# gillesdegottex/percivaltts

Hardware: AMD Instinct MI355X
Metric: acoustic frames/sec per WGAN-GP critic+gen step (higher is better)
Workload: dtype f32

## Files before the change

### percivaltts_amd/csrc/dense.hip

```cpp
#include "common.h"
#include <cstdlib>

namespace ptts {
namespace dns {

typedef __bf16 bf16x8 __attribute__((ext_vector_type(8)));
typedef __bf16 bf16x4 __attribute__((ext_vector_type(4)));
typedef __bf16 bf16x2 __attribute__((ext_vector_type(2)));
typedef float f32x4 __attribute__((ext_vector_type(4)));
typedef float f32x2 __attribute__((ext_vector_type(2)));
typedef unsigned u32x2 __attribute__((ext_vector_type(2)));
typedef unsigned short u16;

constexpr int THREADS = 512;
constexpr int NBLK = 256;
constexpr int BK = 32;

#define DNS_PRODUCTS(X) X(2, 0) X(1, 1) X(0, 2) X(1, 0) X(0, 1) X(0, 0)
#define DNS_PRODUCTS_NPL(NPL, X) do { if (NPL == 3) { X(2, 0) X(1, 1) X(0, 2) X(1, 0) X(0, 1) } X(0, 0) } while (0)

__device__ __forceinline__ unsigned pk_bf16(float a, float b) {
    return __builtin_bit_cast(unsigned, __builtin_convertvector((f32x2){a, b}, bf16x2));
}
__device__ __forceinline__ void split3_pair(float a, float b, unsigned& p1, unsigned& p2, unsigned& p3) {
    p1 = pk_bf16(a, b);
    const float ra = a - __builtin_bit_cast(float, p1 << 16), rb = b - __builtin_bit_cast(float, p1 & 0xffff0000u);
    p2 = pk_bf16(ra, rb);
    const float sa = ra - __builtin_bit_cast(float, p2 << 16), sb = rb - __builtin_bit_cast(float, p2 & 0xffff0000u);
    p3 = pk_bf16(sa, sb);
}
__device__ __forceinline__ float max_fast(float a, float b) {
    float r;
    asm("v_max_f32 %0, %1, %2" : "=v"(r) : "v"(a), "v"(b));
    return r;
}

__global__ __launch_bounds__(256) void split3_dense_weight_kernel(const float* __restrict__ w, long long ldw, int K, int N,
                                                                  int transposed, u16* __restrict__ planes, int NT, int KS) {
    const long long idx = (long long)blockIdx.x * 256 + threadIdx.x;
    if (idx >= (long long)NT * KS * 64) return;
    const int lane = (int)(idx & 63);
    const long long t = idx >> 6;
    const int ks = (int)(t % KS), nt = (int)(t / KS);
    const int n = nt * 16 + (lane & 15), k0 = ks * 32 + (lane >> 4) * 8;
    float v[8];
#pragma unroll
    for (int e = 0; e < 8; ++e) {
        const int k = k0 + e;
        v[e] = (n < N && k < K) ? (transposed ? w[(long long)n * ldw + k] : w[(long long)k * ldw + n]) : 0.f;
    }
    unsigned q[3][4];
#pragma unroll
    for (int h = 0; h < 4; ++h) split3_pair(v[2 * h], v[2 * h + 1], q[0][h], q[1][h], q[2][h]);
    const size_t ps = (size_t)NT * KS * 512;
#pragma unroll
    for (int p = 0; p < 3; ++p)
        *reinterpret_cast<uint4*>(planes + p * ps + (size_t)idx * 8) = make_uint4(q[p][0], q[p][1], q[p][2], q[p][3]);
}

constexpr int SPLIT_GROUP = 32;
struct SplitGroupArgs {
    const float* w[SPLIT_GROUP]; u16* planes[SPLIT_GROUP];
    long long ldw[SPLIT_GROUP];
    int K[SPLIT_GROUP], N[SPLIT_GROUP], transposed[SPLIT_GROUP], NT[SPLIT_GROUP], KS[SPLIT_GROUP];
    int rlo[SPLIT_GROUP], rhi[SPLIT_GROUP];
};
__global__ __launch_bounds__(256) void split3_dense_weight_grouped_kernel(SplitGroupArgs a) {
    const int i = blockIdx.y;
    const int NT = a.NT[i], KS = a.KS[i], K = a.K[i], N = a.N[i], transposed = a.transposed[i];
    const int rlo = a.rlo[i], rhi = a.rhi[i];
    const long long idx = (long long)blockIdx.x * 256 + threadIdx.x;
    if (idx >= (long long)NT * KS * 64) return;
    const float* __restrict__ w = a.w[i];
    u16* __restrict__ planes = a.planes[i];
    const long long ldw = a.ldw[i];
    const int lane = (int)(idx & 63);
    const long long t = idx >> 6;
    const int ks = (int)(t % KS), nt = (int)(t / KS);
    const int n = nt * 16 + (lane & 15), k0 = ks * 32 + (lane >> 4) * 8;
    float v[8];
#pragma unroll
    for (int e = 0; e < 8; ++e) {
        const int k = k0 + e;
        v[e] = (n < N && k < K && k >= rlo && k < rhi) ? (transposed ? w[(long long)n * ldw + k] : w[(long long)k * ldw + n]) : 0.f;
    }
    unsigned q[3][4];
#pragma unroll
    for (int h = 0; h < 4; ++h) split3_pair(v[2 * h], v[2 * h + 1], q[0][h], q[1][h], q[2][h]);
    const size_t ps = (size_t)NT * KS * 512;
#pragma unroll
    for (int p = 0; p < 3; ++p)
        *reinterpret_cast<uint4*>(planes + p * ps + (size_t)idx * 8) = make_uint4(q[p][0], q[p][1], q[p][2], q[p][3]);
}

constexpr int WDFT_FCH = 32;
template <int KW>
__global__ __launch_bounds__(256) void conv1d_wdft_planes_kernel(const float* __restrict__ w, const float* __restrict__ tw,
                                                                u16* __restrict__ planes, long long fstride, int NB, int Cin,
                                                                int N, int Kh, int NT, int KS) {
    const long long idx = (long long)blockIdx.x * 256 + threadIdx.x;
    if (idx >= (long long)NT * KS * 64) return;
    const int lane = (int)(idx & 63);
    const long long t = idx >> 6;
    const int ks = (int)(t % KS), nt = (int)(t / KS);
    const int n = nt * 16 + (lane & 15), k0 = ks * 32 + (lane >> 4) * 8;
    const int part = k0 >= Kh ? 1 : 0, c0 = k0 - part * Kh;
    float wr[KW][8];
#pragma unroll
    for (int k = 0; k < KW; ++k)
#pragma unroll
        for (int e = 0; e < 8; ++e)
            wr[k][e] = (n < N && c0 + e < Cin && k0 < 2 * Kh) ? w[((long long)k * Cin + c0 + e) * N + n] : 0.f;
    const size_t ps = (size_t)NT * KS * 512;
    const int f0 = blockIdx.y * WDFT_FCH;
    for (int f = f0; f < min(NB, f0 + WDFT_FCH); ++f) {
        const float* __restrict__ tr = tw + ((long long)f * 2 + part) * KW;
        float v[8] = {0.f, 0.f, 0.f, 0.f, 0.f, 0.f, 0.f, 0.f};
#pragma unroll
        for (int k = 0; k < KW; ++k) {
            const float c = tr[k];
#pragma unroll
            for (int e = 0; e < 8; ++e) v[e] = fmaf(c, wr[k][e], v[e]);
        }
        unsigned q[3][4];
#pragma unroll
        for (int h = 0; h < 4; ++h) split3_pair(v[2 * h], v[2 * h + 1], q[0][h], q[1][h], q[2][h]);
        u16* pf = planes + (long long)f * fstride;
#pragma unroll
        for (int p = 0; p < 3; ++p)
            *reinterpret_cast<uint4*>(pf + p * ps + (size_t)idx * 8) = make_uint4(q[p][0], q[p][1], q[p][2], q[p][3]);
    }
}

struct SplitStridedArgs {
    const float* w; u16* planes;
    long long stride_w, stride_p, ldw;
    int K, N, transposed, NT, KS;
    int windows;
    int T, NS, S, row_off, kvalid;
};
__global__ __launch_bounds__(256) void split3_dense_weight_strided_kernel(SplitStridedArgs a) {
    const int z = blockIdx.y;
    const int NT = a.NT, KS = a.KS, K = a.K, N = a.N, transposed = a.transposed;
    const long long idx = (long long)blockIdx.x * 256 + threadIdx.x;
    if (idx >= (long long)NT * KS * 64) return;
    const float* __restrict__ w;
    int rlo = 0, rhi = K;
    if (a.windows) {
        const int b = z / a.NS, sg = z - b * a.NS;
        const int r0 = a.row_off + sg * a.S;
        w = a.w + ((long long)b * a.T + r0) * a.ldw;
        rlo = r0 < 0 ? -r0 : 0;
        rhi = min(a.kvalid, a.T - r0);
    } else {
        w = a.w + (long long)z * a.stride_w;
    }
    u16* __restrict__ planes = a.planes + (long long)z * a.stride_p;
    const long long ldw = a.ldw;
    const int lane = (int)(idx & 63);
    const long long t = idx >> 6;
    const int ks = (int)(t % KS), nt = (int)(t / KS);
    const int n = nt * 16 + (lane & 15), k0 = ks * 32 + (lane >> 4) * 8;
    float v[8];
#pragma unroll
    for (int e = 0; e < 8; ++e) {
        const int k = k0 + e;
        v[e] = (n < N && k < K && k >= rlo && k < rhi) ? (transposed ? w[(long long)n * ldw + k] : w[(long long)k * ldw + n]) : 0.f;
    }
    unsigned q[3][4];
#pragma unroll
    for (int h = 0; h < 4; ++h) split3_pair(v[2 * h], v[2 * h + 1], q[0][h], q[1][h], q[2][h]);
    const size_t ps = (size_t)NT * KS * 512;
#pragma unroll
    for (int p = 0; p < 3; ++p)
        *reinterpret_cast<uint4*>(planes + p * ps + (size_t)idx * 8) = make_uint4(q[p][0], q[p][1], q[p][2], q[p][3]);
}

constexpr int SPL_ROW = 256 + 2;
__global__ __launch_bounds__(256) void split3_dense_weight_strided_lds_kernel(SplitStridedArgs a) {
    __shared__ float tile[32 * SPL_ROW];
    const int z = blockIdx.y, ks = blockIdx.x % a.KS, cb = blockIdx.x / a.KS;
    const float* __restrict__ w = a.w + (long long)z * a.stride_w;
    u16* __restrict__ planes = a.planes + (long long)z * a.stride_p;
    const int lane = threadIdx.x & 63, wave = threadIdx.x >> 6;
    const int n0 = cb * 256;
#pragma unroll
    for (int j = 0; j < 8; ++j) {
        const int r = wave + 4 * j, k = ks * 32 + r, n = n0 + 4 * lane;
        f32x4 v = {0.f, 0.f, 0.f, 0.f};
        if (k < a.K && n < a.N) v = *reinterpret_cast<const f32x4*>(w + (long long)k * a.ldw + n);
        float* d = tile + r * SPL_ROW + 4 * lane;
        d[0] = v[0]; d[1] = v[1]; d[2] = v[2]; d[3] = v[3];
    }
    __syncthreads();
    const size_t ps = (size_t)a.NT * a.KS * 512;
    const int li = lane & 15, lg = lane >> 4;
#pragma unroll
    for (int j = 0; j < 4; ++j) {
        const int ntl = wave + 4 * j;
        const int nt = cb * 16 + ntl;
        if (nt >= a.NT) continue;
        float v[8];
#pragma unroll
        for (int e = 0; e < 8; ++e) v[e] = tile[(8 * lg + e) * SPL_ROW + 16 * ntl + li];
        unsigned q[3][4];
#pragma unroll
        for (int h = 0; h < 4; ++h) split3_pair(v[2 * h], v[2 * h + 1], q[0][h], q[1][h], q[2][h]);
        const size_t idx = ((size_t)nt * a.KS + ks) * 64 + lane;
#pragma unroll
        for (int p = 0; p < 3; ++p)
            *reinterpret_cast<uint4*>(planes + p * ps + idx * 8) = make_uint4(q[p][0], q[p][1], q[p][2], q[p][3]);
    }
}

#ifndef DNS_DEPTH
#define DNS_DEPTH 2
#endif
struct DenseArgs {
    const float* A; const float* mask_src; const float* in_scale; const float* in_shift;
    const u16* planes; const float* bias; const float* out_mask; float* C;
    int M, N, K, NT, KS;
    long long lda, ldc;
    float alpha, out_alpha;
    int accumulate, has_affine, vec_out;
    const float* res; int res_rows; long long ldr;
    long long bsA, bsP, bsC;
    double* stats;
    const float* om_scale; const float* om_shift;
};

template <int MODE, bool AFFINE, int MT, int NPL>
__global__ __launch_bounds__(THREADS) void dense_bf16x6_kernel(DenseArgs g) {
    if (gridDim.z > 1) {
        g.A += (long long)blockIdx.z * g.bsA;
        g.planes += (long long)blockIdx.z * g.bsP;
        g.C += (long long)blockIdx.z * g.bsC;
    }
    constexpr int TBM = 16 * MT;
    constexpr int NA = (TBM * 8 + THREADS - 1) / THREADS;
    constexpr int ROWS = NA * THREADS / 8;
    constexpr int PL = ROWS * BK;
    constexpr bool MASK = MODE == PTTS_IN_MASKMUL;
    __shared__ __attribute__((aligned(16))) u16 As[2][NPL * PL];
    const int tid = threadIdx.x, lane = tid & 63;
    const int wave = __builtin_amdgcn_readfirstlane(tid >> 6);
    const int li = lane & 15, lg = lane >> 4;
    const int m0 = blockIdx.x * TBM, n0 = blockIdx.y * NBLK;
    const int KS = g.KS;
    const bool wave_live = n0 + 32 * wave < g.N;

    const int kq = tid & 7;
    const float* pa[NA]; const float* pm[NA]; bool oka[NA]; int dst[NA];
#pragma unroll
    for (int j = 0; j < NA; ++j) {
        const int row = (tid + j * THREADS) >> 3;
        oka[j] = row < TBM && m0 + row < g.M;
        const long long base = (long long)(oka[j] ? m0 + row : 0) * g.lda + 4 * kq;
        pa[j] = g.A + base;
        pm[j] = MASK ? g.mask_src + base : nullptr;
        dst[j] = row * BK + ((((kq >> 1) ^ ((row >> 1) & 2))) << 3) + (kq & 1) * 4;
    }
    struct Stage { f32x4 va[NA], vm[MASK ? NA : 1], sc, sh; bool kok; };
    auto load_a = [&](int s, Stage& sg) {
        const int k = s * BK + 4 * kq;
        sg.kok = k < g.K;
        const int ko = sg.kok ? s * BK : -4 * kq;
#pragma unroll
        for (int j = 0; j < NA; ++j) {
            sg.va[j] = *reinterpret_cast<const f32x4*>(pa[j] + ko);
            if (MASK) sg.vm[j] = *reinterpret_cast<const f32x4*>(pm[j] + ko);
        }
        if (AFFINE) {
            sg.sc = *reinterpret_cast<const f32x4*>(g.in_scale + (sg.kok ? k : 0));
            sg.sh = *reinterpret_cast<const f32x4*>(g.in_shift + (sg.kok ? k : 0));
        }
    };
    auto commit = [&](const Stage& sg, u16* as) {
        const f32x4 z4 = {0.f, 0.f, 0.f, 0.f};
#pragma unroll
        for (int j = 0; j < NA; ++j) {
            f32x4 a = sg.va[j];
            if (MODE == PTTS_IN_LRELU) {
                if (AFFINE) a = a * sg.sc + sg.sh;
                if (!(oka[j] && sg.kok)) a = z4;
#pragma unroll
                for (int e = 0; e < 4; ++e) a[e] = max_fast(a[e], g.alpha * a[e]);
            } else if (MASK) {
                if (!(oka[j] && sg.kok)) a = z4;
#pragma unroll
                for (int e = 0; e < 4; ++e) a[e] = a[e] * (sg.vm[j][e] > 0.f ? 1.f : g.alpha);
            } else {
                if (!(oka[j] && sg.kok)) a = z4;
            }
            u16* d = as + dst[j];
            if (NPL == 3) {
                unsigned a1, a2, a3, b1, b2, b3;
                split3_pair(a[0], a[1], a1, a2, a3);
                split3_pair(a[2], a[3], b1, b2, b3);
                *reinterpret_cast<u32x2*>(d) = (u32x2){a1, b1};
                *reinterpret_cast<u32x2*>(d + PL) = (u32x2){a2, b2};
                *reinterpret_cast<u32x2*>(d + 2 * PL) = (u32x2){a3, b3};
            } else {
                *reinterpret_cast<u32x2*>(d) = (u32x2){pk_bf16(a[0], a[1]), pk_bf16(a[2], a[3])};
            }
        }
    };

    const size_t ps = (size_t)g.NT * KS * 512;
    const u16* wp[2];
#pragma unroll
    for (int j = 0; j < 2; ++j) wp[j] = g.planes + (((size_t)((n0 >> 4) + 2 * (wave_live ? wave : 0) + j) * KS) * 64 + lane) * 8;
    auto load_w = [&](int s, bf16x8 (&wf)[2][NPL]) {
#pragma unroll
        for (int j = 0; j < 2; ++j)
#pragma unroll
            for (int p = 0; p < NPL; ++p) wf[j][p] = *reinterpret_cast<const bf16x8*>(wp[j] + p * ps + (size_t)s * 512);
    };

    f32x4 acc[MT][2];
#pragma unroll
    for (int i = 0; i < MT; ++i) { acc[i][0] = f32x4{0.f, 0.f, 0.f, 0.f}; acc[i][1] = f32x4{0.f, 0.f, 0.f, 0.f}; }
    const int boff = li * BK + ((lg ^ ((li >> 1) & 2)) << 3);
    auto mfma_rows = [&](const u16* as, const bf16x8 (&wf)[2][NPL], int i0, int i1) {
#pragma unroll
        for (int i = i0; i < i1; ++i) {
            bf16x8 bf[NPL];
#pragma unroll
            for (int p = 0; p < NPL; ++p) bf[p] = *reinterpret_cast<const bf16x8*>(as + p * PL + boff + i * 16 * BK);
#define DNS_MM(PA, PW)                                                                                    \
            acc[i][0] = __builtin_amdgcn_mfma_f32_16x16x32_bf16(wf[0][PW < NPL ? PW : 0], bf[PA < NPL ? PA : 0], acc[i][0], 0, 0, 0);    \
            acc[i][1] = __builtin_amdgcn_mfma_f32_16x16x32_bf16(wf[1][PW < NPL ? PW : 0], bf[PA < NPL ? PA : 0], acc[i][1], 0, 0, 0);
            DNS_PRODUCTS_NPL(NPL, DNS_MM);
#undef DNS_MM
        }
    };

    constexpr int DEPTH = DNS_DEPTH;
    Stage sg[DEPTH];
    bf16x8 wc[2][NPL], wn[2][NPL];
#pragma unroll
    for (int j = 0; j < DEPTH; ++j) load_a(j, sg[j]);
    load_w(0, wc);
    commit(sg[0], As[0]);
    load_a(DEPTH, sg[0]);
    __syncthreads();
    auto step = [&](int s, int cut, Stage& nx) {
        const u16* as = As[s & 1];
        load_w(s + 1 < KS ? s + 1 : s, wn);
        mfma_rows(as, wc, 0, cut);
        commit(nx, As[(s + 1) & 1]);
        load_a(s + 1 + DEPTH, nx);
        mfma_rows(as, wc, cut, MT);
#pragma unroll
        for (int j = 0; j < 2; ++j)
#pragma unroll
            for (int p = 0; p < NPL; ++p) wc[j][p] = wn[j][p];
        __syncthreads();
    };
    auto run = [&](int cut) {
        int s = 0;
        for (; s + DEPTH <= KS; s += DEPTH) {
#pragma unroll
            for (int j = 0; j < DEPTH; ++j) step(s + j, cut, sg[(j + 1) % DEPTH]);
        }
#pragma unroll
        for (int j = 0; j < DEPTH; ++j)
            if (s + j < KS) step(s + j, cut, sg[(j + 1) % DEPTH]);
    };
    if (wave < 4) run(2); else run(MT - 2);
    if (!wave_live) return;
    const bool interior = m0 + TBM <= g.M;
    if (!g.vec_out) {
#pragma unroll
        for (int j = 0; j < 2; ++j)
#pragma unroll
            for (int i = 0; i < MT; ++i) {
                const int m = m0 + 16 * i + li;
                if (m >= g.M) continue;
#pragma unroll
                for (int e = 0; e < 4; ++e) {
                    const int n = n0 + 32 * wave + 16 * j + 4 * lg + e;
                    if (n >= g.N) continue;
                    const long long off = (long long)m * g.ldc + n;
                    float v = acc[i][j][e] + (g.bias ? g.bias[n] : 0.f);
                    if (g.out_mask) v *= g.out_mask[off] > 0.f ? 1.f : g.out_alpha;
                    if (g.res) { int mr = m; while (mr >= g.res_rows) mr -= g.res_rows; v += g.res[(long long)mr * g.ldr + n]; }
                    g.C[off] = v;
                }
            }
        return;
    }
#pragma unroll
    for (int j = 0; j < 2; ++j) {
        const int n = n0 + 32 * wave + 16 * j + 4 * lg;
        if (n >= g.N) continue;
        f32x4 bv = {0.f, 0.f, 0.f, 0.f};
        if (g.bias) bv = *reinterpret_cast<const f32x4*>(g.bias + n);
        const long long off0 = (long long)(m0 + li) * g.ldc + n;
        auto res_at = [&](int m) { int mr = m; while (mr >= g.res_rows) mr -= g.res_rows; return g.res + (long long)mr * g.ldr + n; };
        f32x4 ssum = {0.f, 0.f, 0.f, 0.f}, ssq = {0.f, 0.f, 0.f, 0.f};
        f32x4 osc = {1.f, 1.f, 1.f, 1.f}, osh = {0.f, 0.f, 0.f, 0.f};
        if (g.om_scale) { osc = *reinterpret_cast<const f32x4*>(g.om_scale + n); osh = *reinterpret_cast<const f32x4*>(g.om_shift + n); }
        auto aff_store = [&](f32x4& v, const f32x4& z) {
#pragma unroll
            for (int e = 0; e < 4; ++e) {
                const float gd = v[e] * ((z[e] * osc[e] + osh[e]) > 0.f ? 1.f : g.out_alpha);
                ssum[e] += gd * z[e]; ssq[e] += gd;
                v[e] = gd * osc[e];
            }
        };
        if (interior) {
            f32x4 mk[MT], old[MT];
            if (g.out_mask) {
#pragma unroll
                for (int i = 0; i < MT; ++i) mk[i] = *reinterpret_cast<const f32x4*>(g.out_mask + off0 + (long long)16 * i * g.ldc);
            }
            if (g.res) {
#pragma unroll
                for (int i = 0; i < MT; ++i) old[i] = *reinterpret_cast<const f32x4*>(res_at(m0 + 16 * i + li));
            }
#pragma unroll
            for (int i = 0; i < MT; ++i) {
                f32x4 v = acc[i][j] + bv;
                if (g.om_scale) {
                    aff_store(v, mk[i]);
                } else if (g.out_mask) {
#pragma unroll
                    for (int e = 0; e < 4; ++e) v[e] = v[e] * (mk[i][e] > 0.f ? 1.f : g.out_alpha);
                }
                if (g.res) v += old[i];
                if (g.stats && !g.om_scale) { ssum += v; ssq += v * v; }
                *reinterpret_cast<f32x4*>(g.C + off0 + (long long)16 * i * g.ldc) = v;
            }
        } else {
#pragma unroll
            for (int i = 0; i < MT; ++i) {
                const int m = m0 + 16 * i + li;
                if (m >= g.M) continue;
                const long long off = off0 + (long long)16 * i * g.ldc;
                f32x4 v = acc[i][j] + bv;
                if (g.out_mask) {
                    const f32x4 mk = *reinterpret_cast<const f32x4*>(g.out_mask + off);
                    if (g.om_scale) {
                        aff_store(v, mk);
                    } else {
#pragma unroll
                        for (int e = 0; e < 4; ++e) v[e] = v[e] * (mk[e] > 0.f ? 1.f : g.out_alpha);
                    }
                }
                if (g.res) v += *reinterpret_cast<const f32x4*>(res_at(m));
                if (g.stats && !g.om_scale) { ssum += v; ssq += v * v; }
                *reinterpret_cast<f32x4*>(g.C + off) = v;
            }
        }
        if (g.stats) {
#pragma unroll
            for (int e = 0; e < 4; ++e)
#pragma unroll
                for (int m = 1; m < 16; m <<= 1) { ssum[e] += __shfl_xor(ssum[e], m, 64); ssq[e] += __shfl_xor(ssq[e], m, 64); }
            if (li == 0) {
                double* row = g.stats + (size_t)blockIdx.x * 2 * g.N;
#pragma unroll
                for (int e = 0; e < 4; ++e) { row[n + e] = (double)ssum[e]; row[g.N + n + e] = (double)ssq[e]; }
            }
        }
    }
}

static int pick_mt(int M, int col_blocks) {
    static int forced = -1;
    if (forced < 0) { const char* e = getenv("PTTS_DENSE_MT"); forced = e ? atoi(e) : 0; }
    if (forced >= 4 && forced <= 8) return forced;
    int best = 8; double best_eff = -1.0;
    for (int mt = 4; mt <= 8; ++mt) {
        const long long blocks = (long long)((M + 16 * mt - 1) / (16 * mt)) * col_blocks;
        const long long rounds = (blocks + 255) / 256;
        const double eff = (double)M * col_blocks / (double)(rounds * 256 * 16 * mt);
        if (eff > best_eff + 1e-9) { best_eff = eff; best = mt; }
    }
    return best;
}


typedef short s16x4 __attribute__((ext_vector_type(4)));
typedef s16x4 __attribute__((address_space(3)))* lds_s16x4_ptr;
__device__ __forceinline__ bf16x4 tr_read(const u16* p) {
    return __builtin_bit_cast(bf16x4, __builtin_amdgcn_ds_read_tr16_b64_v4i16((lds_s16x4_ptr)(p)));
}
__device__ __forceinline__ bf16x8 cat8(bf16x4 a, bf16x4 b) { return __builtin_shufflevector(a, b, 0, 1, 2, 3, 4, 5, 6, 7); }

struct WgradArgs {
    const float* A; const float* dY; const float* mask_src; const float* in_scale; const float* in_shift;
    float* partials;
    int Kin, N, M;
    long long lda, ldb;
    float alpha;
    int tiles_n, steps_total, split;
};

constexpr int WT = 128;
constexpr int WROW = WT;
constexpr int WPL = 32 * WROW;
constexpr int WPART = WT * WT + WT;

template <int MODE, bool AFFINE, int NPL>
__global__ __launch_bounds__(THREADS) void dense_wgrad_bf16x6_kernel(WgradArgs g) {
    constexpr bool MASK = MODE == PTTS_IN_MASKMUL;
    extern __shared__ __attribute__((aligned(16))) u16 lds_w[];
    const int tid = threadIdx.x, lane = tid & 63;
    const int wave = __builtin_amdgcn_readfirstlane(tid >> 6);
    const int li = lane & 15, lg = lane >> 4;
    const int tile = blockIdx.y, tk = tile / g.tiles_n, tn = tile - tk * g.tiles_n;
    const int k0 = tk * WT, n0 = tn * WT;
    const int per = (g.steps_total + g.split - 1) / g.split;
    const int s_begin = blockIdx.x * per, s_end = min(g.steps_total, s_begin + per);
    const int nsteps = max(0, s_end - s_begin);

    const int c4 = tid & 31;
    const bool a_ok = k0 + 4 * c4 < g.Kin, d_ok = n0 + 4 * c4 < g.N;
    const float* pa = g.A + (a_ok ? k0 + 4 * c4 : 0);
    const float* pm = MASK ? g.mask_src + (a_ok ? k0 + 4 * c4 : 0) : nullptr;
    const float* pd = g.dY + (d_ok ? n0 + 4 * c4 : 0);
    int dst[2];
#pragma unroll
    for (int j = 0; j < 2; ++j) {
        const int row = (tid + j * THREADS) >> 5;
        dst[j] = row * WROW + ((((c4 >> 2) + row + 4 * (row >> 3)) & 7) << 4) + (c4 & 3) * 4;
    }
    f32x4 sc = {1.f, 1.f, 1.f, 1.f}, sh = {0.f, 0.f, 0.f, 0.f};
    if (AFFINE && a_ok) { sc = *reinterpret_cast<const f32x4*>(g.in_scale + k0 + 4 * c4); sh = *reinterpret_cast<const f32x4*>(g.in_shift + k0 + 4 * c4); }
    struct Stage { f32x4 va[2], vm[MASK ? 2 : 1], vd[2]; bool ok[2]; };
    auto load = [&](int s, Stage& sg) {
#pragma unroll
        for (int j = 0; j < 2; ++j) {
            const int m = (s_begin + s) * 32 + ((tid + j * THREADS) >> 5);
            sg.ok[j] = s < nsteps && m < g.M;
            const long long r = sg.ok[j] ? m : 0;
            sg.va[j] = *reinterpret_cast<const f32x4*>(pa + r * g.lda);
            if (MASK) sg.vm[j] = *reinterpret_cast<const f32x4*>(pm + r * g.lda);
            sg.vd[j] = *reinterpret_cast<const f32x4*>(pd + r * g.ldb);
        }
    };
    f32x4 bsum = {0.f, 0.f, 0.f, 0.f};
    auto commit = [&](const Stage& sg, u16* ls) {
        const f32x4 z4 = {0.f, 0.f, 0.f, 0.f};
#pragma unroll
        for (int j = 0; j < 2; ++j) {
            f32x4 a = sg.va[j], d = sg.vd[j];
            if (MODE == PTTS_IN_LRELU) {
                if (AFFINE) a = a * sc + sh;
                if (!(sg.ok[j] && a_ok)) a = z4;
#pragma unroll
                for (int e = 0; e < 4; ++e) a[e] = max_fast(a[e], g.alpha * a[e]);
            } else if (MASK) {
                if (!(sg.ok[j] && a_ok)) a = z4;
#pragma unroll
                for (int e = 0; e < 4; ++e) a[e] = a[e] * (sg.vm[j][e] > 0.f ? 1.f : g.alpha);
            } else {
                if (!(sg.ok[j] && a_ok)) a = z4;
            }
            if (!(sg.ok[j] && d_ok)) d = z4;
            bsum += d;
            u16* q = ls + dst[j];
            if (NPL == 3) {
                unsigned a1, a2, a3, b1, b2, b3;
                split3_pair(a[0], a[1], a1, a2, a3);
                split3_pair(a[2], a[3], b1, b2, b3);
                *reinterpret_cast<u32x2*>(q) = (u32x2){a1, b1};
                *reinterpret_cast<u32x2*>(q + WPL) = (u32x2){a2, b2};
                *reinterpret_cast<u32x2*>(q + 2 * WPL) = (u32x2){a3, b3};
                split3_pair(d[0], d[1], a1, a2, a3);
                split3_pair(d[2], d[3], b1, b2, b3);
                q += 3 * WPL;
                *reinterpret_cast<u32x2*>(q) = (u32x2){a1, b1};
                *reinterpret_cast<u32x2*>(q + WPL) = (u32x2){a2, b2};
                *reinterpret_cast<u32x2*>(q + 2 * WPL) = (u32x2){a3, b3};
            } else {
                *reinterpret_cast<u32x2*>(q) = (u32x2){pk_bf16(a[0], a[1]), pk_bf16(a[2], a[3])};
                *reinterpret_cast<u32x2*>(q + 3 * WPL) = (u32x2){pk_bf16(d[0], d[1]), pk_bf16(d[2], d[3])};
            }
        }
    };

    auto tr_off = [&](int t, int half) {
        const int row = 8 * lg + (li >> 2) + 4 * half;
        return row * WROW + (((t + row + 4 * (row >> 3)) & 7) << 4) + (li & 3) * 4;
    };
    int ao[2][2], bo[4][2];
#pragma unroll
    for (int h = 0; h < 2; ++h) {
#pragma unroll
        for (int i = 0; i < 2; ++i) ao[i][h] = tr_off(2 * (wave & 3) + i, h);
#pragma unroll
        for (int i = 0; i < 4; ++i) bo[i][h] = 3 * WPL + tr_off(4 * (wave >> 2) + i, h);
    }
    f32x4 acc[2][4];
#pragma unroll
    for (int i = 0; i < 2; ++i)
#pragma unroll
        for (int j = 0; j < 4; ++j) acc[i][j] = f32x4{0.f, 0.f, 0.f, 0.f};
    auto mfma_tile_row = [&](const u16* ls, int i, const bf16x8 (&bf)[4][NPL]) {
        bf16x8 af[NPL];
#pragma unroll
        for (int p = 0; p < NPL; ++p) af[p] = cat8(tr_read(ls + p * WPL + ao[i][0]), tr_read(ls + p * WPL + ao[i][1]));
#define DNS_MM(PA, PW)                                                                                       \
        _Pragma("unroll") for (int j = 0; j < 4; ++j)                                                        \
            acc[i][j] = __builtin_amdgcn_mfma_f32_16x16x32_bf16(af[PA < NPL ? PA : 0], bf[j][PW < NPL ? PW : 0], acc[i][j], 0, 0, 0);
        DNS_PRODUCTS_NPL(NPL, DNS_MM);
#undef DNS_MM
    };
    auto read_bf = [&](const u16* ls, bf16x8 (&bf)[4][NPL]) {
#pragma unroll
        for (int j = 0; j < 4; ++j)
#pragma unroll
            for (int p = 0; p < NPL; ++p) bf[j][p] = cat8(tr_read(ls + p * WPL + bo[j][0]), tr_read(ls + p * WPL + bo[j][1]));
    };

    Stage sg;
    load(0, sg);
    commit(sg, lds_w);
    load(1, sg);
    __syncthreads();
    u16* const buf0 = lds_w;
    u16* const buf1 = lds_w + 6 * WPL;
    auto step = [&](int s, const u16* cur, u16* nxt, bool stage_first) {
        bf16x8 bf[4][NPL];
        if (stage_first) { commit(sg, nxt); load(s + 2, sg); }
        read_bf(cur, bf);
        mfma_tile_row(cur, 0, bf);
        if (!stage_first) { commit(sg, nxt); load(s + 2, sg); }
        mfma_tile_row(cur, 1, bf);
        __syncthreads();
    };
    if (wave < 4) {
        int s = 0;
        for (; s + 1 < nsteps; s += 2) { step(s, buf0, buf1, false); step(s + 1, buf1, buf0, false); }
        if (s < nsteps) step(s, buf0, buf1, false);
    } else {
        int s = 0;
        for (; s + 1 < nsteps; s += 2) { step(s, buf0, buf1, true); step(s + 1, buf1, buf0, true); }
        if (s < nsteps) step(s, buf0, buf1, true);
    }

    float* out = g.partials + ((size_t)tile * g.split + blockIdx.x) * WPART;
#pragma unroll
    for (int i = 0; i < 2; ++i)
#pragma unroll
        for (int j = 0; j < 4; ++j) {
            const int n = 64 * (wave >> 2) + 16 * j + li;
#pragma unroll
            for (int r = 0; r < 4; ++r) {
                const int k = 32 * (wave & 3) + 16 * i + 4 * lg + r;
                out[k * WT + n] = acc[i][j][r];
            }
        }
    {
        float* red = reinterpret_cast<float*>(lds_w);
        __syncthreads();
        *reinterpret_cast<f32x4*>(red + tid * 4) = bsum;
        __syncthreads();
        if (tid < WT) {
            float v = 0.f;
#pragma unroll
            for (int q = 0; q < 16; ++q) v += red[(q * 32 + (tid >> 2)) * 4 + (tid & 3)];
            out[WT * WT + tid] = v;
        }
    }
}


constexpr int DR_MAX = 16;
struct DwReduceArgs {
    int n;
    int blk_begin[DR_MAX + 1];
    const float* partials[DR_MAX]; float* C[DR_MAX]; float* colsum[DR_MAX];
    int split[DR_MAX], tiles_n[DR_MAX], Kin[DR_MAX], N[DR_MAX];
    long long ldc[DR_MAX];
};
constexpr int DR_BPT = (WPART + 255) / 256;
__global__ __launch_bounds__(256) void dense_wgrad_reduce_kernel(DwReduceArgs a) {
    int gi = 0;
    while ((int)blockIdx.x >= a.blk_begin[gi + 1]) ++gi;
    const int b = blockIdx.x - a.blk_begin[gi];
    const int tile = b / DR_BPT, e = (b - tile * DR_BPT) * 256 + threadIdx.x;
    if (e >= WPART) return;
    const int S = a.split[gi];
    const float* p = a.partials[gi] + (size_t)tile * S * WPART + e;
    float v0 = 0.f, v1 = 0.f, v2 = 0.f, v3 = 0.f, v4 = 0.f, v5 = 0.f, v6 = 0.f, v7 = 0.f;
    int s = 0;
    for (; s + 8 <= S; s += 8) {
        const float* q = p + (size_t)s * WPART;
        const float t0 = q[0], t1 = q[(size_t)WPART], t2 = q[(size_t)2 * WPART], t3 = q[(size_t)3 * WPART];
        const float t4 = q[(size_t)4 * WPART], t5 = q[(size_t)5 * WPART], t6 = q[(size_t)6 * WPART], t7 = q[(size_t)7 * WPART];
        v0 += t0; v1 += t1; v2 += t2; v3 += t3; v4 += t4; v5 += t5; v6 += t6; v7 += t7;
    }
    for (; s < S; ++s) v0 += p[(size_t)s * WPART];
    const float v = ((v0 + v1) + (v2 + v3)) + ((v4 + v5) + (v6 + v7));
    const int tk = tile / a.tiles_n[gi], tn = tile - tk * a.tiles_n[gi];
    if (e < WT * WT) {
        const int k = tk * WT + (e >> 7), n = tn * WT + (e & (WT - 1));
        if (k < a.Kin[gi] && n < a.N[gi]) atomicAdd(a.C[gi] + (long long)k * a.ldc[gi] + n, v);
    } else if (tk == 0 && a.colsum[gi]) {
        const int n = tn * WT + (e - WT * WT);
        if (n < a.N[gi]) atomicAdd(a.colsum[gi] + n, v);
    }
}

}
}

using namespace ptts;
using namespace ptts::dns;

extern "C" size_t ptts_dense_planes_bytes(int N, int K) {
    if (N <= 0 || K <= 0) return 0;
    const size_t NT = (size_t)((N + NBLK - 1) / NBLK) * (NBLK / 16), KS = (size_t)(K + BK - 1) / BK;
    return 3 * NT * KS * 512 * sizeof(u16);
}

extern "C" int ptts_split3_dense_weight(const float* w, long long ldw, int K, int N, int transposed, void* planes, void* stream) {
    PTTS_REQUIRE(w && planes, "split3_dense_weight: null pointer");
    PTTS_REQUIRE(K > 0 && N > 0 && ldw >= (transposed ? K : N), "split3_dense_weight: bad dims K=%d N=%d ldw=%lld", K, N, ldw);
    const int NT = (N + NBLK - 1) / NBLK * (NBLK / 16), KS = (K + BK - 1) / BK;
    const long long total = (long long)NT * KS * 64;
    hipLaunchKernelGGL(split3_dense_weight_kernel, dim3((unsigned)((total + 255) / 256)), dim3(256), 0, (hipStream_t)stream,
                       w, ldw, K, N, transposed, (u16*)planes, NT, KS);
    return check_launch("split3_dense_weight");
}

extern "C" int ptts_split3_dense_weight_grouped(const ptts_dense_split_desc* descs, int n, void* stream) {
    PTTS_REQUIRE(descs && n > 0, "split3_dense_weight_grouped: nothing to split");
    for (int base = 0; base < n; base += SPLIT_GROUP) {
        SplitGroupArgs a;
        const int m = n - base < SPLIT_GROUP ? n - base : SPLIT_GROUP;
        long long most = 0;
        for (int i = 0; i < m; ++i) {
            const ptts_dense_split_desc& d = descs[base + i];
            PTTS_REQUIRE(d.w && d.planes, "split3_dense_weight_grouped: null pointer (weight %d)", base + i);
            PTTS_REQUIRE(d.K > 0 && d.N > 0 && d.ldw >= (d.transposed ? d.K : d.N), "split3_dense_weight_grouped: bad dims K=%d N=%d ldw=%lld (weight %d)", d.K, d.N, d.ldw, base + i);
            a.w[i] = d.w; a.planes[i] = (u16*)d.planes; a.ldw[i] = d.ldw; a.K[i] = d.K; a.N[i] = d.N; a.transposed[i] = d.transposed;
            a.rlo[i] = 0; a.rhi[i] = d.K;
            a.NT[i] = (d.N + NBLK - 1) / NBLK * (NBLK / 16); a.KS[i] = (d.K + BK - 1) / BK;
            const long long total = (long long)a.NT[i] * a.KS[i] * 64;
            if (total > most) most = total;
        }
        hipLaunchKernelGGL(split3_dense_weight_grouped_kernel, dim3((unsigned)((most + 255) / 256), (unsigned)m), dim3(256), 0, (hipStream_t)stream, a);
    }
    return check_launch("split3_dense_weight_grouped");
}

extern "C" int ptts_split3_dense_weight_strided(const float* w, long long stride_w, void* planes, long long stride_planes_bytes, int n,
                                                long long ldw, int K, int N, int transposed, void* stream) {
    PTTS_REQUIRE(w && planes && n > 0 && n <= 65535, "split3_dense_weight_strided: nothing to split (or more than 65535 matrices)");
    PTTS_REQUIRE(K > 0 && N > 0 && ldw >= (transposed ? K : N), "split3_dense_weight_strided: bad dims K=%d N=%d ldw=%lld", K, N, ldw);
    PTTS_REQUIRE(stride_planes_bytes % 16 == 0, "split3_dense_weight_strided: the planes' stride must keep 16-byte alignment");
    SplitStridedArgs a;
    a.w = w; a.planes = (u16*)planes; a.stride_w = stride_w; a.stride_p = stride_planes_bytes / 2; a.ldw = ldw;
    a.K = K; a.N = N; a.transposed = transposed;
    a.NT = (N + NBLK - 1) / NBLK * (NBLK / 16); a.KS = (K + BK - 1) / BK;
    a.windows = 0; a.T = a.NS = a.S = a.row_off = a.kvalid = 0;
    const long long total = (long long)a.NT * a.KS * 64;
    static int lds_form = -1;
    if (lds_form < 0) { const char* e = getenv("PTTS_SPLIT_LDS"); lds_form = e ? atoi(e) : 1; }
    if (lds_form && !transposed && N % 4 == 0 && ldw % 4 == 0 && stride_w % 4 == 0 && ((uintptr_t)w & 15) == 0) {
        const unsigned cbn = (unsigned)((N + 255) / 256);
        hipLaunchKernelGGL(split3_dense_weight_strided_lds_kernel, dim3((unsigned)a.KS * cbn, (unsigned)n), dim3(256), 0, (hipStream_t)stream, a);
        return check_launch("split3_dense_weight_strided");
    }
    hipLaunchKernelGGL(split3_dense_weight_strided_kernel, dim3((unsigned)((total + 255) / 256), (unsigned)n), dim3(256), 0, (hipStream_t)stream, a);
    return check_launch("split3_dense_weight_strided");
}

extern "C" int ptts_split3_frame_windows(const float* x, int B, int T, int C, int NS, int S, int row_off, int P, int kvalid,
                                         void* planes, long long stride_planes_bytes, void* stream) {
    PTTS_REQUIRE(x && planes && B > 0 && T > 0 && C > 0 && NS > 0 && S > 0 && P > 0 && kvalid > 0 && kvalid <= P, "split3_frame_windows: bad arguments");
    PTTS_REQUIRE((long long)B * NS <= 65535 && stride_planes_bytes % 16 == 0, "split3_frame_windows: more than 65535 windows, or a planes stride off 16-byte alignment");
    SplitStridedArgs a;
    a.w = x; a.planes = (u16*)planes; a.stride_w = 0; a.stride_p = stride_planes_bytes / 2; a.ldw = C;
    a.K = P; a.N = C; a.transposed = 0;
    a.NT = (C + NBLK - 1) / NBLK * (NBLK / 16); a.KS = (P + BK - 1) / BK;
    a.windows = 1; a.T = T; a.NS = NS; a.S = S; a.row_off = row_off; a.kvalid = kvalid;
    const long long total = (long long)a.NT * a.KS * 64;
    hipLaunchKernelGGL(split3_dense_weight_strided_kernel, dim3((unsigned)((total + 255) / 256), (unsigned)(B * NS)), dim3(256), 0, (hipStream_t)stream, a);
    return check_launch("split3_frame_windows");
}

extern "C" int ptts_dense_bf16x6_supported(int M, int N, int K, long long lda, long long ldc) {
    (void)ldc;
    return (M > 0 && N > 0 && K > 0 && K % 4 == 0 && lda % 4 == 0 && K <= 65536 &&
            (long long)((N + NBLK - 1) / NBLK) <= 65535) ? 1 : 0;
}

extern "C" int ptts_dense_bf16x6_res(const float* A, const void* planes, const float* bias, float* C, int M, int N, int K,
                                     long long lda, long long ldc, int in_mode, const float* in_scale, const float* in_shift,
                                     const float* mask_src, float alpha, const float* res, int res_rows, long long ldr,
                                     const float* out_mask, void* stream);
extern "C" int ptts_dense_bf16x6(const float* A, const void* planes, const float* bias, float* C, int M, int N, int K,
                                 long long lda, long long ldc, int in_mode, const float* in_scale, const float* in_shift,
                                 const float* mask_src, float alpha, int accumulate, const float* out_mask, void* stream) {
    return ptts_dense_bf16x6_res(A, planes, bias, C, M, N, K, lda, ldc, in_mode, in_scale, in_shift, mask_src, alpha,
                                 accumulate ? C : nullptr, M, ldc, out_mask, stream);
}

static int dense_launch(const float* A, const void* planes, const float* bias, float* C, int M, int N, int K,
                        long long lda, long long ldc, int in_mode, const float* in_scale, const float* in_shift,
                        const float* mask_src, float alpha, const float* res, int res_rows, long long ldr,
                        const float* out_mask, double* stats, int stats_capacity_rows, int* stats_rows_out, void* stream);
static thread_local const float* g_om_scale = nullptr;
static thread_local const float* g_om_shift = nullptr;

extern "C" int ptts_dense_bf16x6_res(const float* A, const void* planes, const float* bias, float* C, int M, int N, int K,
                                     long long lda, long long ldc, int in_mode, const float* in_scale, const float* in_shift,
                                     const float* mask_src, float alpha, const float* res, int res_rows, long long ldr,
                                     const float* out_mask, void* stream) {
    return dense_launch(A, planes, bias, C, M, N, K, lda, ldc, in_mode, in_scale, in_shift, mask_src, alpha, res, res_rows, ldr, out_mask,
                        nullptr, 0, nullptr, stream);
}

extern "C" int ptts_dense_bf16x6_stats(const float* A, const void* planes, const float* bias, float* C, int M, int N, int K,
                                       long long lda, long long ldc, int in_mode, const float* in_scale, const float* in_shift,
                                       float alpha, double* stats, int capacity_rows, int* nrows_out, void* stream) {
    PTTS_REQUIRE(stats && nrows_out && capacity_rows > 0, "dense_bf16x6_stats: no room for the sums");
    return dense_launch(A, planes, bias, C, M, N, K, lda, ldc, in_mode, in_scale, in_shift, nullptr, alpha, nullptr, 0, 0, nullptr,
                        stats, capacity_rows, nrows_out, stream);
}
extern "C" int ptts_dense_bf16x6_bwd_affine(const float* A, const void* planes, float* C, int M, int N, int K, long long lda, long long ldc,
                                            const float* z, const float* scale, const float* shift, float alpha,
                                            double* stats, int capacity_rows, int* nrows_out, void* stream) {
    PTTS_REQUIRE(z && scale && shift && stats && nrows_out && capacity_rows > 0, "dense_bf16x6_bwd_affine: null pointer");
    PTTS_REQUIRE((((uintptr_t)scale | (uintptr_t)shift) & 15) == 0, "dense_bf16x6_bwd_affine: scale / shift must be 16-byte aligned");
    g_om_scale = scale; g_om_shift = shift;
    const int rc = dense_launch(A, planes, nullptr, C, M, N, K, lda, ldc, PTTS_IN_NONE, nullptr, nullptr, nullptr, alpha, nullptr, 0, 0, z,
                                stats, capacity_rows, nrows_out, stream);
    g_om_scale = g_om_shift = nullptr;
    return rc;
}
extern "C" int ptts_dense_bf16x6_stats_rows(int M, int N) {
    if (M <= 0 || N <= 0) return 0;
    const int mt = pick_mt(M, (N + NBLK - 1) / NBLK);
    return (M + 16 * mt - 1) / (16 * mt);
}

static int dense_launch(const float* A, const void* planes, const float* bias, float* C, int M, int N, int K,
                        long long lda, long long ldc, int in_mode, const float* in_scale, const float* in_shift,
                        const float* mask_src, float alpha, const float* res, int res_rows, long long ldr,
                        const float* out_mask, double* stats, int stats_capacity_rows, int* stats_rows_out, void* stream) {
    const int accumulate = res != nullptr;
    PTTS_REQUIRE(!res || (res_rows > 0 && ldr >= N && M <= 8LL * res_rows), "dense_bf16x6: bad residual (rows %d, ldr %lld)", res_rows, ldr);
    PTTS_REQUIRE(A && planes && C, "dense_bf16x6: null matrix");
    PTTS_REQUIRE(ptts_dense_bf16x6_supported(M, N, K, lda, ldc), "dense_bf16x6: unsupported shape M=%d N=%d K=%d lda=%lld ldc=%lld (K and lda must be multiples of 4)", M, N, K, lda, ldc);
    PTTS_REQUIRE(lda >= K && ldc >= N, "dense_bf16x6: bad leading dims");
    PTTS_REQUIRE(in_mode >= 0 && in_mode <= 2, "dense_bf16x6: bad in_mode %d", in_mode);
    PTTS_REQUIRE((in_scale == nullptr) == (in_shift == nullptr), "dense_bf16x6: scale/shift must come together");
    PTTS_REQUIRE(in_mode != PTTS_IN_MASKMUL || mask_src, "dense_bf16x6: MASKMUL needs mask_src");
    PTTS_REQUIRE(in_mode == PTTS_IN_LRELU || !in_scale, "dense_bf16x6: scale/shift need PTTS_IN_LRELU");
    PTTS_REQUIRE(!(out_mask && bias), "dense_bf16x6: out_mask with bias is not defined");
    PTTS_REQUIRE(alpha >= 0.f && alpha <= 1.f, "dense_bf16x6: LeakyReLU slope %g outside [0, 1]", alpha);
    const bool vec_out = N % 4 == 0 && ldc % 4 == 0 && ((uintptr_t)C & 15) == 0 && (!bias || ((uintptr_t)bias & 15) == 0) &&
                         (!out_mask || ((uintptr_t)out_mask & 15) == 0) && (!res || (((uintptr_t)res & 15) == 0 && ldr % 4 == 0));
    PTTS_REQUIRE(((uintptr_t)A & 15) == 0 && (!mask_src || ((uintptr_t)mask_src & 15) == 0) &&
                 (!in_scale || (((uintptr_t)in_scale | (uintptr_t)in_shift) & 15) == 0), "dense_bf16x6: A, its mask and scale/shift must be 16-byte aligned");
    DenseArgs g;
    g.A = A; g.mask_src = mask_src; g.in_scale = in_scale; g.in_shift = in_shift; g.planes = (const u16*)planes; g.bias = bias;
    g.out_mask = out_mask; g.C = C; g.M = M; g.N = N; g.K = K;
    g.NT = (N + NBLK - 1) / NBLK * (NBLK / 16); g.KS = (K + BK - 1) / BK;
    g.lda = lda; g.ldc = ldc; g.alpha = alpha; g.out_alpha = alpha; g.accumulate = accumulate; g.has_affine = in_scale != nullptr; g.vec_out = vec_out;
    g.res = res; g.res_rows = res ? res_rows : 1; g.ldr = ldr;
    g.bsA = g.bsP = g.bsC = 0;
    const int cb = (N + NBLK - 1) / NBLK;
    const int mt = pick_mt(M, cb);
    const dim3 grid((unsigned)((M + 16 * mt - 1) / (16 * mt)), (unsigned)cb);
    g.stats = stats;
    g.om_scale = g_om_scale; g.om_shift = g_om_shift;
    if (stats) {
        PTTS_REQUIRE(vec_out, "dense_bf16x6_stats: N and ldc must be multiples of 4, C (and bias) 16-byte aligned");
        PTTS_REQUIRE(stats_capacity_rows >= (int)grid.x, "dense_bf16x6_stats: room for %d rows of sums, %d needed", stats_capacity_rows, (int)grid.x);
        *stats_rows_out = (int)grid.x;
    }
    hipStream_t st = (hipStream_t)stream;
    const bool one = ptts::bf16_products();
#define DNS_L(MODE, AFF, MT) do { if (one) hipLaunchKernelGGL((dense_bf16x6_kernel<MODE, AFF, MT, 1>), grid, dim3(THREADS), 0, st, g); \
                                  else hipLaunchKernelGGL((dense_bf16x6_kernel<MODE, AFF, MT, 3>), grid, dim3(THREADS), 0, st, g); } while (0)
#define DNS_M(MT)                                                                \
    do {                                                                         \
        if (in_mode == PTTS_IN_LRELU) { if (in_scale) DNS_L(PTTS_IN_LRELU, true, MT); else DNS_L(PTTS_IN_LRELU, false, MT); } \
        else if (in_mode == PTTS_IN_MASKMUL) DNS_L(PTTS_IN_MASKMUL, false, MT);  \
        else DNS_L(PTTS_IN_NONE, false, MT);                                     \
    } while (0)
    switch (mt) {
        case 4: DNS_M(4); break;
        case 5: DNS_M(5); break;
        case 6: DNS_M(6); break;
        case 7: DNS_M(7); break;
        default: DNS_M(8); break;
    }
#undef DNS_M
#undef DNS_L
    return check_launch("dense_bf16x6");
}

extern "C" int ptts_conv1d_freq_kernel_planes(const float* w, const float* tw, void* planes, int NB, int KW, int Cin, int N, int Kh,
                                              void* stream) {
    PTTS_REQUIRE(w && tw && planes && NB > 0 && Cin > 0 && N > 0, "conv1d_freq_kernel_planes: bad arguments");
    PTTS_REQUIRE(Kh >= Cin && Kh % 8 == 0, "conv1d_freq_kernel_planes: Kh=%d must be a multiple of 8 and >= Cin=%d", Kh, Cin);
    const int NT = (N + NBLK - 1) / NBLK * (NBLK / 16), KS = (2 * Kh + BK - 1) / BK;
    const long long total = (long long)NT * KS * 64;
    const long long fstride = (long long)(ptts_dense_planes_bytes(N, 2 * Kh) / sizeof(u16));
    const dim3 grid((unsigned)((total + 255) / 256), (unsigned)((NB + WDFT_FCH - 1) / WDFT_FCH));
#define WDFT(KWv) hipLaunchKernelGGL(conv1d_wdft_planes_kernel<KWv>, grid, dim3(256), 0, (hipStream_t)stream, w, tw, (u16*)planes, fstride, NB, Cin, N, Kh, NT, KS)
    switch (KW) {
        case 3: WDFT(3); break;
        case 5: WDFT(5); break;
        case 7: WDFT(7); break;
        case 9: WDFT(9); break;
        case 11: WDFT(11); break;
        case 21: WDFT(21); break;
        default: set_error("conv1d_freq_kernel_planes: KW=%d not instantiated (3, 5, 7, 9, 11, 21)", KW); return PTTS_EINVAL;
    }
#undef WDFT
    return check_launch("conv1d_freq_kernel_planes");
}

extern "C" int ptts_dense_bf16x6_batched(const float* A, long long strideA, const void* planes, long long stride_planes_bytes,
                                         const float* bias, float* C, long long strideC, int nbatch, int M, int N, int K,
                                         long long lda, long long ldc, int planes_count, void* stream) {
    PTTS_REQUIRE(A && planes && C && nbatch > 0 && nbatch <= 65535, "dense_bf16x6_batched: bad arguments");
    PTTS_REQUIRE(ptts_dense_bf16x6_supported(M, N, K, lda, ldc), "dense_bf16x6_batched: unsupported shape M=%d N=%d K=%d lda=%lld ldc=%lld", M, N, K, lda, ldc);
    PTTS_REQUIRE(lda >= K && ldc >= N && planes_count >= 1 && planes_count <= 3 && planes_count != 2, "dense_bf16x6_batched: bad leading dims / planes");
    PTTS_REQUIRE(stride_planes_bytes % 16 == 0 && strideA % 4 == 0 && ((uintptr_t)A & 15) == 0, "dense_bf16x6_batched: strides of A / planes must keep 16-byte alignment");
    const bool vec_out = N % 4 == 0 && ldc % 4 == 0 && strideC % 4 == 0 && ((uintptr_t)C & 15) == 0 && (!bias || ((uintptr_t)bias & 15) == 0);
    DenseArgs g;
    g.A = A; g.mask_src = nullptr; g.in_scale = nullptr; g.in_shift = nullptr; g.planes = (const u16*)planes; g.bias = bias;
    g.out_mask = nullptr; g.C = C; g.M = M; g.N = N; g.K = K;
    g.NT = (N + NBLK - 1) / NBLK * (NBLK / 16); g.KS = (K + BK - 1) / BK;
    g.lda = lda; g.ldc = ldc; g.alpha = 0.f; g.out_alpha = 0.f; g.accumulate = 0; g.has_affine = 0; g.vec_out = vec_out;
    g.res = nullptr; g.res_rows = 1; g.ldr = 0;
    g.bsA = strideA; g.bsP = stride_planes_bytes / 2; g.bsC = strideC;
    g.stats = nullptr; g.om_scale = g.om_shift = nullptr;
    const int cb = (N + NBLK - 1) / NBLK;
    int mt = 8; double best_eff = -1.0;
    {
        static int forced = -1;
        if (forced < 0) { const char* e = getenv("PTTS_DENSE_BATCHED_MT"); forced = e ? atoi(e) : 0; }
        for (int m = 8; m >= 4; --m) {
            const int tiles = (M + 16 * m - 1) / (16 * m);
            const double eff = (double)M / (double)(tiles * 16 * m);
            if (eff > best_eff + 1e-9) { best_eff = eff; mt = m; }
        }
        if (forced >= 4 && forced <= 8) mt = forced;
    }
    const dim3 grid((unsigned)((M + 16 * mt - 1) / (16 * mt)), (unsigned)cb, (unsigned)nbatch);
    hipStream_t st = (hipStream_t)stream;
    const bool one = planes_count == 1;
#define DNS_B(MT) do { if (one) hipLaunchKernelGGL((dense_bf16x6_kernel<PTTS_IN_NONE, false, MT, 1>), grid, dim3(THREADS), 0, st, g); \
                       else hipLaunchKernelGGL((dense_bf16x6_kernel<PTTS_IN_NONE, false, MT, 3>), grid, dim3(THREADS), 0, st, g); } while (0)
    switch (mt) {
        case 4: DNS_B(4); break;
        case 5: DNS_B(5); break;
        case 6: DNS_B(6); break;
        case 7: DNS_B(7); break;
        default: DNS_B(8); break;
    }
#undef DNS_B
    return check_launch("dense_bf16x6_batched");
}

extern "C" int ptts_dense_wgrad_bf16x6_supported(int Kin, int N, int M, long long lda, long long ldb) {
    return (Kin > 0 && N > 0 && M > 0 && Kin % 4 == 0 && N % 4 == 0 && lda % 4 == 0 && ldb % 4 == 0 &&
            (long long)((Kin + WT - 1) / WT) * ((N + WT - 1) / WT) <= 65535) ? 1 : 0;
}

namespace {
int wgrad_split(int Kin, int N, int M) {
    const int tiles = ((Kin + WT - 1) / WT) * ((N + WT - 1) / WT), steps = (M + 31) / 32;
    int split = (256 + tiles - 1) / tiles;
    static int env_split = -1;
    if (env_split < 0) { const char* e = getenv("PTTS_DENSE_WGRAD_SPLIT"); env_split = e ? atoi(e) : 0; }
    if (env_split > 0) split = env_split;
    if (split > steps) split = steps;
    return split < 1 ? 1 : split;
}
}

extern "C" size_t ptts_dense_wgrad_workspace_bytes(int Kin, int N, int M) {
    if (Kin <= 0 || N <= 0 || M <= 0) return 0;
    const size_t tiles = (size_t)((Kin + WT - 1) / WT) * ((N + WT - 1) / WT);
    return tiles * wgrad_split(Kin, N, M) * WPART * sizeof(float);
}

extern "C" int ptts_dense_wgrad_bf16x6_partials(const float* A, const float* dY, const float* mask_src, const float* in_scale,
                                                const float* in_shift, void* workspace, size_t workspace_bytes, int* split_out,
                                                int Kin, int N, int M, long long lda, long long ldb, int in_mode, float alpha,
                                                void* stream) {
    PTTS_REQUIRE(A && dY && workspace && split_out, "dense_wgrad_bf16x6: null pointer");
    PTTS_REQUIRE(ptts_dense_wgrad_bf16x6_supported(Kin, N, M, lda, ldb), "dense_wgrad_bf16x6: unsupported shape Kin=%d N=%d M=%d lda=%lld ldb=%lld", Kin, N, M, lda, ldb);
    PTTS_REQUIRE(lda >= Kin && ldb >= N, "dense_wgrad_bf16x6: bad leading dims");
    PTTS_REQUIRE(in_mode >= 0 && in_mode <= 2, "dense_wgrad_bf16x6: bad in_mode %d", in_mode);
    PTTS_REQUIRE((in_scale == nullptr) == (in_shift == nullptr), "dense_wgrad_bf16x6: scale/shift must come together");
    PTTS_REQUIRE(in_mode != PTTS_IN_MASKMUL || mask_src, "dense_wgrad_bf16x6: MASKMUL needs mask_src");
    PTTS_REQUIRE(in_mode == PTTS_IN_LRELU || !in_scale, "dense_wgrad_bf16x6: scale/shift need PTTS_IN_LRELU");
    PTTS_REQUIRE(alpha >= 0.f && alpha <= 1.f, "dense_wgrad_bf16x6: LeakyReLU slope %g outside [0, 1]", alpha);
    PTTS_REQUIRE(((uintptr_t)A & 15) == 0 && ((uintptr_t)dY & 15) == 0 && (!mask_src || ((uintptr_t)mask_src & 15) == 0) &&
                 (!in_scale || (((uintptr_t)in_scale | (uintptr_t)in_shift) & 15) == 0), "dense_wgrad_bf16x6: operands must be 16-byte aligned");
    const size_t need = ptts_dense_wgrad_workspace_bytes(Kin, N, M);
    if (workspace_bytes < need) { set_error("dense_wgrad_bf16x6: workspace %zu < %zu", workspace_bytes, need); return PTTS_EWORKSPACE; }
    WgradArgs g;
    g.A = A; g.dY = dY; g.mask_src = mask_src; g.in_scale = in_scale; g.in_shift = in_shift; g.partials = (float*)workspace;
    g.Kin = Kin; g.N = N; g.M = M; g.lda = lda; g.ldb = ldb; g.alpha = alpha;
    const int tiles_k = (Kin + WT - 1) / WT;
    g.tiles_n = (N + WT - 1) / WT;
    g.steps_total = (M + 31) / 32;
    const int tiles = tiles_k * g.tiles_n;
    g.split = wgrad_split(Kin, N, M);
    *split_out = g.split;
    const dim3 grid((unsigned)g.split, (unsigned)tiles);
    hipStream_t st = (hipStream_t)stream;
    constexpr size_t lds = (size_t)2 * 6 * WPL * sizeof(u16);
    const bool one = ptts::bf16_products();
#define DNS_W(MODE, AFF)                                                                                                  \
    do {                                                                                                                  \
        static bool attr = false;                                                                                         \
        if (!attr) { (void)hipFuncSetAttribute(reinterpret_cast<const void*>(&dense_wgrad_bf16x6_kernel<MODE, AFF, 3>), hipFuncAttributeMaxDynamicSharedMemorySize, (int)lds); \
                     (void)hipFuncSetAttribute(reinterpret_cast<const void*>(&dense_wgrad_bf16x6_kernel<MODE, AFF, 1>), hipFuncAttributeMaxDynamicSharedMemorySize, (int)lds); attr = true; } \
        if (one) hipLaunchKernelGGL((dense_wgrad_bf16x6_kernel<MODE, AFF, 1>), grid, dim3(THREADS), lds, st, g);          \
        else hipLaunchKernelGGL((dense_wgrad_bf16x6_kernel<MODE, AFF, 3>), grid, dim3(THREADS), lds, st, g);              \
    } while (0)
    if (in_mode == PTTS_IN_LRELU) { if (in_scale) DNS_W(PTTS_IN_LRELU, true); else DNS_W(PTTS_IN_LRELU, false); }
    else if (in_mode == PTTS_IN_MASKMUL) DNS_W(PTTS_IN_MASKMUL, false);
    else DNS_W(PTTS_IN_NONE, false);
#undef DNS_W
    return check_launch("dense_wgrad_bf16x6_partials");
}

extern "C" int ptts_dense_wgrad_reduce_grouped(const ptts_dense_wgrad_reduce_desc* descs, int n, void* stream) {
    PTTS_REQUIRE(descs && n > 0, "dense_wgrad_reduce_grouped: nothing to reduce");
    for (int base = 0; base < n; base += DR_MAX) {
        DwReduceArgs a;
        a.n = n - base < DR_MAX ? n - base : DR_MAX;
        int blocks = 0;
        for (int i = 0; i < a.n; ++i) {
            const ptts_dense_wgrad_reduce_desc& d = descs[base + i];
            PTTS_REQUIRE(d.partials && d.C && d.split > 0 && d.Kin > 0 && d.N > 0 && d.ldc >= d.N, "dense_wgrad_reduce_grouped: bad product %d", base + i);
            a.blk_begin[i] = blocks;
            a.tiles_n[i] = (d.N + WT - 1) / WT;
            blocks += ((d.Kin + WT - 1) / WT) * a.tiles_n[i] * DR_BPT;
            a.partials[i] = d.partials; a.C[i] = d.C; a.colsum[i] = d.colsum_b; a.split[i] = d.split; a.Kin[i] = d.Kin; a.N[i] = d.N; a.ldc[i] = d.ldc;
        }
        a.blk_begin[a.n] = blocks;
        hipLaunchKernelGGL(dense_wgrad_reduce_kernel, dim3((unsigned)blocks), dim3(256), 0, (hipStream_t)stream, a);
        int rc = check_launch("dense_wgrad_reduce_grouped");
        if (rc) return rc;
    }
    return PTTS_OK;
}

extern "C" int ptts_dense_wgrad_bf16x6(const float* A, const float* dY, const float* mask_src, const float* in_scale,
                                       const float* in_shift, float* C, float* colsum_b, void* workspace, size_t workspace_bytes,
                                       int Kin, int N, int M, long long lda, long long ldb, long long ldc, int in_mode,
                                       float alpha, void* stream) {
    PTTS_REQUIRE(C && ldc >= N, "dense_wgrad_bf16x6: bad output");
    int split = 0;
    int rc = ptts_dense_wgrad_bf16x6_partials(A, dY, mask_src, in_scale, in_shift, workspace, workspace_bytes, &split, Kin, N, M,
                                              lda, ldb, in_mode, alpha, stream);
    if (rc) return rc;
    ptts_dense_wgrad_reduce_desc d;
    d.partials = (const float*)workspace; d.split = split; d.Kin = Kin; d.N = N; d.ldc = ldc; d.C = C; d.colsum_b = colsum_b;
    return ptts_dense_wgrad_reduce_grouped(&d, 1, stream);
}
```

### percivaltts_amd/ops.py

```python
import contextlib
import ctypes
import os

import torch

from . import _hip
from ._hip import call, ptr, stream, f32c, _workspace
from .ops_offline import *

IN_NONE, IN_LRELU, IN_MASKMUL = 0, 1, 2
PAD_SAME, PAD_CAUSAL = 0, 1
ACT_NONE, ACT_LRELU, ACT_SIGMOID, ACT_TANH = 0, 1, 2, 3
ACT_CODES = {None: ACT_NONE, 'linear': ACT_NONE, 'lrelu': ACT_LRELU, 'sigmoid': ACT_SIGMOID, 'tanh': ACT_TANH}


class Lazy(object):
    __slots__ = ('z', 'scale', 'shift', 'lrelu', 'alpha')

    def __init__(self, z, scale=None, shift=None, lrelu=False, alpha=0.3):
        self.z, self.scale, self.shift, self.lrelu, self.alpha = z, scale, shift, lrelu, alpha

    @property
    def shape(self):
        return self.z.shape

    def tensor(self):
        if self.scale is None and not self.lrelu:
            return self.z
        return affine_act(self.z, self.scale, self.shift, 'lrelu' if self.lrelu else None, self.alpha)


def as_lazy(v):
    return v if isinstance(v, Lazy) else Lazy(v)


def as_tensor(v):
    return v.tensor() if isinstance(v, Lazy) else v


def _fusable(lz):
    if lz.lrelu:
        return IN_LRELU, lz.scale, lz.shift
    if lz.scale is None:
        return IN_NONE, None, None
    return None


def _prep(v):
    lz = as_lazy(v)
    f = _fusable(lz)
    if f is None:
        return lz.tensor(), IN_NONE, None, None, lz.alpha
    return lz.z, f[0], f[1], f[2], lz.alpha


class _Flags(object):
    skip_param_grads = False
    deterministic = os.environ.get('PTTS_DETERMINISTIC', '0') == '1'
    bf16_products = False


def bf16_products(on=None):
    if on is not None:
        _Flags.bf16_products = bool(on)
    _hip.lib().ptts_set_bf16_products(1 if _Flags.bf16_products else 0)
    return _Flags.bf16_products


def deterministic(on=None):
    if on is not None:
        _Flags.deterministic = bool(on)
    _hip.lib().ptts_set_deterministic(1 if _Flags.deterministic else 0)
    return _Flags.deterministic


@contextlib.contextmanager
def input_grad_only():
    old = _Flags.skip_param_grads
    _Flags.skip_param_grads = True
    try:
        yield
    finally:
        _Flags.skip_param_grads = old


class _Deferred(object):
    active = False
    items = []
    conv_items = []
    streams = []

    @classmethod
    def live(cls):
        return cls.active and not _Flags.deterministic

    @classmethod
    def targets(cls, *params):
        return tuple([grad_target(p) for p in params] if cls.live() else [None] * len(params))

    @classmethod
    def note_stream(cls, s=None):
        sid = _hip.stream_id() if s is None else s.cuda_stream
        if all(sid != q.cuda_stream for q in cls.streams):
            cls.streams.append(torch.cuda.current_stream() if s is None else s)
        return sid

    @classmethod
    def queue_conv(cls, *passes):
        cls.note_stream()
        cls.conv_items.extend(passes)

    @classmethod
    def reset(cls):
        st = (cls.items, cls.conv_items, cls.streams)
        cls.items, cls.conv_items, cls.streams = [], [], []
        return st


@contextlib.contextmanager
def deferred_weight_grads():
    old = _Deferred.active
    _Deferred.active = True
    try:
        yield
        flush_weight_grads()
    finally:
        _Deferred.active = old
        _Deferred.reset()


def deferred_detach():
    return _Deferred.reset()


def deferred_attach(st):
    if st is None:
        return
    items, conv_items, streams = st
    _Deferred.items = list(items) + _Deferred.items
    _Deferred.conv_items = list(conv_items) + _Deferred.conv_items
    for q in streams:
        _Deferred.note_stream(q)


def grad_target(p):
    if p is None or not p.requires_grad:
        return None
    if p.is_leaf:
        g = p.grad
        return g if (g is not None and g.is_contiguous() and g.shape == p.shape) else None
    base = p._base
    if base is None or not base.is_leaf or base.grad is None or not p.is_contiguous() or not base.grad.is_contiguous():
        return None
    if base.stride() != base.grad.stride():
        return None
    off = p.storage_offset() - base.storage_offset()
    return base.grad.view(-1)[off:off + p.numel()].view(p.shape)


_WG_FLUSH_AT = int(__import__('os').environ.get('PTTS_WG_FLUSH', '3'))


def _defer_wgrad(x2, dy2, gw, gb, K_in, N, M_rows, mode, scale, shift, mask_src, alpha):
    sid = _Deferred.note_stream()
    _Deferred.items.append((sid, x2, dy2, mask_src, scale, shift, gw, gb, K_in, N, M_rows, mode, alpha))
    if _WG_FLUSH_AT > 0:
        mine = [it for it in _Deferred.items if it[0] == sid]
        if len(mine) >= _WG_FLUSH_AT:
            _Deferred.items = [it for it in _Deferred.items if it[0] != sid]
            _launch_wgrads(mine)


def _wgrad_split_ok(x2, dy2, mask_src, scale, shift, K_in, N, M_rows):
    if not (_DenseSplit.enabled and not _Flags.deterministic and M_rows >= 2048 and N >= _DenseSplit.wgrad_min_n and K_in >= 16):
        return False
    if not _hip.lib().ptts_dense_wgrad_bf16x6_supported(K_in, N, M_rows, x2.stride(0), dy2.stride(0)):
        return False
    return all(t is None or t.data_ptr() % 16 == 0 for t in (x2, dy2, mask_src, scale, shift))


def _launch_wgrads(items):
    cur = torch.cuda.current_stream()
    rest, split_items = [], []
    for it in items:
        (_, x2, dy2, mask_src, scale, shift, gw, gb, K_in, N, M_rows, mode, alpha) = it
        if _wgrad_split_ok(x2, dy2, mask_src, scale, shift, K_in, N, M_rows):
            for t in (x2, dy2, mask_src):
                if t is not None:
                    t.record_stream(cur)
            ws = torch.empty(_hip.lib().ptts_dense_wgrad_workspace_bytes(K_in, N, M_rows), dtype=torch.uint8, device=x2.device)
            nsplit = ctypes.c_int(0)
            call('ptts_dense_wgrad_bf16x6_partials', ptr(x2), ptr(dy2), ptr(mask_src), ptr(scale), ptr(shift), ptr(ws), ws.numel(),
                 ctypes.byref(nsplit), K_in, N, M_rows, x2.stride(0), dy2.stride(0), mode, alpha, stream(), tag=(K_in, N, M_rows))
            split_items.append((ws, nsplit.value, K_in, N, gw, gb))
        else:
            rest.append(it)
    if split_items:
        descs = (_hip.DenseWgradReduceDesc * len(split_items))()
        for d, (ws, nsplit, K_in, N, gw, gb) in zip(descs, split_items):
            d.partials, d.split, d.Kin, d.N, d.ldc = ws.data_ptr(), nsplit, K_in, N, gw.stride(0)
            d.C, d.colsum_b = gw.data_ptr(), (gb.data_ptr() if gb is not None else None)
        call('ptts_dense_wgrad_reduce_grouped', ctypes.cast(descs, ctypes.c_void_p), len(split_items), stream(), tag=(len(split_items),))
    items = rest
    if not items:
        return
    descs = (_hip.WGradDesc * len(items))()
    for d, (_, x2, dy2, mask_src, scale, shift, gw, gb, K_in, N, M_rows, mode, alpha) in zip(descs, items):
        for t in (x2, dy2, mask_src):
            if t is not None:
                t.record_stream(cur)
        d.A, d.B, d.C, d.colsum_b = x2.data_ptr(), dy2.data_ptr(), gw.data_ptr(), (gb.data_ptr() if gb is not None else None)
        d.in_scale = scale.data_ptr() if scale is not None else None
        d.in_shift = shift.data_ptr() if shift is not None else None
        d.mask_src = mask_src.data_ptr() if mask_src is not None else None
        d.M, d.N, d.K = K_in, N, M_rows
        d.lda, d.ldb, d.ldc = x2.stride(0), dy2.stride(0), gw.stride(0)
        d.in_mode, d.alpha = mode, alpha
    call('ptts_gemm_wgrad_grouped', ctypes.cast(descs, ctypes.c_void_p), len(items), stream(), tag=(len(items),))


def flush_weight_grads():
    items, conv_items, streams = _Deferred.reset()
    if not (items or conv_items or streams):
        return
    cur = torch.cuda.current_stream()
    for s in streams:
        if s.cuda_stream != cur.cuda_stream:
            cur.wait_stream(s)
    if items:
        _launch_wgrads(items)
    if conv_items:
        _conv2d_reduce(conv_items, cur)


def _conv2d_reduce(passes, record=None):
    descs = (_hip.Conv2dReduceDesc * len(passes))()
    for d, (buf, off, nblocks, npart, nw, cout, dw, db) in zip(descs, passes):
        if record is not None:
            buf.record_stream(record)
        d.partials = buf.data_ptr() + off
        d.nblocks, d.npart, d.nw, d.cout = nblocks, npart, nw, cout
        d.dw = dw.data_ptr() if dw is not None else None
        d.dbias = db.data_ptr() if db is not None else None
    call('ptts_conv2d_reduce_grouped', ctypes.cast(descs, ctypes.c_void_p), len(passes), stream(), tag=(len(passes),))


_counter_cache = {}


def _stream_counter(device):
    key = (device.index, _hip.stream_id())
    c = _counter_cache.get(key)
    if c is None:
        c = _counter_cache[key] = torch.zeros(1, dtype=torch.int32, device=device)
    return c


class _C2M(object):
    default = os.environ.get('PTTS_CONV2D_MFMA', '1') == '1'
    enabled = default
    tables = {}

    @staticmethod
    def eligible(x, w, dil_t):
        KT, KF, Cin, Cout = w.shape
        return x.is_cuda and Cin == 4 and Cout == 4 and KT == 5 and KF == 5 and dil_t in (1, 2, 4, 8)

    @classmethod
    def table(cls, w, transposed, planes=3):
        flat = getattr(w, '_ptts_flat', None)
        epoch = None if flat is None else flat.epoch
        sid = _hip.stream_id()
        key = (id(w), sid, planes)
        ent = cls.tables.get(key)
        if ent is None or ent[0] is not w or ent[1] != w._version or ent[2] != epoch or flat is None:
            nb = _hip.lib().ptts_conv2d_mfma_table_bytes(5)
            reuse = ent is not None and ent[0] is w
            tf = ent[3] if reuse else torch.empty(nb, dtype=torch.uint8, device=w.device)
            tb = ent[4] if reuse else torch.empty(nb, dtype=torch.uint8, device=w.device)
            if len(cls.tables) > 512:
                cls.tables = {}
            cls.tables[key] = ent = (w, w._version, epoch, tf, tb)
            todo = [ent]
            if flat is not None:
                for k2, e2 in cls.tables.items():
                    if k2 is not key and k2[1] == sid and k2[2] == planes and getattr(e2[0], '_ptts_flat', None) is flat and \
                            (e2[1] != e2[0]._version or e2[2] != epoch):
                        cls.tables[k2] = e2 = (e2[0], e2[0]._version, epoch, e2[3], e2[4])
                        todo.append(e2)
            if len(todo) == 1:
                call('ptts_conv2d_mfma_tables', ptr(w), ptr(tf), ptr(tb), 5, 5, 4, 4, planes, stream(), tag=(5, 5, planes))
            else:
                n = len(todo)
                pw = (ctypes.c_void_p * n)(*[e[0].data_ptr() for e in todo])
                pf = (ctypes.c_void_p * n)(*[e[3].data_ptr() for e in todo])
                pb = (ctypes.c_void_p * n)(*[e[4].data_ptr() for e in todo])
                call('ptts_conv2d_mfma_tables_grouped', ctypes.cast(pw, ctypes.c_void_p), ctypes.cast(pf, ctypes.c_void_p),
                     ctypes.cast(pb, ctypes.c_void_p), n, planes, stream(), tag=(n, planes))
        return ent[4] if transposed else ent[3]

    @staticmethod
    def pad_t(dil_t, pad_mode):
        return 4 * dil_t if pad_mode == PAD_CAUSAL else 2 * dil_t

    @classmethod
    def clear(cls):
        cls.tables = {k: (e[0], None, -1, e[3], e[4]) for k, e in cls.tables.items()}


def conv2d_mfma(on):
    _C2M.enabled = _C2M.default if on is None else bool(on)
    _C2M.clear()


def conv2d_path_description():
    return ('4->4 5x5 layers: bf16x6 split on the bf16 matrix cores (fp32 accumulate); 1->4 / 4->1 layers: fp32 packed-FMA stencil'
            if _C2M.enabled else 'fp32 packed-FMA stencil')


def _is16(t):
    return t is not None and t.dtype == torch.bfloat16


class _BNStats(object):
    enabled = os.environ.get('PTTS_CONV_BN_STATS', '1') == '1'
    want = False
    last = None


def conv_bn_stats(on):
    _BNStats.enabled = (os.environ.get('PTTS_CONV_BN_STATS', '1') == '1') if on is None else bool(on)


def _conv2d_mfma_fwd(x, w, table, b, scale, shift, mask_src, out_mask, mode, alpha, dil_t, pad_t, planes=3, out_bf16=False):
    B, T, F, _ = x.shape
    assert planes in (1, 3) and (planes == 1 or not (_is16(x) or out_bf16)), 'bf16 tensors need the one-plane (bf16 arithmetic) kernels'
    assert mask_src is None or mask_src.dtype == x.dtype, 'conv2d: the mask source has the input\'s storage type'
    y = torch.empty((B, T, F, 4), dtype=torch.bfloat16 if out_bf16 else torch.float32, device=x.device)
    assert out_mask is None or out_mask.dtype == y.dtype, 'conv2d: the output mask has the output\'s storage type'
    if _BNStats.want and _BNStats.enabled and planes == 3 and mask_src is None and out_mask is None and \
            _hip.lib().ptts_conv2d_mfma_fwd_stats_supported(F, dil_t, mode):
        part = torch.empty((256, 8), dtype=torch.float64, device=x.device)
        nrows = ctypes.c_int(0)
        call('ptts_conv2d_mfma_fwd_stats', ptr(x), ptr(table), ptr(b), ptr(scale), ptr(shift), ptr(y), B, T, F, 5, pad_t, mode, alpha,
             ptr(part), 256, ctypes.byref(nrows), stream(), tag=(B, T, F, 4, 4, mode, 'stats'))
        _BNStats.last = (part, nrows.value, B * T * F)
        return y
    call('ptts_conv2d_mfma_fwd', ptr(x), ptr(table), ptr(b), ptr(scale), ptr(shift), ptr(mask_src), ptr(out_mask), ptr(y),
         B, T, F, 5, dil_t, pad_t, mode, alpha, planes, int(_is16(x)), int(out_bf16), stream(),
         tag=(B, T, F, 4, 4, mode, int(out_mask is not None), planes))
    return y


def _conv2d_mfma_wgrad(dy, x, mask_src, mode, alpha, dil_t, pad_t, planes=3):
    B, T, F, _ = x.shape
    assert planes == 1 or not (_is16(x) or _is16(dy))
    assert mask_src is None or mask_src.dtype == x.dtype
    nws = _hip.lib().ptts_conv2d_mfma_wgrad_workspace_bytes(B, T)
    buf = torch.empty(int(nws), dtype=torch.uint8, device=x.device)
    nblocks, npart = ctypes.c_int(0), ctypes.c_int(0)
    call('ptts_conv2d_mfma_wgrad_partials', ptr(dy), ptr(x), ptr(mask_src), ptr(buf), buf.numel(), ctypes.byref(nblocks),
         ctypes.byref(npart), B, T, F, 5, dil_t, pad_t, mode, alpha, planes, int(_is16(x)), int(_is16(dy)), stream(),
         tag=(B, T, F, 4, 4, mode, planes))
    return buf, nblocks.value, npart.value


class _C2MFused(object):
    default = os.environ.get('PTTS_C2M_FUSED', '1') == '1'
    enabled = default

    @staticmethod
    def ok(x, dil_t, pad_mode, planes):
        return _C2MFused.enabled and planes == 3 and dil_t == 1 and pad_mode == PAD_SAME and not _is16(x)


def conv2d_fused(on):
    _C2MFused.enabled = _C2MFused.default if on is None else bool(on)


def _conv2d_mfma_bwd_fused(kind, p, q, mask_src, w, alpha):
    B, T, F, _ = p.shape
    f32c(p, 'conv2d_bwd_fused.p'); f32c(q, 'conv2d_bwd_fused.q'); f32c(mask_src)
    assert q.shape == p.shape and (mask_src is None or mask_src.shape == p.shape)
    y = torch.empty_like(p)
    nws = _hip.lib().ptts_conv2d_mfma_bwd_fused_workspace_bytes(B, T)
    buf = torch.empty(int(nws), dtype=torch.uint8, device=p.device)
    nblocks, npart = ctypes.c_int(0), ctypes.c_int(0)
    call('ptts_conv2d_mfma_bwd_fused', ptr(p), ptr(q), ptr(mask_src), ptr(_C2M.table(w, kind == 1)), ptr(y), ptr(buf), buf.numel(),
         ctypes.byref(nblocks), ctypes.byref(npart), B, T, F, 5, 2, kind, alpha, stream(), tag=(B, T, F, kind))
    return y, buf, nblocks.value, npart.value


def _conv2d_mfma_bwd_fused_affine(dy, x, w, alpha, scale, shift):
    B, T, F, _ = dy.shape
    f32c(dy, 'conv2d_bwd_fused.dy'); f32c(x, 'conv2d_bwd_fused.x'); f32c(scale); f32c(shift)
    assert x.shape == dy.shape
    y = torch.empty_like(dy)
    nws = _hip.lib().ptts_conv2d_mfma_bwd_fused_workspace_bytes(B, T)
    buf = torch.empty(int(nws), dtype=torch.uint8, device=dy.device)
    nblocks, npart = ctypes.c_int(0), ctypes.c_int(0)
    call('ptts_conv2d_mfma_bwd_fused_affine', ptr(dy), ptr(x), ptr(_C2M.table(w, True)), ptr(y), ptr(buf), buf.numel(),
         ctypes.byref(nblocks), ctypes.byref(npart), B, T, F, 5, 2, alpha, ptr(scale), ptr(shift), stream(), tag=(B, T, F, 'affine'))
    return y, buf, nblocks.value, npart.value


def _st(t, name='tensor'):
    if t is None:
        return None
    if not (t.is_cuda and t.dtype in (torch.float32, torch.bfloat16) and t.is_contiguous()):
        raise _hip.HipLibraryError('{}: expected a contiguous float32 / bfloat16 device tensor, got {} {} contiguous={}'.format(
            name, t.device, t.dtype, t.is_contiguous()))
    return t


def _conv2d_fwd_raw(x, w, b, scale, shift, mask_src, mode, alpha, dil_t, pad_mode, planes=3, out_bf16=False):
    if planes == 1:
        _st(x, 'conv2d.x'); _st(mask_src, 'conv2d.mask_src'); f32c(w, 'conv2d.w'); f32c(b, 'conv2d.b'); f32c(scale); f32c(shift)
        if not (_C2M.eligible(x, w, dil_t) and dil_t == 1 and 0.0 <= alpha <= 1.0):
            raise _hip.HipLibraryError('conv2d: bf16 storage is built for the 4 -> 4 channel 5x5 layers at dilation 1')
        return _conv2d_mfma_fwd(x, w, _C2M.table(w, False, 1), b, scale, shift, mask_src, None, mode, alpha, dil_t,
                                _C2M.pad_t(dil_t, pad_mode), 1, out_bf16)
    f32c(x, 'conv2d.x'); f32c(w, 'conv2d.w'); f32c(b, 'conv2d.b'); f32c(scale); f32c(shift); f32c(mask_src)
    B, T, F, Cin = x.shape
    KT, KF, Ci2, Cout = w.shape
    assert Ci2 == Cin, 'conv2d: kernel Cin {} != input {}'.format(Ci2, Cin)
    assert b is None or b.numel() == Cout
    assert scale is None or (scale.numel() == Cin and shift.numel() == Cin)
    assert mask_src is None or mask_src.shape == x.shape
    if _C2M.enabled and _C2M.eligible(x, w, dil_t) and 0.0 <= alpha <= 1.0:
        return _conv2d_mfma_fwd(x, w, _C2M.table(w, False), b, scale, shift, mask_src, None, mode, alpha, dil_t,
                                _C2M.pad_t(dil_t, pad_mode))
    y = torch.empty((B, T, F, Cout), dtype=torch.float32, device=x.device)
    call('ptts_conv2d_fwd', ptr(x), ptr(w), ptr(b), ptr(scale), ptr(shift), ptr(mask_src), ptr(y),
         B, T, F, Cin, Cout, KT, KF, dil_t, pad_mode, mode, alpha, stream(), tag=(B, T, F, Cin, Cout, mode))
    return y


def _conv2d_mfma_bwd(dy, x, w, mask_src, mode, alpha, dil_t, pad_mode, want_dx, want_rows, planes):
    pad_t = _C2M.pad_t(dil_t, pad_mode)
    dx = None
    if want_dx and want_rows and mode == IN_LRELU and _C2MFused.ok(x, dil_t, pad_mode, planes):
        dx, buf, nblocks, npart = _conv2d_mfma_bwd_fused(1, dy, x, None, w, alpha)
    else:
        if want_dx:
            assert mode != IN_MASKMUL, 'conv2d_bwd: dx is not defined for MASKMUL (weight-only sweep)'
            dx = _conv2d_mfma_fwd(dy, w, _C2M.table(w, True, planes), None, None, None, None, x if mode == IN_LRELU else None,
                                  IN_NONE, alpha, dil_t, 4 * dil_t - pad_t, planes, _is16(x))
        if want_rows:
            buf, nblocks, npart = _conv2d_mfma_wgrad(dy, x, mask_src, mode, alpha, dil_t, pad_t, planes)
    return dx, ((buf, 4096, nblocks, npart, w.numel(), w.shape[3]) if want_rows else None)


def _conv2d_bwd_raw(dy, x, w, scale, shift, mask_src, mode, alpha, dil_t, pad_mode,
                    want_dx, want_dw, want_db, want_affine, planes=3):
    if planes == 1:
        _st(dy, 'conv2d_bwd.dy'); _st(x, 'conv2d_bwd.x'); _st(mask_src); f32c(w)
        assert scale is None and not want_affine, 'conv2d: no BatchNorm-fused input on the bf16-storage path'
    else:
        f32c(dy, 'conv2d_bwd.dy'); f32c(x, 'conv2d_bwd.x'); f32c(w); f32c(scale); f32c(shift); f32c(mask_src)
    B, T, F, Cin = x.shape
    KT, KF, _, Cout = w.shape
    assert dy.shape == (B, T, F, Cout), 'conv2d_bwd: dy shape {} vs {}'.format(tuple(dy.shape), (B, T, F, Cout))
    assert mask_src is None or mask_src.shape == x.shape
    dev = x.device
    if (planes == 1 or _C2M.enabled) and _C2M.eligible(x, w, dil_t) and scale is None and not want_affine and 0.0 <= alpha <= 1.0:
        dw = db = None
        dx, rows = _conv2d_mfma_bwd(dy, x, w, mask_src, mode, alpha, dil_t, pad_mode, want_dx, want_dw or want_db, planes)
        if rows is not None:
            dw = torch.zeros_like(w) if want_dw else None
            db = torch.zeros(Cout, dtype=torch.float32, device=dev) if want_db else None
            _conv2d_reduce([rows + (dw, db)])
        return dx, dw, db, None, None
    if planes == 3 and scale is not None and mode == IN_LRELU and want_dx and mask_src is None and _C2M.enabled and _BNStats.enabled and \
            _C2M.eligible(x, w, dil_t) and 0.0 <= alpha <= 1.0 and _C2MFused.ok(x, dil_t, pad_mode, planes) and \
            scale.data_ptr() % 16 == 0 and shift.data_ptr() % 16 == 0:
        dx, buf, nblocks, npart = _conv2d_mfma_bwd_fused_affine(dy, x, w, alpha, scale, shift)
        nw = KT * KF * Cin * Cout
        dw = torch.zeros_like(w) if want_dw else None
        db = torch.zeros(Cout, dtype=torch.float32, device=dev) if want_db else None
        daff = torch.zeros(2 * Cin, dtype=torch.float32, device=dev) if want_affine else None
        passes = []
        if want_dw or want_db:
            passes.append((buf, 4096, nblocks, npart, nw, Cout, dw, db))
        if want_affine:
            passes.append((buf, 4096 + 4 * (nw + Cout), nblocks, npart, Cin, Cin, daff[:Cin], daff[Cin:]))
        if passes:
            _conv2d_reduce(passes)
        return dx, dw, db, (daff[:Cin] if want_affine else None), (daff[Cin:] if want_affine else None)
    dx = torch.empty_like(x) if want_dx else None
    dw = torch.empty_like(w) if (want_dw or want_db) else None
    db = torch.empty(Cout, dtype=torch.float32, device=dev) if want_db else None
    dscale = torch.empty(Cin, dtype=torch.float32, device=dev) if want_affine else None
    dshift = torch.empty(Cin, dtype=torch.float32, device=dev) if want_affine else None
    nws = _hip.lib().ptts_conv2d_bwd_workspace_bytes(B, T, F, Cin, Cout, KT, KF, dil_t)
    ws = _workspace(nws, dev)
    call('ptts_conv2d_bwd', ptr(dy), ptr(x), ptr(w), ptr(scale), ptr(shift), ptr(mask_src),
         ptr(dx), ptr(dw), ptr(db), ptr(dscale), ptr(dshift), ptr(ws), ws.numel(),
         B, T, F, Cin, Cout, KT, KF, dil_t, pad_mode, mode, alpha, stream(),
         tag=(B, T, F, Cin, Cout, mode, int(want_dx), int(want_dw or want_db), int(want_affine)))
    return dx, (dw if want_dw else None), db, dscale, dshift


def _conv2d_bwd_deferred(dy, x, w, mask_src, mode, alpha, dil_t, pad_mode, want_dx, gw, gb, planes=3):
    B, T, F, Cin = x.shape
    KT, KF, _, Cout = w.shape
    if (planes == 1 or _C2M.enabled) and _C2M.eligible(x, w, dil_t) and 0.0 <= alpha <= 1.0:
        dx, rows = _conv2d_mfma_bwd(dy, x, w, mask_src, mode, alpha, dil_t, pad_mode, want_dx, True, planes)
        _Deferred.queue_conv(rows + (gw, gb))
        return dx
    nws = _hip.lib().ptts_conv2d_bwd_workspace_bytes(B, T, F, Cin, Cout, KT, KF, dil_t)
    if nws <= 16:
        return False
    dev = x.device
    buf = torch.empty(int(nws), dtype=torch.uint8, device=dev)
    dx = torch.empty_like(x) if want_dx else None
    nblocks = ctypes.c_int(0)
    call('ptts_conv2d_bwd_partials', ptr(dy), ptr(x), ptr(w), ptr(mask_src), ptr(dx), ptr(buf), buf.numel(),
         ctypes.byref(nblocks), B, T, F, Cin, Cout, KT, KF, dil_t, pad_mode, mode, alpha, stream(),
         tag=(B, T, F, Cin, Cout, mode, int(want_dx), 1, 0))
    nw = KT * KF * Cin * Cout
    _Deferred.queue_conv((buf, 4096, nblocks.value, nw + Cout + 2 * Cin, nw, Cout, gw, gb))
    return dx


class _DenseSplit(object):
    default = os.environ.get('PTTS_DENSE_SPLIT', '1') == '1'
    enabled = default
    planes = {}
    wgrad_min_n = int(os.environ.get('PTTS_DENSE_WGRAD_MIN_N', '16'))

    @classmethod
    def get(cls, Bm, K, N, ldb, transB):
        owner = Bm if hasattr(Bm, '_ptts_flat') else getattr(Bm, '_base', None)
        flat = getattr(owner, '_ptts_flat', None)
        if flat is None:
            return None
        sid = _hip.stream_id()
        key = (id(owner), Bm.data_ptr(), K, N, ldb, transB, sid)
        ent = cls.planes.get(key)
        if ent is None or ent[0] is not owner or ent[1] != owner._version or ent[2] != flat.epoch:
            reuse = ent is not None and ent[0] is owner
            buf = ent[3] if reuse else torch.empty(_hip.lib().ptts_dense_planes_bytes(N, K), dtype=torch.uint8, device=Bm.device)
            if len(cls.planes) > 512:
                cls.planes = {}
            cls.planes[key] = ent = (owner, owner._version, flat.epoch, buf, Bm)
            todo = [(key, ent)]
            for k2, e2 in cls.planes.items():
                if k2 is not key and k2[6] == sid and len(e2) == 5 and getattr(e2[0], '_ptts_flat', None) is flat and \
                        (e2[1] != e2[0]._version or e2[2] != flat.epoch) and e2[4].data_ptr() == k2[1]:
                    todo.append((k2, e2))
            if len(todo) == 1:
                call('ptts_split3_dense_weight', ptr(Bm), ldb, K, N, transB, ptr(buf), stream(), tag=(K, N, transB))
            else:
                descs = (_hip.DenseSplitDesc * len(todo))()
                for d, (k2, e2) in zip(descs, todo):
                    d.w, d.planes, d.ldw, d.K, d.N, d.transposed = k2[1], e2[3].data_ptr(), k2[4], k2[2], k2[3], k2[5]
                    cls.planes[k2] = (e2[0], e2[0]._version, flat.epoch, e2[3], e2[4])
                call('ptts_split3_dense_weight_grouped', ctypes.cast(descs, ctypes.c_void_p), len(todo), stream(), tag=(len(todo),))
        return ent[3]

    @classmethod
    def clear(cls):
        cls.planes = {k: (e[0], None, None, e[3], e[4]) for k, e in cls.planes.items() if len(e) == 5}

    @classmethod
    def eligible(cls, A, C, M, N, K, lda, ldc, in_side):
        if not (cls.enabled and M >= 1024 and N >= 16 and K >= 16 and K % 4 == 0 and lda % 4 == 0):
            return False
        if not _hip.lib().ptts_dense_bf16x6_supported(M, N, K, lda, ldc):
            return False
        return all(t is None or t.data_ptr() % 16 == 0 for t in (A,) + tuple(in_side))


def dense_split(on):
    _DenseSplit.enabled = _DenseSplit.default if on is None else bool(on)


def _ptr_off(t, off):
    return None if t is None else t.as_strided((1,), (1,), t.storage_offset() + off)


def gemm_raw(A, Bm, C, M, N, K, transA=0, lda=None, rows_per_seg=None, seg_stride=0, transB=0, ldb=None, ldc=None,
             bias=None, mode=IN_NONE, scale=None, shift=None, mask_src=None, alpha=0.3, accumulate=0, out_mask=None,
             colsum_b=None, res=None):
    if res is not None:
        R = res.numel() // N
        assert not accumulate and out_mask is None and M % R == 0 and res.is_contiguous()
        N1 = N if (N <= 256 or N % 256 == 0 or N % 256 > 32) else N - N % 256
        if transA == 0 and seg_stride == 0 and (rows_per_seg is None or rows_per_seg == M) and colsum_b is None and N1 == N and \
                _DenseSplit.eligible(A, C, M, N, K, K if lda is None else lda, N if ldc is None else ldc, (scale, shift, mask_src)):
            planes = _DenseSplit.get(Bm, K, N, (N if transB == 0 else K) if ldb is None else ldb, transB)
            if planes is not None:
                call('ptts_dense_bf16x6_res', ptr(A), ptr(planes), ptr(bias), ptr(C), M, N, K, K if lda is None else lda, N if ldc is None else ldc,
                     mode, ptr(scale), ptr(shift), ptr(mask_src), alpha, ptr(res), R, N, None, stream(), tag=(M, N, K, transB, 'res'))
                return C
        gemm_raw(A, Bm, C, M, N, K, transA, lda, rows_per_seg, seg_stride, transB, ldb, ldc, bias, mode, scale, shift, mask_src, alpha)
        Cv = C.view(M // R, R, N) if (ldc is None or ldc == N) else None
        assert Cv is not None, 'gemm_raw: a residual needs a dense C'
        Cv.add_(res.view(1, R, N))
        return C
    for t in (A, Bm, C, bias, scale, shift, mask_src):
        if t is not None:
            assert t.is_cuda and t.dtype == torch.float32
    if lda is None:
        lda = K if transA == 0 else M
    if rows_per_seg is None:
        rows_per_seg = M if transA == 0 else K
    if ldb is None:
        ldb = N if transB == 0 else K
    if ldc is None:
        ldc = N
    if transA == 1 and transB == 0 and seg_stride == 0 and rows_per_seg == K and out_mask is None and bias is None \
            and _wgrad_split_ok(A.as_strided((1, 1), (lda, 1)), Bm.as_strided((1, 1), (ldb, 1)), mask_src, scale, shift, M, N, K):
        if not accumulate:
            C.zero_()
        if colsum_b is not None:
            colsum_b.zero_()
        ws = _workspace(_hip.lib().ptts_dense_wgrad_workspace_bytes(M, N, K), A.device)
        call('ptts_dense_wgrad_bf16x6', ptr(A), ptr(Bm), ptr(mask_src), ptr(scale), ptr(shift), ptr(C), ptr(colsum_b),
             ptr(ws), ws.numel(), M, N, K, lda, ldb, ldc, mode, alpha, stream(), tag=(M, N, K))
        return C
    if transA == 0 and seg_stride == 0 and rows_per_seg == M and colsum_b is None:
        N1 = N if (N <= 256 or N % 256 == 0 or N % 256 > 32) else N - N % 256
        if _DenseSplit.eligible(A, C, M, N1, K, lda, ldc, (scale, shift, mask_src)):
            planes = _DenseSplit.get(Bm, K, N1, ldb, transB)
            if planes is not None and _BNStats.want and _BNStats.enabled and N1 == N and N % 4 == 0 and ldc % 4 == 0 and mask_src is None and \
                    out_mask is None and not accumulate and mode in (IN_NONE, IN_LRELU):
                cap = _hip.lib().ptts_dense_bf16x6_stats_rows(M, N)
                part = torch.empty((cap, 2 * N), dtype=torch.float64, device=A.device)
                nrows = ctypes.c_int(0)
                call('ptts_dense_bf16x6_stats', ptr(A), ptr(planes), ptr(bias), ptr(C), M, N, K, lda, ldc, mode, ptr(scale), ptr(shift),
                     alpha, ptr(part), cap, ctypes.byref(nrows), stream(), tag=(M, N, K, transB, 'stats'))
                _BNStats.last = (part, nrows.value, M)
                return C
            if planes is not None:
                call('ptts_dense_bf16x6', ptr(A), ptr(planes), ptr(bias), ptr(C), M, N1, K, lda, ldc, mode, ptr(scale), ptr(shift),
                     ptr(mask_src), alpha, accumulate, ptr(out_mask), stream(), tag=(M, N1, K, transB))
                if N1 < N:
                    gemm_raw(A, _ptr_off(Bm, N1 * (ldb if transB else 1)), _ptr_off(C, N1), M, N - N1, K, lda=lda,
                             transB=transB, ldb=ldb, ldc=ldc, bias=_ptr_off(bias, N1), mode=mode, scale=scale,
                             shift=shift, mask_src=mask_src, alpha=alpha, accumulate=accumulate, out_mask=_ptr_off(out_mask, N1))
                return C
    call('ptts_gemm', ptr(A), ptr(Bm), ptr(bias), ptr(C), M, N, K, transA, lda, rows_per_seg, seg_stride,
         transB, ldb, ldc, mode, ptr(scale), ptr(shift), ptr(mask_src), alpha, accumulate, ptr(out_mask), ptr(colsum_b), stream(),
         tag=(M, N, K, transA, transB, int(seg_stride != 0)))
    return C


def colsums(x2d, mode=IN_NONE, scale=None, shift=None, mask_src=None, alpha=0.3):
    f32c(x2d, 'colsums.x')
    rows, C = x2d.shape
    sums = torch.empty(2 * C, dtype=torch.float64, device=x2d.device)
    nws = _hip.lib().ptts_colstats_workspace_bytes(rows, C)
    ws = _workspace(nws, x2d.device)
    call('ptts_colstats', ptr(x2d), rows, C, mode, ptr(scale), ptr(shift), ptr(mask_src), alpha, ptr(sums),
         ptr(ws), ws.numel(), stream(), tag=(rows, C, mode))
    return sums


def _colsum_f32(x2d):
    return colsums(x2d)[:x2d.shape[1]].to(torch.float32)


def _affine_act_bwd_raw(dy, x, y, scale, shift, act, alpha, want_dx=True):
    f32c(dy, 'act_bwd.dy'); f32c(x, 'act_bwd.x')
    C = x.shape[-1]
    rows = x.numel() // C
    dx = torch.empty_like(x) if want_dx else None
    dsums = torch.empty(2 * C, dtype=torch.float64, device=x.device)
    nws = _hip.lib().ptts_colstats_workspace_bytes(rows, C)
    ws = _workspace(nws, x.device)
    call('ptts_affine_act_bwd', ptr(dy), ptr(x), ptr(y), ptr(scale), ptr(shift), ptr(dx), ptr(dsums), ptr(ws),
         ws.numel(), rows, C, act, alpha, stream())
    d32 = dsums.to(torch.float32)
    return dx, d32[:C], d32[C:]


class Conv2dFn(torch.autograd.Function):
    @staticmethod
    def forward(ctx, x, w, b, scale, shift, mode, alpha, dil_t, pad_mode, bf16=None):
        ctx.save_for_backward(x, w, scale, shift)
        ctx.has_b = b is not None
        ctx.cfg = (mode, alpha, dil_t, pad_mode)
        ctx.planes = 1 if bf16 else 3
        ctx.gw, ctx.gb = _Deferred.targets(w, b)
        ctx.set_materialize_grads(False)
        return _conv2d_fwd_raw(x, w, b, scale, shift, None, mode, alpha, dil_t, pad_mode, ctx.planes, bf16 == 'out16')

    @staticmethod
    def backward(ctx, dy):
        if dy is None:
            return (None,) * 10
        x, w, scale, shift = ctx.saved_tensors
        mode, alpha, dil_t, pad_mode = ctx.cfg
        planes = ctx.planes
        need_x, need_w, need_b = ctx.needs_input_grad[0], ctx.needs_input_grad[1], ctx.has_b and ctx.needs_input_grad[2]
        need_aff = scale is not None and (ctx.needs_input_grad[3] or ctx.needs_input_grad[4])
        dy = dy.contiguous()
        if _Flags.skip_param_grads:
            need_w = need_b = need_aff = False
        if torch.is_grad_enabled() and need_x:
            if scale is not None:
                raise RuntimeError('second-order gradients through a BatchNorm-fused conv2d are not supported')
            dx = Conv2dBwdDataFn.apply(dy, x, w, mode, alpha, dil_t, pad_mode, ctx.gw, planes)
            dw = db = None
            if need_w or need_b:
                with torch.no_grad():
                    if _conv2d_can_defer(ctx, need_w, need_b) and \
                            _conv2d_bwd_deferred(dy, x, w, None, mode, alpha, dil_t, pad_mode, False,
                                                 ctx.gw if need_w else None, ctx.gb if need_b else None, planes) is not False:
                        return dx, None, None, None, None, None, None, None, None, None
                    _, dw, db, _, _ = _conv2d_bwd_raw(dy, x, w, None, None, None, mode, alpha, dil_t, pad_mode,
                                                      False, need_w, need_b, False, planes)
            return dx, dw, db, None, None, None, None, None, None, None
        if (need_w or need_b) and not need_aff and scale is None and _conv2d_can_defer(ctx, need_w, need_b):
            dxd = _conv2d_bwd_deferred(dy, x, w, None, mode, alpha, dil_t, pad_mode, need_x,
                                       ctx.gw if need_w else None, ctx.gb if need_b else None, planes)
            if dxd is not False:
                return dxd, None, None, None, None, None, None, None, None, None
        dx, dw, db, dscale, dshift = _conv2d_bwd_raw(dy, x, w, scale, shift, None, mode, alpha, dil_t, pad_mode,
                                                     need_x, need_w, need_b, need_aff, planes)
        return dx, dw, db, dscale, dshift, None, None, None, None, None


def _conv2d_can_defer(ctx, need_w, need_b):
    return _Deferred.live() and (not need_w or ctx.gw is not None) and (not need_b or ctx.gb is not None)


class Conv2dBwdDataFn(torch.autograd.Function):
    @staticmethod
    def forward(ctx, dy, x, w, mode, alpha, dil_t, pad_mode, gw=None, planes=3):
        ctx.save_for_backward(dy, x, w)
        ctx.cfg = (mode, alpha, dil_t, pad_mode)
        ctx.gw = gw
        ctx.planes = planes
        ctx.set_materialize_grads(False)
        dx, _, _, _, _ = _conv2d_bwd_raw(dy, x, w, None, None, None, mode, alpha, dil_t, pad_mode,
                                         True, False, False, False, planes)
        return dx

    @staticmethod
    @torch.autograd.function.once_differentiable
    def backward(ctx, u):
        if u is None:
            return (None,) * 9
        dy, x, w = ctx.saved_tensors
        mode, alpha, dil_t, pad_mode = ctx.cfg
        planes = ctx.planes
        u = u.contiguous()
        m2, msk = (IN_MASKMUL, x) if mode == IN_LRELU else (IN_NONE, None)
        cot_dy = cot_w = None
        if ctx.needs_input_grad[0] and ctx.needs_input_grad[2] and m2 == IN_MASKMUL and _C2M.enabled and _C2M.eligible(u, w, dil_t) and \
                0.0 <= alpha <= 1.0 and _C2MFused.ok(u, dil_t, pad_mode, planes):
            cot_dy, buf, nblocks, npart = _conv2d_mfma_bwd_fused(2, u, dy, msk, w, alpha)
            rows = (buf, 4096, nblocks, npart, w.numel(), w.shape[3])
            if _Deferred.live() and ctx.gw is not None:
                _Deferred.queue_conv(rows + (ctx.gw, None))
            else:
                cot_w = torch.zeros_like(w)
                _conv2d_reduce([rows + (cot_w, None)])
            return cot_dy, None, cot_w, None, None, None, None, None, None
        if ctx.needs_input_grad[0]:
            cot_dy = _conv2d_fwd_raw(u, w, None, None, None, msk, m2, alpha, dil_t, pad_mode, planes, _is16(dy))
        if ctx.needs_input_grad[2]:
            if _Deferred.live() and ctx.gw is not None and \
                    _conv2d_bwd_deferred(dy, u, w, msk, m2, alpha, dil_t, pad_mode, False, ctx.gw, None, planes) is not False:
                return cot_dy, None, None, None, None, None, None, None, None
            _, cot_w, _, _, _ = _conv2d_bwd_raw(dy, u, w, None, None, msk, m2, alpha, dil_t, pad_mode,
                                                False, True, False, False, planes)
        return cot_dy, None, cot_w, None, None, None, None, None, None


def conv2d(v, w, b=None, dil_t=1, pad_mode=PAD_SAME, bf16=None):
    z, mode, scale, shift, alpha = _prep(v)
    return Conv2dFn.apply(z, w, b, scale, shift, mode, alpha, dil_t, pad_mode, bf16)


class _PairFlags(object):
    enabled = os.environ.get('PTTS_PAIR_FORWARD', '1') == '1'


def pair_forward(on):
    _PairFlags.enabled = (os.environ.get('PTTS_PAIR_FORWARD', '1') == '1') if on is None else bool(on)


def _adjacent(x0, x1):
    return (torch.is_tensor(x0) and torch.is_tensor(x1) and x0.is_cuda and x0.dtype == torch.float32 and x1.dtype == torch.float32 and
            x0.is_contiguous() and x1.is_contiguous() and x0.shape[1:] == x1.shape[1:] and
            x1.data_ptr() == x0.data_ptr() + x0.numel() * 4 and
            x0.untyped_storage().data_ptr() == x1.untyped_storage().data_ptr())


def _cat_view(x0, x1):
    return torch.as_strided(x0, (x0.shape[0] + x1.shape[0],) + tuple(x0.shape[1:]), x0.stride())


class _FakeCtx(object):
    def __init__(self, saved, needs, **attrs):
        self.saved_tensors, self.needs_input_grad = saved, needs
        for k, v in attrs.items():
            setattr(self, k, v)


def _sum_opt(a, b):
    return b if a is None else (a if b is None else a + b)


class Conv2dPairFn(torch.autograd.Function):
    @staticmethod
    def forward(ctx, x0, x1, w, b, mode, alpha, dil_t, pad_mode):
        y = _conv2d_fwd_raw(_cat_view(x0, x1), w, b, None, None, None, mode, alpha, dil_t, pad_mode, 3, False)
        ctx.save_for_backward(x0, x1, w)
        ctx.has_b = b is not None
        ctx.cfg = (mode, alpha, dil_t, pad_mode)
        ctx.gw, ctx.gb = _Deferred.targets(w, b)
        ctx.set_materialize_grads(False)
        return y[:x0.shape[0]], y[x0.shape[0]:]

    @staticmethod
    def backward(ctx, dy0, dy1):
        x0, x1, w = ctx.saved_tensors
        nig = ctx.needs_input_grad
        dxs, dw, db = [None, None], None, None
        for i, (dy, x) in enumerate(((dy0, x0), (dy1, x1))):
            if dy is None:
                continue
            c = _FakeCtx((x, w, None, None), (nig[i], nig[2], nig[3], False, False), has_b=ctx.has_b, cfg=ctx.cfg, planes=3, gw=ctx.gw, gb=ctx.gb)
            g = Conv2dFn.backward(c, dy)
            dxs[i], dw, db = g[0], _sum_opt(dw, g[1]), _sum_opt(db, g[2])
        return dxs[0], dxs[1], dw, db, None, None, None, None


def conv2d_pair(v0, v1, w, b=None, dil_t=1, pad_mode=PAD_SAME, bf16=None):
    z0, mode0, sc0, sh0, al0 = _prep(v0)
    z1, mode1, sc1, sh1, al1 = _prep(v1)
    if _PairFlags.enabled and bf16 is None and sc0 is None and sc1 is None and mode0 == mode1 and al0 == al1 and _adjacent(z0, z1):
        return Conv2dPairFn.apply(z0, z1, w, b, mode0, al0, dil_t, pad_mode)
    return conv2d(v0, w, b, dil_t, pad_mode, bf16), conv2d(v1, w, b, dil_t, pad_mode, bf16)


class _C2C(object):
    tables = {}

    @staticmethod
    def supported(F, ws):
        if not ws:
            return False
        KT, KF, cin0, Cc = ws[0].shape
        if any(tuple(w.shape) != (KT, KF, 4, Cc) for w in ws[1:]):
            return False
        return bool(_hip.lib().ptts_conv2d_chain_supported(int(F), len(ws), int(cin0), int(Cc), int(KT), int(KF)))

    @classmethod
    def table(cls, ws, bs):
        flat = getattr(ws[0], '_ptts_flat', None)
        epoch = None if flat is None else flat.epoch
        sid = _hip.stream_id()
        key = (tuple(id(w) for w in ws), sid)
        vers = tuple(w._version for w in ws) + tuple(-1 if b is None else b._version for b in bs)
        ent = cls.tables.get(key)
        if ent is None or any(a is not b for a, b in zip(ent[0], ws)) or ent[2] != vers or ent[3] != epoch or flat is None:
            tab = ent[4] if ent is not None else torch.empty(_hip.lib().ptts_conv2d_chain_tables_bytes(), dtype=torch.uint8, device=ws[0].device)
            for w in ws:
                f32c(w, 'conv2d_chain.w')
            wp = (ctypes.c_void_p * len(ws))(*[w.data_ptr() for w in ws])
            bp = (ctypes.c_void_p * len(ws))(*[None if b is None else f32c(b, 'conv2d_chain.b').data_ptr() for b in bs])
            call('ptts_conv2d_chain_tables', wp, bp, ptr(tab), len(ws), int(ws[0].shape[2]), stream(), tag=(len(ws),))
            ent = (tuple(ws), tuple(bs), vers, epoch, tab)
            if len(cls.tables) > 64:
                cls.tables = {}
            cls.tables[key] = ent
        return ent[4]

    @classmethod
    def clear(cls):
        cls.tables = {}


def _chain_x0(x0):
    if not (x0.is_cuda and x0.dtype == torch.float32 and x0.dim() == 3 and x0.stride(2) == 1 and x0.stride(0) == x0.shape[1] * x0.stride(1)):
        x0 = x0.contiguous()
        if not (x0.is_cuda and x0.dtype == torch.float32):
            raise _hip.HipLibraryError('conv2d_chain: expected a float32 device tensor [B,T,F], got {} {}'.format(x0.device, x0.dtype))
    return x0


def _chain_reduce(parts, nblocks, npart, ws, gws, gbs, want_b):
    L = len(ws)
    rows = [(parts, l * nblocks * npart * 4, nblocks, npart, w.numel(), w.shape[3]) for l, w in enumerate(ws)]
    if _Deferred.live() and all(g is not None for g in gws) and (not want_b or all(g is not None for g in gbs)):
        _Deferred.queue_conv(*[r + (gw, gb if want_b else None) for r, gw, gb in zip(rows, gws, gbs)])
        return None, None
    dws = [torch.zeros_like(w) for w in ws]
    dbs = [torch.zeros(w.shape[3], dtype=torch.float32, device=w.device) for w in ws] if want_b else [None] * L
    _conv2d_reduce([r + (dw, db) for r, dw, db in zip(rows, dws, dbs)])
    return dws, dbs


class Conv2dChainFn(torch.autograd.Function):
    @staticmethod
    def forward(ctx, x0, alpha, *wb):
        ws, bs = list(wb[0::2]), list(wb[1::2])
        x0 = _chain_x0(x0)
        B, T, F = x0.shape
        L = len(ws)
        tab = _C2C.table(ws, bs)
        FP = (F + 1) & ~1
        maps = torch.empty((max(L - 1, 1), B, T, FP, 4), dtype=torch.bfloat16, device=x0.device)
        a_last = torch.empty((B, T, F, 4), dtype=torch.bfloat16, device=x0.device)
        call('ptts_conv2d_chain_fwd', ptr(x0), x0.stride(1), ptr(tab), ptr(maps), ptr(a_last), B, T, F, L, alpha, stream(), tag=(B, T, F, L))
        ctx.save_for_backward(x0, maps, a_last, tab, *ws)
        ctx.alpha, ctx.L, ctx.has_b = alpha, L, [b is not None for b in bs]
        ctx.gws, ctx.gbs = _Deferred.targets(*ws), _Deferred.targets(*bs)
        ctx.set_materialize_grads(False)
        return a_last

    @staticmethod
    def backward(ctx, d_last):
        if d_last is None:
            return (None,) * (2 + 2 * ctx.L)
        x0, maps, a_last, tab = ctx.saved_tensors[:4]
        a_last = a_last.detach()
        ws = list(ctx.saved_tensors[4:])
        L, alpha = ctx.L, ctx.alpha
        B, T, F = x0.shape
        need_x = ctx.needs_input_grad[0]
        need_w = any(ctx.needs_input_grad[2 + 2 * l] or (ctx.has_b[l] and ctx.needs_input_grad[3 + 2 * l]) for l in range(L))
        if _Flags.skip_param_grads:
            need_w = False
        d_last = _st(d_last.contiguous(), 'conv2d_chain.d_last')
        g0 = None
        grads = [None] * (2 * L)
        if need_x:
            if torch.is_grad_enabled():
                g0 = Conv2dChainBwdDataFn.apply(d_last, maps, a_last, tab, alpha, (ctx.gws, int(ws[0].shape[2])), *ws)
            else:
                g0 = torch.empty((B, T, F), dtype=torch.float32, device=x0.device)
                call('ptts_conv2d_chain_bwd_data', ptr(d_last), int(_is16(d_last)), ptr(maps), ptr(a_last), ptr(tab), None, ptr(g0),
                     B, T, F, L, alpha, stream(), tag=(B, T, F, L, 0))
        if need_w:
            with torch.no_grad():
                parts = torch.empty(_hip.lib().ptts_conv2d_chain_partials_bytes(L), dtype=torch.uint8, device=x0.device)
                nblocks, npart = ctypes.c_int(0), ctypes.c_int(0)
                call('ptts_conv2d_chain_bwd', ptr(d_last), int(_is16(d_last)), ptr(x0), x0.stride(1), ptr(maps), ptr(a_last), ptr(tab),
                     ptr(parts), parts.numel(), ctypes.byref(nblocks), ctypes.byref(npart), B, T, F, L, int(ws[0].shape[2]), alpha, stream(),
                     tag=(B, T, F, L))
                want_b = any(ctx.has_b)
                dws, dbs = _chain_reduce(parts, nblocks.value, npart.value, ws, ctx.gws, ctx.gbs, want_b)
                if dws is not None:
                    for l in range(L):
                        grads[2 * l] = dws[l]
                        grads[2 * l + 1] = dbs[l] if ctx.has_b[l] else None
        return (g0, None) + tuple(grads)


class Conv2dChainBwdDataFn(torch.autograd.Function):
    @staticmethod
    def forward(ctx, d_last, maps, a_last, tab, alpha, extra, *ws):
        gws, cin0 = extra
        B, T, F, _ = a_last.shape
        L = len(ws)
        FP = (F + 1) & ~1
        gmaps = torch.empty((L, B, T, FP, 4), dtype=torch.bfloat16, device=a_last.device)
        g0 = torch.empty((B, T, F), dtype=torch.float32, device=a_last.device)
        call('ptts_conv2d_chain_bwd_data', ptr(d_last), int(_is16(d_last)), ptr(maps), ptr(a_last), ptr(tab), ptr(gmaps), ptr(g0),
             B, T, F, L, alpha, stream(), tag=(B, T, F, L, 1))
        ctx.save_for_backward(gmaps, maps, a_last, tab, *ws)
        ctx.cfg = (alpha, L, cin0, d_last.dtype)
        ctx.gws = gws
        ctx.set_materialize_grads(False)
        return g0

    @staticmethod
    @torch.autograd.function.once_differentiable
    def backward(ctx, u0):
        if u0 is None:
            return (None,) * (6 + len(ctx.saved_tensors) - 4)
        gmaps, maps, a_last, tab = ctx.saved_tensors[:4]
        ws = list(ctx.saved_tensors[4:])
        alpha, L, cin0, d_dtype = ctx.cfg
        B, T, F, _ = a_last.shape
        u0 = f32c(u0.contiguous(), 'conv2d_chain.u0')
        out = torch.empty((B, T, F, 4), dtype=d_dtype, device=u0.device)
        parts = torch.empty(_hip.lib().ptts_conv2d_chain_partials_bytes(L), dtype=torch.uint8, device=u0.device)
        nblocks, npart = ctypes.c_int(0), ctypes.c_int(0)
        call('ptts_conv2d_chain_second', ptr(u0), ptr(gmaps), ptr(maps), ptr(a_last), ptr(tab), ptr(out), int(d_dtype == torch.bfloat16),
             ptr(parts), parts.numel(), ctypes.byref(nblocks), ctypes.byref(npart), B, T, F, L, cin0, alpha, stream(), tag=(B, T, F, L))
        need_w = any(ctx.needs_input_grad[6 + l] for l in range(L))
        grads = [None] * L
        if need_w:
            dws, _ = _chain_reduce(parts, nblocks.value, npart.value, ws, ctx.gws, [None] * L, False)
            if dws is not None:
                grads = dws
        return (out if ctx.needs_input_grad[0] else None, None, None, None, None, None) + tuple(grads)


def conv2d_chain(x0, ws, bs, alpha=0.3):
    wb = []
    for w, b in zip(ws, bs):
        wb += [w, b]
    return Conv2dChainFn.apply(x0, float(alpha), *wb)


def _dense_bwd_data(dy2, x2, w, mode, scale, shift, alpha, want_affine):
    M, N = dy2.shape
    K = w.shape[0]
    da = torch.empty((M, K), dtype=torch.float32, device=dy2.device)
    if mode == IN_LRELU and scale is None:
        gemm_raw(dy2, w, da, M, K, N, transB=1, ldb=N, alpha=alpha, out_mask=x2)
        return da, None, None
    if mode == IN_LRELU and _BNStats.enabled and K % 4 == 0 and _DenseSplit.eligible(dy2, da, M, K, N, N, K, (x2, scale, shift)):
        planes = _DenseSplit.get(w, N, K, N, 1)
        if planes is not None:
            cap = _hip.lib().ptts_dense_bf16x6_stats_rows(M, K)
            part = torch.empty((cap, 2 * K), dtype=torch.float64, device=dy2.device)
            nrows = ctypes.c_int(0)
            call('ptts_dense_bf16x6_bwd_affine', ptr(dy2), ptr(planes), ptr(da), M, K, N, N, K, ptr(x2), ptr(scale), ptr(shift), alpha,
                 ptr(part), cap, ctypes.byref(nrows), stream(), tag=(M, K, N, 1, 'bwd_affine'))
            if not want_affine:
                return da, None, None
            dsums = torch.empty(2 * K, dtype=torch.float64, device=dy2.device)
            call('ptts_partial_rows_sum', ptr(part), nrows.value, 2 * K, ptr(dsums), stream())
            d32 = dsums.to(torch.float32)
            return da, d32[:K], d32[K:]
    gemm_raw(dy2, w, da, M, K, N, transB=1, ldb=N)
    if mode == IN_NONE:
        return da, None, None
    dx, dscale, dshift = _affine_act_bwd_raw(da, x2, None, scale, shift, ACT_LRELU, alpha)
    if not want_affine:
        dscale = dshift = None
    return dx, dscale, dshift


class DenseFn(torch.autograd.Function):
    @staticmethod
    def forward(ctx, x, w, b, scale, shift, mode, alpha, res=None):
        f32c(x, 'dense.x'); f32c(w, 'dense.w')
        K, N = w.shape
        assert x.shape[-1] == K, 'dense: input width {} != kernel rows {}'.format(x.shape[-1], K)
        M = x.numel() // K
        y = torch.empty(x.shape[:-1] + (N,), dtype=torch.float32, device=x.device)
        gemm_raw(x, w, y, M, N, K, bias=b, mode=mode, scale=scale, shift=shift, alpha=alpha, res=None if res is None else f32c(res, 'dense.res'))
        ctx.res_shape = None if res is None else tuple(res.shape)
        ctx.save_for_backward(x, w, scale, shift)
        ctx.has_b = b is not None
        ctx.cfg = (mode, alpha)
        ctx.gw, ctx.gb = _Deferred.targets(w, b)
        ctx.set_materialize_grads(False)
        return y

    @staticmethod
    def backward(ctx, dy):
        if dy is None:
            return (None,) * 8
        x, w, scale, shift = ctx.saved_tensors
        mode, alpha = ctx.cfg
        K, N = w.shape
        M = x.numel() // K
        dres = None
        if ctx.res_shape is not None and ctx.needs_input_grad[7]:
            R = 1
            for d_ in ctx.res_shape: R *= d_
            k = dy.numel() // R
            dres = dy.reshape(ctx.res_shape) if k == 1 else dy.reshape((k,) + ctx.res_shape).sum(0)
        need_x, need_w, need_b = ctx.needs_input_grad[0], ctx.needs_input_grad[1], ctx.has_b and ctx.needs_input_grad[2]
        need_aff = scale is not None and (ctx.needs_input_grad[3] or ctx.needs_input_grad[4])
        if _Flags.skip_param_grads:
            need_w = need_b = need_aff = False
        dy = dy.contiguous()
        dy2, x2 = dy.view(M, N), x.view(M, K)
        second_order = torch.is_grad_enabled() and need_x
        dx = dw = db = dscale = dshift = None
        if second_order:
            if scale is not None:
                raise RuntimeError('second-order gradients through a BatchNorm-fused dense layer are not supported')
            dx = DenseBwdDataFn.apply(dy, x, w, mode, alpha, ctx.gw)
        with torch.no_grad():
            if need_x and not second_order:
                dx2, dscale, dshift = _dense_bwd_data(dy2, x2, w, mode, scale, shift, alpha, need_aff)
                dx = dx2.view(x.shape)
            elif need_aff:
                _, dscale, dshift = _dense_bwd_data(dy2, x2, w, mode, scale, shift, alpha, True)
            if need_w and _Deferred.live() and ctx.gw is not None and N > 4 and (not need_b or ctx.gb is not None) \
                    and M >= 2048 and (scale is None or mode == IN_LRELU):
                _defer_wgrad(x2, dy2, ctx.gw, ctx.gb if need_b else None, K, N, M, mode, scale, shift, None, alpha)
                need_w = need_b = False
            if need_w:
                dw = torch.empty_like(w)
                fuse_b = need_b and N > 4
                if fuse_b:
                    db = torch.empty(N, dtype=torch.float32, device=dy.device)
                gemm_raw(x2, dy2, dw, K, N, M, transA=1, lda=K, rows_per_seg=M,
                         mode=mode, scale=scale, shift=shift, alpha=alpha, colsum_b=db if fuse_b else None)
            if need_b and db is None:
                db = _colsum_f32(dy2)
        return dx, dw, db, dscale, dshift, None, None, dres


class DenseBwdDataFn(torch.autograd.Function):
    @staticmethod
    def forward(ctx, dy, x, w, mode, alpha, gw=None):
        K, N = w.shape
        M = x.numel() // K
        ctx.save_for_backward(dy, x, w)
        ctx.cfg = (mode, alpha)
        ctx.gw = gw
        ctx.set_materialize_grads(False)
        dx2, _, _ = _dense_bwd_data(dy.view(M, N), x.view(M, K), w, mode, None, None, alpha, False)
        return dx2.view(x.shape)

    @staticmethod
    @torch.autograd.function.once_differentiable
    def backward(ctx, u):
        if u is None:
            return (None,) * 6
        dy, x, w = ctx.saved_tensors
        mode, alpha = ctx.cfg
        K, N = w.shape
        M = x.numel() // K
        u2 = u.contiguous().view(M, K)
        m2, msk = (IN_MASKMUL, x.view(M, K)) if mode == IN_LRELU else (IN_NONE, None)
        cot_dy = cot_w = None
        if ctx.needs_input_grad[0]:
            cot_dy = torch.empty((M, N), dtype=torch.float32, device=u.device)
            gemm_raw(u2, w, cot_dy, M, N, K, mode=m2, mask_src=msk, alpha=alpha)
            cot_dy = cot_dy.view(dy.shape)
        if ctx.needs_input_grad[2]:
            if _Deferred.live() and ctx.gw is not None and N > 4 and M >= 2048:
                _defer_wgrad(u2, dy.view(M, N), ctx.gw, None, K, N, M, m2, None, None, msk, alpha)
            else:
                cot_w = torch.empty_like(w)
                gemm_raw(u2, dy.view(M, N), cot_w, K, N, M, transA=1, lda=K, rows_per_seg=M,
                         mode=m2, mask_src=msk, alpha=alpha)
        return cot_dy, None, cot_w, None, None, None


class DensePairFn(torch.autograd.Function):
    @staticmethod
    def forward(ctx, x0, x1, w, b, mode, alpha, res):
        K, N = w.shape
        xc = _cat_view(x0, x1)
        M = xc.numel() // K
        y = torch.empty(xc.shape[:-1] + (N,), dtype=torch.float32, device=xc.device)
        gemm_raw(xc, w, y, M, N, K, bias=b, mode=mode, alpha=alpha, res=res)
        ctx.save_for_backward(x0, x1, w)
        ctx.has_b = b is not None
        ctx.cfg = (mode, alpha)
        ctx.res_shape = None if res is None else tuple(res.shape)
        ctx.gw, ctx.gb = _Deferred.targets(w, b)
        ctx.set_materialize_grads(False)
        return y[:x0.shape[0]], y[x0.shape[0]:]

    @staticmethod
    def backward(ctx, dy0, dy1):
        x0, x1, w = ctx.saved_tensors
        nig = ctx.needs_input_grad
        dxs, dw, db, dres = [None, None], None, None, None
        for i, (dy, x) in enumerate(((dy0, x0), (dy1, x1))):
            if dy is None:
                continue
            c = _FakeCtx((x, w, None, None), (nig[i], nig[2], nig[3], False, False, False, False, nig[6]), has_b=ctx.has_b, cfg=ctx.cfg,
                         res_shape=ctx.res_shape, gw=ctx.gw, gb=ctx.gb)
            g = DenseFn.backward(c, dy)
            dxs[i], dw, db, dres = g[0], _sum_opt(dw, g[1]), _sum_opt(db, g[2]), _sum_opt(dres, g[7])
        return dxs[0], dxs[1], dw, db, None, None, dres


def dense_pair(v0, v1, w, b=None, res=None):
    z0, mode0, sc0, sh0, al0 = _prep(v0)
    z1, mode1, sc1, sh1, al1 = _prep(v1)
    if _PairFlags.enabled and sc0 is None and sc1 is None and mode0 == mode1 and al0 == al1 and _adjacent(z0, z1):
        return DensePairFn.apply(z0, z1, w, b, mode0, al0, None if res is None else res.contiguous())
    return dense(v0, w, b, res), dense(v1, w, b, res)


def dense(v, w, b=None, res=None):
    z, mode, scale, shift, alpha = _prep(v)
    if res is None:
        return DenseFn.apply(z, w, b, scale, shift, mode, alpha)
    return DenseFn.apply(z, w, b, scale, shift, mode, alpha, res.contiguous())


def _pad_time(a, lo, hi):
    B, T, C = a.shape
    ap = torch.zeros((B, T + lo + hi, C), dtype=torch.float32, device=a.device)
    ap[:, lo:lo + T].copy_(a)
    return ap


class _C1Cache(object):
    enabled = False
    capture = False
    key = None
    ap = None
    y = None


def conv1d_cache(on):
    _C1Cache.enabled = bool(on)
    _C1Cache.key = _C1Cache.ap = _C1Cache.y = None


class _C1Split(object):
    default = os.environ.get('PTTS_CONV1D_SPLIT', '1') == '1'
    enabled = default
    x_src = None
    x_key = None
    x_planes = None
    w_planes = {}

    @staticmethod
    def eligible(a, w):
        B, T, Cin = a.shape
        KW, _, N = w.shape
        return a.is_cuda and N % 128 == 0 and (T >= 128 or B == 1) and 2 * (KW - 1) + 127 < 176

    @classmethod
    def frames(cls, a, pl, pr):
        B, T, Cin = a.shape
        Cp = (Cin + 31) // 32 * 32
        key = (a._version, tuple(a.shape), pl, pr, _hip.stream_id())
        if cls.x_src is a and cls.x_key == key:
            return cls.x_planes, Cp
        planes = torch.empty((3, Cp // 32, B, T + pl + pr, 32), dtype=torch.bfloat16, device=a.device)
        call('ptts_split3_frames', ptr(a), ptr(planes[0]), ptr(planes[1]), ptr(planes[2]), B, T, Cin, pl, pr, Cp, stream(),
             tag=(B, T, Cin))
        cls.x_src, cls.x_key, cls.x_planes = a, key, planes
        return planes, Cp

    @classmethod
    def kernel(cls, w):
        KW, Cin, N = w.shape
        Cp = (Cin + 31) // 32 * 32
        flat = getattr(w, '_ptts_flat', None)
        epoch = None if flat is None else flat.epoch
        ent = cls.w_planes.get(id(w))
        sid = _hip.stream_id()
        if ent is not None and ent[0] is w and ent[1] == w._version and ent[2] == epoch and ent[4] == sid and flat is not None:
            return ent[3]
        planes = ent[3] if ent is not None and ent[0] is w and ent[4] == sid else torch.empty((3, Cp // 32, N, KW, 32), dtype=torch.bfloat16, device=w.device)
        call('ptts_split3_weight_t', ptr(w), ptr(planes[0]), ptr(planes[1]), ptr(planes[2]), KW, Cin, N, Cp, stream(),
             tag=(KW, Cin, N))
        cls.w_planes[id(w)] = (w, w._version, epoch, planes, sid)
        return planes

    WGRAD_KW = (3, 5, 21)
    xt_src = None
    xt_key = None
    xt_planes = None

    @staticmethod
    def eligible_wgrad(KW, N):
        return KW in _C1Split.WGRAD_KW and N % 32 == 0

    @staticmethod
    def plane_len(B, T, KW):
        qsteps = (B * (T + KW - 1) + 31) // 32
        return (qsteps * 32 + 64 + 63) // 64 * 64

    @staticmethod
    def transposed(x, B, T, C, pl, Tp, Pp):
        Crows = (C + 63) // 64 * 64
        planes = torch.empty((3, Crows, Pp), dtype=torch.bfloat16, device=x.device)
        call('ptts_split3_frames_t', ptr(x), ptr(planes[0]), ptr(planes[1]), ptr(planes[2]), B, T, C, pl, Tp, Crows, Pp, stream(),
             tag=(B, T, C))
        return planes, Crows

    @classmethod
    def frames_t(cls, src, saved, padded, B, T, C, KW):
        Tp = T + KW - 1
        Pp = cls.plane_len(B, T, KW)
        key = None if src is None else (src._version, tuple(src.shape), KW, _hip.stream_id())
        if src is not None and cls.xt_src is src and cls.xt_key == key:
            return cls.xt_planes
        if padded:
            planes, Crows = cls.transposed(saved, B, Tp, C, 0, Tp, Pp)
        else:
            planes, Crows = cls.transposed(saved, B, T, C, (KW - 1) // 2, Tp, Pp)
        out = (planes, Crows, Pp)
        if src is not None:
            cls.xt_src, cls.xt_key, cls.xt_planes = src, key, out
        return out

    @classmethod
    def clear(cls):
        cls.x_src = cls.x_key = cls.x_planes = None
        cls.xt_src = cls.xt_key = cls.xt_planes = None
        cls.w_planes = {}


class _C1WgradT(object):
    enabled = os.environ.get('PTTS_WGRAD_T', '1') == '1'
    src = None
    key = None
    planes = None

    @classmethod
    def frames_t(cls, src, ap, KW):
        B, Tp, C = ap.shape
        Pp = _C1Split.plane_len(B, Tp - (KW - 1), KW)
        Crows = (C + 63) // 64 * 64
        key = None if src is None else (src._version, tuple(src.shape), KW, _hip.stream_id())
        if src is not None and cls.src is src and cls.key == key:
            return cls.planes
        xt = torch.empty((Crows, Pp), dtype=torch.float32, device=ap.device)
        call('ptts_transpose_frames', ptr(ap), ptr(xt), B, Tp, C, 0, Tp, Crows, Pp, stream(), tag=(B, Tp, C))
        out = (xt, Crows, Pp)
        if src is not None:
            cls.src, cls.key, cls.planes = src, key, out
        return out

    @classmethod
    def clear(cls):
        cls.src = cls.key = cls.planes = None


def clear_caches():
    _C1Split.clear()
    _C1FFT.clear()
    _C1WgradT.clear()
    _C2M.clear()
    _C2C.clear()
    _DenseSplit.clear()
    _C1Cache.key = _C1Cache.ap = _C1Cache.y = None


class _C1FFT(object):
    default = os.environ.get('PTTS_CONV1D_FFT', '1') == '1'
    enabled = default
    KWS = (3, 5, 7, 9, 11, 21)
    wgrad_enabled = os.environ.get('PTTS_CONV1D_FFT_WGRAD', '1') == '1'
    bf16_one_product = os.environ.get('PTTS_CONV1D_FFT_BF16', '1') == '1'
    seg_target = int(os.environ.get('PTTS_CONV1D_FFT_SEG', '100'))
    consts = {}
    x_src = None; x_key = None; x_hat = None
    xw_src = None; xw_key = None; xw_planes = None
    w_hat = {}
    bufs = {}

    @staticmethod
    def eligible(a, w):
        B, T, Cin = a.shape
        KW, _, N = w.shape
        if not (a.is_cuda and B * T >= 4096 and KW >= 3 and KW % 2 == 1 and T % 4 == 0 and N % 4 == 0 and Cin >= 64):
            return False
        return B * (T // _C1FFT.segment(T, KW)) <= 65535

    @classmethod
    def segment(cls, T, KW):
        tgt = cls.seg_target
        if tgt <= 0:
            return T
        best = T
        for S in range(4, T + 1, 4):
            if T % S == 0 and S >= 2 * KW and abs(S - tgt) < abs(best - tgt):
                best = S
        return best

    @classmethod
    def _buf(cls, name, key, nfloats, dev):
        sid = _hip.stream_id()
        k = (name, key, sid)
        t = cls.bufs.get(k)
        if t is None:
            for k2 in [k2 for k2 in cls.bufs if k2[0] == name and k2[2] == sid]:
                del cls.bufs[k2]
            t = cls.bufs[k] = torch.zeros(nfloats, dtype=torch.float32, device=dev)
        return t

    @classmethod
    def _scratch(cls, name, nbytes, dev):
        k = ('scratch', name, _hip.stream_id())
        t = cls.bufs.get(k)
        if t is None or t.numel() < nbytes:
            t = cls.bufs[k] = torch.empty(int(nbytes), dtype=torch.uint8, device=dev)
        return t

    @classmethod
    def const(cls, T, KW, Cin, dev):
        key = (T, KW, Cin, dev.index, _hip.stream_id(), cls.seg_target)
        c = cls.consts.get(key)
        if c is not None:
            return c
        import math
        S = cls.segment(T, KW)
        NS = T // S
        P = (S + KW - 1 + 3) // 4 * 4
        NB = P // 2 + 1
        pl = (KW - 1) // 2
        f = torch.arange(NB, dtype=torch.float64).view(NB, 1)
        i = torch.arange(P, dtype=torch.float64).view(1, P)
        th = 2.0 * math.pi * torch.remainder(f * i, P) / P
        D = torch.stack([torch.cos(th), -torch.sin(th)], dim=1).reshape(2 * NB, P)
        cf = torch.full((NB,), 2.0, dtype=torch.float64); cf[0] = 1.0; cf[P // 2] = 1.0
        R = 2 * NB
        Rp = (R + 3) // 4 * 4
        E = torch.zeros(S, Rp, dtype=torch.float64)
        E[:, 0:R:2] = (torch.cos(th[:, :S]) * cf.view(NB, 1) / P).t()
        E[:, 1:R:2] = (-torch.sin(th[:, :S]) * cf.view(NB, 1) / P).t()
        k = torch.arange(KW, dtype=torch.float64).view(1, KW)
        tk = 2.0 * math.pi * torch.remainder(f * k, P) / P
        Tw = torch.stack([torch.cos(tk), torch.sin(tk)], dim=1).reshape(R, KW)
        NBp = (NB + 3) // 4 * 4
        T2 = torch.zeros(2 * KW, NBp, dtype=torch.float64)
        T2[:KW, :NB] = (torch.cos(tk) * cf.view(NB, 1) / P).t()
        T2[KW:, :NB] = (torch.sin(tk) * cf.view(NB, 1) / P).t()
        TP = (2 * KW + 15) // 16 * 16
        T2f = torch.zeros(NB, TP, dtype=torch.float64)
        T2f[:, :2 * KW] = T2[:, :NB].t()
        to = lambda m: m.to(torch.float32).to(dev).contiguous()
        c = {'S': S, 'NS': NS, 'P': P, 'NB': NB, 'R': R, 'Rp': Rp, 'NBp': NBp, 'TP': TP, 'pl': pl, 'Kh': (Cin + 7) // 8 * 8,
             'D': to(D), 'E': to(E), 'Tw': to(Tw), 'T2': to(T2), 'T2f': to(T2f)}
        cls.consts[key] = c
        return c

    @classmethod
    def x_transform(cls, a, KW):
        B, T, Cin = a.shape
        key = (a._version, tuple(a.shape), KW, _hip.stream_id())
        if cls.x_src is a and cls.x_key == key:
            return cls.x_hat
        c = cls.const(T, KW, Cin, a.device)
        NB, Kh, NS, S, P = c['NB'], c['Kh'], c['NS'], c['S'], c['P']
        Z = B * NS
        Ap = cls._buf('Ap', (B, T, Cin, KW, S), NB * 2 * Z * 2 * Kh, a.device)
        lib = _hip.lib()
        npb = lib.ptts_dense_planes_bytes(Cin, P)
        xpl = cls._scratch('xpl', Z * npb, a.device)
        call('ptts_split3_frame_windows', ptr(a), B, T, Cin, NS, S, -c['pl'], P, P, ptr(xpl), npb, stream(), tag=('x', Z))
        call('ptts_dense_bf16x6_batched', ptr(c['D']), 0, ptr(xpl), npb, None, ptr(Ap), 2 * Kh, Z, c['R'], Cin, P, P, Z * 2 * Kh, 3, stream(),
             tag=('dft', Z, c['R'], Cin, P))
        call('ptts_dft_mirror', ptr(Ap), NB, Z, Cin, Kh, stream())
        cls.x_src, cls.x_key, cls.x_hat = a, key, Ap
        return Ap

    @classmethod
    def kernel(cls, w, T):
        KW, Cin, N = w.shape
        flat = getattr(w, '_ptts_flat', None)
        epoch = None if flat is None else flat.epoch
        sid = _hip.stream_id()
        c = cls.const(T, KW, Cin, w.device)
        NB, Kh = c['NB'], c['Kh']
        geo = (c['S'], NB, Kh)
        ent = cls.w_hat.get((id(w), sid))
        if ent is not None and ent[0] is w and ent[1] == w._version and ent[2] == epoch and flat is not None and ent[5] == geo:
            if cls.frozen_log is not None and id(flat) in cls.frozen:
                cls.frozen_log.append((w, ent[4], T))
            return ent[4]
        lib = _hip.lib()
        npb = lib.ptts_dense_planes_bytes(N, 2 * Kh)
        if ent is not None and ent[0] is w and ent[5] == geo:
            planes = ent[4]
        else:
            planes = torch.empty(NB * npb, dtype=torch.uint8, device=w.device)
        cls._build_kernel_planes(w, c, planes)
        if len(cls.w_hat) >= 8 and (id(w), sid) not in cls.w_hat:
            cls.w_hat = {k: e for k, e in cls.w_hat.items() if id(getattr(e[0], '_ptts_flat', None)) in cls.frozen}
        cls.w_hat[(id(w), sid)] = (w, w._version, epoch, None, planes, geo, T)
        return planes

    @classmethod
    def _build_kernel_planes(cls, w, c, planes):
        KW, Cin, N = w.shape
        NB, Kh = c['NB'], c['Kh']
        if KW in cls.KWS:
            call('ptts_conv1d_freq_kernel_planes', ptr(w), ptr(c['Tw']), ptr(planes), NB, KW, Cin, N, Kh, stream(), tag=(NB, KW, Cin, N))
        else:
            npb = _hip.lib().ptts_dense_planes_bytes(N, 2 * Kh)
            What = torch.zeros(c['R'] * Kh * N, dtype=torch.float32, device=w.device)
            gemm_raw(c['Tw'], w.view(KW, Cin * N), What, c['R'], Cin * N, KW, lda=KW, ldb=Cin * N, ldc=Kh * N)
            call('ptts_split3_dense_weight_strided', ptr(What), 2 * Kh * N, ptr(planes), npb, NB, N, 2 * Kh, N, 0, stream(), tag=('w', NB))

    frozen = set()
    frozen_log = None

    @classmethod
    def refresh_planes(cls, items):
        for w, planes, T in items:
            KW, Cin, N = w.shape
            cls._build_kernel_planes(w, cls.const(T, KW, Cin, w.device), planes)
        return len(items)

    @classmethod
    def forward(cls, a, w, b, y):
        B, T, Cin = a.shape
        KW, _, N = w.shape
        c = cls.const(T, KW, Cin, a.device)
        NB, Kh, NS, S = c['NB'], c['Kh'], c['NS'], c['S']
        Z = B * NS
        lib = _hip.lib()
        Ap = cls.x_transform(a, KW)
        wpl = cls.kernel(w, T)
        npw = lib.ptts_dense_planes_bytes(N, 2 * Kh)
        Yh = cls._scratch('Yh', NB * 2 * Z * N * 4, a.device)
        call('ptts_dense_bf16x6_batched', ptr(Ap), 2 * Z * 2 * Kh, ptr(wpl), npw, None, ptr(Yh), 2 * Z * N, NB, 2 * Z, N, 2 * Kh,
             2 * Kh, N, 1 if _Flags.bf16_products else 3, stream(), tag=('freq', NB, 2 * Z, N, 2 * Kh))
        npy = lib.ptts_dense_planes_bytes(N, c['R'])
        ypl = cls._scratch('ypl', Z * npy, a.device)
        call('ptts_split3_dense_weight_strided', ptr(Yh), N, ptr(ypl), npy, Z, Z * N, c['R'], N, 0, stream(), tag=('y', Z))
        call('ptts_dense_bf16x6_batched', ptr(c['E']), 0, ptr(ypl), npy, ptr(b), ptr(y), S * N, Z, S, N, c['Rp'], c['Rp'], N, 3, stream(),
             tag=('idft', Z, S, N, c['Rp']))

    @classmethod
    def has_x(cls, a, KW):
        return a is not None and cls.x_src is a and cls.x_key == (a._version, tuple(a.shape), KW, _hip.stream_id())

    @classmethod
    def wgrad(cls, a, dy, KW):
        B, T, Cin = a.shape
        N = dy.shape[-1]
        c = cls.const(T, KW, Cin, a.device)
        NB, Kh, NS, S, P = c['NB'], c['Kh'], c['NS'], c['S'], c['P']
        Z = B * NS
        lib = _hip.lib()
        dev = a.device
        Ap = cls.x_hat
        npx = lib.ptts_dense_planes_bytes(2 * Kh, 2 * Z)
        if cls.xw_src is not a or cls.xw_key != cls.x_key or cls.xw_planes is None:
            xw = cls._scratch('xw', NB * npx, dev)
            call('ptts_split3_dense_weight_strided', ptr(Ap), 2 * Z * 2 * Kh, ptr(xw), npx, NB, 2 * Kh, 2 * Z, 2 * Kh, 0, stream(), tag=('xw', NB))
            cls.xw_src, cls.xw_key, cls.xw_planes = a, cls.x_key, xw
        npd = lib.ptts_dense_planes_bytes(N, P)
        dpl = cls._scratch('dpl', Z * npd, dev)
        call('ptts_split3_frame_windows', ptr(dy), B, T, N, NS, S, 0, P, S, ptr(dpl), npd, stream(), tag=('dy', Z))
        DYh = cls._scratch('DYh', NB * 2 * Z * N * 4, dev)
        call('ptts_dense_bf16x6_batched', ptr(c['D']), 0, ptr(dpl), npd, None, ptr(DYh), N, Z, c['R'], N, P, P, Z * N, 3, stream(),
             tag=('dft_dy', Z, c['R'], N, P))
        DYt = cls._scratch('DYt', NB * N * 2 * Z * 4, dev)
        call('ptts_transpose_batched', ptr(DYh), ptr(DYt), NB, 2 * Z, N, stream())
        Gt = cls._scratch('Gt', NB * N * 2 * Kh * 4, dev)
        call('ptts_dense_bf16x6_batched', ptr(DYt), N * 2 * Z, ptr(cls.xw_planes), npx, None, ptr(Gt), N * 2 * Kh, NB, N, 2 * Kh, 2 * Z,
             2 * Z, 2 * Kh, 1 if _Flags.bf16_products else 3, stream(), tag=('corr', NB, N, 2 * Kh, 2 * Z))
        dw = torch.empty((KW, Cin, N), dtype=torch.float32, device=dev)
        if KW in cls.KWS:
            ws = _workspace(lib.ptts_conv1d_freq_wgrad_inverse_workspace_bytes(KW, Cin, N), dev)
            call('ptts_conv1d_freq_wgrad_inverse', ptr(Gt), ptr(c['T2f']), ptr(dw), ptr(ws), ws.numel(), NB, c['TP'], KW, Cin, N, Kh, stream(),
                 tag=(NB, KW, Cin, N))
        else:
            out2 = torch.empty(2 * KW * N * 2 * Kh, dtype=torch.float32, device=dev)
            gemm_raw(c['T2'], Gt[:NB * N * 2 * Kh * 4].view(torch.float32), out2, 2 * KW, N * 2 * Kh, NB, lda=c['NBp'], ldb=N * 2 * Kh, ldc=N * 2 * Kh)
            call('ptts_conv1d_freq_wgrad_combine', ptr(out2), ptr(dw), KW, Cin, N, Kh, stream())
        return dw

    @classmethod
    def clear(cls):
        cls.x_src = cls.x_key = cls.x_hat = None
        cls.xw_src = cls.xw_key = cls.xw_planes = None
        cls.w_hat = {k: (e if id(getattr(e[0], '_ptts_flat', None)) in cls.frozen else (e[0], None, None, e[3], e[4], e[5]) + tuple(e[6:]))
                     for k, e in cls.w_hat.items()}


def conv1d_fft(on):
    _C1FFT.enabled = _C1FFT.default if on is None else bool(on)
    _C1FFT.clear()


def conv1d_split(on):
    _C1Split.enabled = _C1Split.default if on is None else bool(on)
    _C1Split.clear()


class Conv1dFn(torch.autograd.Function):
    @staticmethod
    def forward(ctx, a, w, b, pre=None):
        f32c(a, 'conv1d.a'); f32c(w, 'conv1d.w')
        B, T, Cin = a.shape
        KW, Ci2, N = w.shape
        assert Ci2 == Cin
        pl = (KW - 1) // 2
        if pre is not None:
            saved, padded, y = pre
        else:
            y = torch.empty((B, T, N), dtype=torch.float32, device=a.device)
            if _C1FFT.enabled and _C1Split.enabled and (not _Flags.bf16_products or _C1FFT.bf16_one_product) and _C1FFT.eligible(a, w):
                _C1FFT.forward(a, w, b, y)
                saved, padded = a, False
            elif _C1Split.enabled and not _Flags.deterministic and _C1Split.eligible(a, w):
                xp, Cp = _C1Split.frames(a, pl, KW - 1 - pl)
                wp = _C1Split.kernel(w)
                call('ptts_conv1d_bf16x6', ptr(xp[0]), ptr(xp[1]), ptr(xp[2]), ptr(wp[0]), ptr(wp[1]), ptr(wp[2]), ptr(b), ptr(y),
                     B, T, KW, Cp, N, stream(), tag=(B, T, KW, Cp, N))
                saved, padded = a, False
            else:
                saved, padded = _pad_time(a, pl, KW - 1 - pl), True
                gemm_raw(saved, w, y, B * T, N, KW * Cin, lda=Cin, rows_per_seg=T, seg_stride=(T + KW - 1) * Cin, bias=b)
            if _C1Cache.capture:
                _C1Cache.ap = (saved, padded)
        ctx.save_for_backward(saved, w)
        ctx.padded = padded
        ctx.x_src = a
        ctx.has_b = b is not None
        ctx.dims = (B, T, Cin, KW, N, pl)
        return y

    @staticmethod
    @torch.autograd.function.once_differentiable
    def backward(ctx, dy):
        saved, w = ctx.saved_tensors
        B, T, Cin, KW, N, pl = ctx.dims
        dy = dy.contiguous()
        da = dw = db = None
        need_b = ctx.has_b and ctx.needs_input_grad[2] and not _Flags.skip_param_grads
        want_w = ctx.needs_input_grad[1] and not _Flags.skip_param_grads

        def padded_frames():
            return saved if ctx.padded else _pad_time(saved, pl, KW - 1 - pl)

        if want_w and _C1FFT.enabled and _C1FFT.wgrad_enabled and _C1Split.enabled and (not _Flags.bf16_products or _C1FFT.bf16_one_product) and dy.is_cuda and \
                _C1FFT.has_x(ctx.x_src, KW) and not ctx.padded and (B * (T // _C1FFT.segment(T, KW))) % 2 == 0:
            dw = _C1FFT.wgrad(ctx.x_src, dy, KW)
        elif want_w and _C1Split.enabled and not _Flags.deterministic and dy.is_cuda and _C1Split.eligible_wgrad(KW, N):
            xt, Crows, Pp = _C1Split.frames_t(ctx.x_src, saved, ctx.padded, B, T, Cin, KW)
            yt, _ = _C1Split.transposed(dy, B, T, N, 0, T + KW - 1, Pp)
            dw = torch.empty_like(w)
            call('ptts_conv1d_wgrad_bf16x6', ptr(xt[0]), ptr(xt[1]), ptr(xt[2]), ptr(yt[0]), ptr(yt[1]), ptr(yt[2]), ptr(dw),
                 B, T, KW, Cin, N, Crows, Pp, stream(), tag=(B, T, KW, Cin, N))
        elif want_w and _C1WgradT.enabled and not _Flags.deterministic and dy.is_cuda \
                and _C1Split.eligible_wgrad(KW, N) and B * T >= 2048:
            xt, Crows, Pp = _C1WgradT.frames_t(ctx.x_src, padded_frames(), KW)
            yt = torch.empty((N, Pp), dtype=torch.float32, device=dy.device)
            call('ptts_transpose_frames', ptr(dy), ptr(yt), B, T, N, 0, T + KW - 1, N, Pp, stream(), tag=(B, T, N))
            dw = torch.empty_like(w)
            if need_b:
                db = torch.empty(N, dtype=torch.float32, device=dy.device)
            call('ptts_conv1d_wgrad_t', ptr(xt), ptr(yt), ptr(dw), ptr(db), B, T, KW, Cin, N, Crows, Pp, stream(),
                 tag=(B, T, KW, Cin, N))
        elif want_w:
            dw = torch.empty_like(w)
            if need_b and N > 4:
                db = torch.empty(N, dtype=torch.float32, device=dy.device)
            gemm_raw(padded_frames(), dy, dw, KW * Cin, N, B * T, transA=1, lda=Cin, rows_per_seg=T,
                     seg_stride=(T + KW - 1) * Cin, colsum_b=db)
        if need_b and db is None:
            db = _colsum_f32(dy.view(B * T, N))
        if ctx.needs_input_grad[0]:
            dyp = _pad_time(dy, KW - 1 - pl, pl)
            wf = w.flip(0).permute(0, 2, 1).contiguous()
            da = torch.empty((B, T, Cin), dtype=torch.float32, device=dy.device)
            gemm_raw(dyp, wf, da, B * T, Cin, KW * N, lda=N, rows_per_seg=T, seg_stride=(T + KW - 1) * N)
        return da, dw, db, None


def conv1d(v, w, b=None):
    a = as_tensor(v)
    c = _C1Cache
    flat = getattr(w, '_ptts_flat', None) if c.enabled else None
    if flat is not None:
        key = (a.data_ptr(), a._version, tuple(a.shape), w.data_ptr(), w._version, flat.epoch,
               None if b is None else (b.data_ptr(), b._version), _hip.stream_id())
        if not torch.is_grad_enabled():
            c.capture = True
            try:
                y = Conv1dFn.apply(a, w, b)
            finally:
                c.capture = False
            c.key, c.y = key, y
            return y
        if c.key == key and c.y is not None and c.ap is not None:
            return Conv1dFn.apply(a, w, b, (c.ap[0], c.ap[1], c.y))
    return Conv1dFn.apply(a, w, b)


BN_EPS, BN_MOMENTUM = 1e-3, 0.99


class _SyncBN(object):
    world = 1


def sync_batchnorm(world):
    _SyncBN.world = int(world) if world else 1


def _allreduce_small(t):
    import torch.distributed as dist
    dist.all_reduce(t, op=dist.ReduceOp.SUM)
    return t


class BatchNormTrainFn(torch.autograd.Function):
    @staticmethod
    def forward(ctx, z, gamma, beta, moving_mean, moving_var, update_moving, unbiased_moving):
        f32c(z, 'bn.z')
        C = z.shape[-1]
        rows = z.numel() // C
        dev = z.device
        scale = torch.empty(C, dtype=torch.float32, device=dev)
        shift = torch.empty(C, dtype=torch.float32, device=dev)
        mean = torch.empty(C, dtype=torch.float32, device=dev)
        rstd = torch.empty(C, dtype=torch.float32, device=dev)
        ctx.sync = _SyncBN.world
        ctx.gt = _Deferred.targets(gamma, beta)
        part = getattr(z, '_ptts_bn_partials', None)
        if part is not None and ctx.sync <= 1 and part[2] == rows and part[0].shape[1] == 2 * C:
            call('ptts_bn_finalize_partials', ptr(part[0]), part[1], rows, C, ptr(gamma), ptr(beta), ptr(moving_mean), ptr(moving_var),
                 BN_EPS, BN_MOMENTUM, 1 if update_moving else 0, 1 if unbiased_moving else 0, ptr(scale), ptr(shift), ptr(mean), ptr(rstd),
                 stream(), tag=(rows, C))
            ctx.save_for_backward(z, gamma, mean, rstd)
            return z.view_as(z), scale, shift
        if ctx.sync <= 1 and z.data_ptr() % 16 == 0 and _hip.lib().ptts_bn_batch_stats_supported(rows, C):
            ws = _workspace(_hip.lib().ptts_colstats_workspace_bytes(rows, C), dev)
            call('ptts_bn_batch_stats', ptr(z), rows, C, ptr(gamma), ptr(beta), ptr(moving_mean), ptr(moving_var), BN_EPS, BN_MOMENTUM,
                 1 if update_moving else 0, 1 if unbiased_moving else 0, ptr(scale), ptr(shift), ptr(mean), ptr(rstd),
                 ptr(ws), ws.numel(), ptr(_stream_counter(dev)), stream(), tag=(rows, C))
            ctx.save_for_backward(z, gamma, mean, rstd)
            return z.view_as(z), scale, shift
        sums = colsums(z.view(rows, C))
        if ctx.sync > 1:
            _allreduce_small(sums)
            rows = rows * ctx.sync
        call('ptts_bn_finalize', ptr(sums), rows, ptr(gamma), ptr(beta), ptr(moving_mean), ptr(moving_var),
             BN_EPS, BN_MOMENTUM, 1, 1 if update_moving else 0, 1 if unbiased_moving else 0, C,
             ptr(scale), ptr(shift), ptr(mean), ptr(rstd), stream())
        ctx.save_for_backward(z, gamma, mean, rstd)
        return z.view_as(z), scale, shift

    @staticmethod
    @torch.autograd.function.once_differentiable
    def backward(ctx, dz_through, dscale, dshift):
        z, gamma, mean, rstd = ctx.saved_tensors
        C = z.shape[-1]
        rows = z.numel() // C
        dev = z.device
        dscale = dscale.contiguous() if dscale is not None else torch.zeros(C, dtype=torch.float32, device=dev)
        dshift = dshift.contiguous() if dshift is not None else torch.zeros(C, dtype=torch.float32, device=dev)
        c0 = torch.empty(C, dtype=torch.float32, device=dev)
        c2 = torch.empty(C, dtype=torch.float32, device=dev)
        gt = ctx.gt
        direct = gt[0] is not None and gt[1] is not None and _Deferred.live() and \
            ctx.needs_input_grad[1] and ctx.needs_input_grad[2]
        if direct:
            call('ptts_bn_bwd_coefs_acc', ptr(dscale), ptr(dshift), ptr(mean), ptr(rstd), ptr(gamma), rows, C,
                 ptr(gt[0]), ptr(gt[1]), ptr(c0), ptr(c2), stream())
            _Deferred.note_stream()
            dgamma = dbeta = None
        else:
            dgamma = torch.empty(C, dtype=torch.float32, device=dev)
            dbeta = torch.empty(C, dtype=torch.float32, device=dev)
            call('ptts_bn_bwd_coefs', ptr(dscale), ptr(dshift), ptr(mean), ptr(rstd), ptr(gamma), rows, C,
                 ptr(dgamma), ptr(dbeta), ptr(c0), ptr(c2), stream())
        if ctx.sync > 1:
            both = torch.cat([dscale, dshift])
            _allreduce_small(both)
            scratch = torch.empty(2 * C, dtype=torch.float32, device=dev)
            call('ptts_bn_bwd_coefs', ptr(both[:C]), ptr(both[C:]), ptr(mean), ptr(rstd), ptr(gamma), rows * ctx.sync, C,
                 ptr(scratch[:C]), ptr(scratch[C:]), ptr(c0), ptr(c2), stream())
        dz = None
        if ctx.needs_input_grad[0]:
            dz = torch.empty_like(z)
            if dz_through is not None:
                dz_through = f32c(dz_through.contiguous(), 'bn.dz')
            call('ptts_axpby_cols', ptr(dz_through), None, ptr(z), ptr(c2), ptr(c0), ptr(dz), rows, C, stream())
        return dz, dgamma, dbeta, None, None, None, None


def batchnorm_affine(z, gamma, beta, moving_mean, moving_var, training, update_moving=True, unbiased_moving=False):
    if training:
        return BatchNormTrainFn.apply(z, gamma, beta, moving_mean, moving_var, update_moving, unbiased_moving)
    C = z.shape[-1]
    scale = torch.empty(C, dtype=torch.float32, device=z.device)
    shift = torch.empty(C, dtype=torch.float32, device=z.device)
    call('ptts_bn_finalize', None, 1, ptr(gamma), ptr(beta), ptr(moving_mean), ptr(moving_var), BN_EPS, BN_MOMENTUM,
         0, 0, 0, C, ptr(scale), ptr(shift), None, None, stream())
    return z, scale, shift


class AffineActFn(torch.autograd.Function):
    @staticmethod
    def forward(ctx, x, scale, shift, act, alpha):
        f32c(x, 'affine_act.x')
        C = x.shape[-1]
        rows = x.numel() // C
        y = torch.empty_like(x)
        call('ptts_affine_act', ptr(x), ptr(scale), ptr(shift), ptr(y), rows, C, act, alpha, stream())
        ctx.save_for_backward(x, y, scale, shift)
        ctx.cfg = (act, alpha)
        return y

    @staticmethod
    @torch.autograd.function.once_differentiable
    def backward(ctx, dy):
        x, y, scale, shift = ctx.saved_tensors
        act, alpha = ctx.cfg
        dx, dscale, dshift = _affine_act_bwd_raw(dy.contiguous(), x, y, scale, shift, act, alpha,
                                                 want_dx=ctx.needs_input_grad[0])
        if scale is None:
            dscale = dshift = None
        return dx, dscale, dshift, None, None


def affine_act(x, scale=None, shift=None, act=None, alpha=0.3):
    return AffineActFn.apply(x.contiguous(), scale, shift, ACT_CODES[act], alpha)


class _RNG(object):
    seed = None
    blocks = {}
    scratch = {}
    MASK = (1 << 64) - 1

    @classmethod
    def state(cls, device):
        device = torch.device(device)
        if device.type != 'cuda':
            raise _hip.HipLibraryError('the random generator lives on the device (got {}); there is no CPU path'.format(device))
        idx = torch.cuda.current_device() if device.index is None else device.index
        st = cls.blocks.get(idx)
        if st is None:
            if torch.cuda.is_current_stream_capturing():
                raise _hip.HipLibraryError('the random state block of cuda:{} must exist before a graph is captured: '
                                           'run the model once (or call ops.rng_state()) first'.format(idx))
            st = torch.zeros(2, dtype=torch.int64, device=torch.device('cuda', idx))
            seed = torch.initial_seed() if cls.seed is None else cls.seed
            with torch.cuda.device(idx):
                call('ptts_rng_seed', ptr(st), seed & cls.MASK, 0, stream())
            cls.blocks[idx] = st
            cls.scratch[idx] = torch.zeros(1, dtype=torch.int64, device=st.device)
        return st


def rng_seed(seed, counter=0, device=None):
    seed = int(seed) & _RNG.MASK
    if device is None:
        _RNG.seed = seed
        targets = list(_RNG.blocks.items())
    else:
        st = _RNG.state(device)
        targets = [(st.device.index, st)]
    for idx, st in targets:
        with torch.cuda.device(idx):
            call('ptts_rng_seed', ptr(st), seed, int(counter) & _RNG.MASK, stream())


def rng_state(device=None):
    st = _RNG.state(torch.device('cuda', torch.cuda.current_device()) if device is None else device)
    out = (ctypes.c_ulonglong * 2)()
    with torch.cuda.device(st.device.index):
        call('ptts_rng_state_get', ptr(st), ctypes.cast(out, ctypes.c_void_p), stream())
    return int(out[0]), int(out[1])


def _rank():
    from . import parallel
    return parallel.rank()


class DropoutFn(torch.autograd.Function):
    @staticmethod
    def forward(ctx, z, scale, shift, mode, alpha, rate, b0):
        f32c(z, 'dropout.x')
        if z.dim() != 3:
            raise _hip.HipLibraryError('dropout: expected a [batch, time, features] tensor, got {}'.format(tuple(z.shape)))
        B, T, D = z.shape
        st = _RNG.state(z.device)
        y = torch.empty_like(z)
        used = torch.empty(1, dtype=torch.int64, device=z.device)
        call('ptts_dropout_fwd', ptr(z), ptr(scale), ptr(shift), ptr(y), ptr(st), ptr(used), rate, alpha, mode, B, T, D, b0,
             stream(), tag=(B, T, D, mode))
        ctx.save_for_backward(z, scale, shift, used)
        ctx.cfg = (mode, alpha, rate, b0)
        ctx.mark_non_differentiable(used)
        return y, used

    @staticmethod
    @torch.autograd.function.once_differentiable
    def backward(ctx, dy, _dused):
        z, scale, shift, used = ctx.saved_tensors
        mode, alpha, rate, b0 = ctx.cfg
        B, T, D = z.shape
        dy = dy.contiguous()
        da = torch.empty_like(dy)
        call('ptts_dropout_bwd', ptr(dy), ptr(da), ptr(used), ptr(_RNG.state(z.device)), rate, B, T, D, b0, stream(), tag=(B, T, D))
        if mode != IN_LRELU:
            return da, None, None, None, None, None, None
        dz, dscale, dshift = _affine_act_bwd_raw(da, z, None, scale, shift, ACT_LRELU, alpha, want_dx=ctx.needs_input_grad[0])
        if scale is None:
            dscale = dshift = None
        return dz, dscale, dshift, None, None, None, None


def dropout(v, rate, b0=None):
    lz = as_lazy(v)
    f = _fusable(lz)
    if f is None:
        z, mode, scale, shift = lz.tensor(), IN_NONE, None, None
    else:
        z, (mode, scale, shift) = lz.z, f
    z = z.contiguous()
    if b0 is None:
        b0 = _rank() * z.shape[0]
    return DropoutFn.apply(z, scale, shift, mode, lz.alpha, float(rate), int(b0))[0]


def normal(shape, stddev=1.0, device=None, i0=None):
    device = torch.device('cuda', torch.cuda.current_device()) if device is None else torch.device(device)
    st = _RNG.state(device)
    out = torch.empty(tuple(shape), dtype=torch.float32, device=st.device)
    n = out.numel()
    if i0 is None:
        i0 = _rank() * n
    call('ptts_normal_fill', ptr(out), ptr(st), ptr(_RNG.scratch[st.device.index]), float(stddev), int(i0), n, stream(),
         tag=(n,))
    return out


class GatedMulFn(torch.autograd.Function):
    @staticmethod
    def forward(ctx, a, b):
        f32c(a, 'gated_mul.a'); f32c(b, 'gated_mul.b')
        assert a.shape == b.shape
        y = torch.empty_like(a)
        call('ptts_gated_mul_fwd', ptr(a), ptr(b), ptr(y), a.numel(), stream(), tag=(a.numel(),))
        ctx.save_for_backward(a, b)
        return y

    @staticmethod
    @torch.autograd.function.once_differentiable
    def backward(ctx, dy):
        a, b = ctx.saved_tensors
        dy = dy.contiguous()
        da, db = torch.empty_like(a), torch.empty_like(b)
        call('ptts_gated_mul_bwd', ptr(dy), ptr(a), ptr(b), ptr(da), ptr(db), a.numel(), stream(), tag=(a.numel(),))
        return da, db


def gated_mul(a, b):
    return GatedMulFn.apply(as_tensor(a).contiguous(), as_tensor(b).contiguous())


lstm_trace = None


def _lstm_mark(tag):
    if lstm_trace is not None:
        ev = torch.cuda.Event(enable_timing=True)
        ev.record()
        lstm_trace.append((tag, ev))


class _GradGateFn(torch.autograd.Function):
    @staticmethod
    def forward(ctx, x):
        return x.view_as(x)

    @staticmethod
    def backward(ctx, g):
        return g


def grad_gate(x):
    return _GradGateFn.apply(x)


class _GradInjectFn(torch.autograd.Function):
    @staticmethod
    def forward(ctx, x, holder):
        ctx.holder = holder
        return x.view_as(x)

    @staticmethod
    def backward(ctx, g):
        h = ctx.holder
        extra = h.get('grad')
        if extra is None:
            return g, None
        if h.get('event') is not None:
            torch.cuda.current_stream().wait_event(h['event'])
        h['grad'] = None
        return (extra if g is None else g + extra), None


def grad_inject(x, holder):
    return _GradInjectFn.apply(x, holder)


def lstm_launch(x, W, U, b, reverse=False):
    f32c(x, 'lstm.x'); f32c(W); f32c(U); f32c(b)
    B, T, In = x.shape
    ndir, H, G4 = U.shape
    assert G4 == 4 * H and W.shape == (In, ndir * G4)
    dev = x.device
    xproj = torch.empty((B, T, ndir * G4), dtype=torch.float32, device=dev)
    h = torch.empty((B, T, ndir * H), dtype=torch.float32, device=dev)
    c = torch.empty((B, T, ndir * H), dtype=torch.float32, device=dev)
    gates = torch.empty((B, T, ndir * G4), dtype=torch.float32, device=dev)
    gemm_raw(x, W, xproj, B * T, ndir * G4, In, bias=b)
    wsf = _workspace(_hip.lib().ptts_lstm_fwd_workspace_bytes(B, T, H, ndir), dev)
    _lstm_mark('fwd0')
    call('ptts_lstm_fwd', ptr(xproj), ptr(U), ptr(h), ptr(gates), ptr(c), ptr(wsf), wsf.numel(), B, T, H, ndir, int(reverse), stream())
    _lstm_mark('fwd1')
    return h, c, gates


def _h_prev(h, ndir, H, reverse=False):
    T = h.shape[1]
    hprev = torch.zeros_like(h)
    if T > 1:
        for d in range(ndir):
            rev = (d == 1) if ndir == 2 else bool(reverse)
            sl = slice(d * H, (d + 1) * H)
            if rev:
                hprev[:, :-1, sl].copy_(h[:, 1:, sl])
            else:
                hprev[:, 1:, sl].copy_(h[:, :-1, sl])
    return hprev


lstm_dx_ready = None


class LSTMFn(torch.autograd.Function):
    @staticmethod
    def forward(ctx, x, W, U, b, reverse, pre=None):
        h, c, gates = lstm_launch(x, W, U, b, reverse) if pre is None else pre
        ctx.save_for_backward(x, W, U, h, c, gates)
        ctx.reverse = int(reverse)
        ctx.gt = _Deferred.targets(W, U, b)
        return h

    @staticmethod
    @torch.autograd.function.once_differentiable
    def backward(ctx, dh):
        x, W, U, h, c, gates = ctx.saved_tensors
        B, T, In = x.shape
        ndir, H, G4 = U.shape
        dev = x.device
        dh = dh.contiguous()
        dgates = torch.empty_like(gates)
        nws = _hip.lib().ptts_lstm_bwd_workspace_bytes(B, T, H, ndir)
        ws = _workspace(nws, dev)
        _lstm_mark('bwd0')
        call('ptts_lstm_bwd', ptr(dh), ptr(U), ptr(gates), ptr(c), ptr(dgates), ptr(ws), ws.numel(),
             B, T, H, ndir, ctx.reverse, stream())
        _lstm_mark('bwd1')
        M = B * T
        dx = dW = dU = db = None
        if ctx.needs_input_grad[0]:
            dx = torch.empty_like(x)
            gemm_raw(dgates, W, dx, M, In, ndir * G4, transB=1, ldb=ndir * G4)
            global lstm_dx_ready
            lstm_dx_ready = (dx.data_ptr(), torch.cuda.current_stream().record_event())
        if ctx.needs_input_grad[1]:
            dW = torch.empty_like(W)
            gemm_raw(x, dgates, dW, In, ndir * G4, M, transA=1, lda=In, rows_per_seg=M)
        if ctx.needs_input_grad[3]:
            db = _colsum_f32(dgates.view(M, ndir * G4))
        if ctx.needs_input_grad[2]:
            hprev = _h_prev(h, ndir, H, ctx.reverse)
            dU = torch.empty_like(U)
            for d in range(ndir):
                gemm_raw(hprev.view(M, ndir * H)[:, d * H:], dgates.view(M, ndir * G4)[:, d * G4:], dU[d],
                         H, G4, M, transA=1, lda=ndir * H, rows_per_seg=M, ldb=ndir * G4)
        gt = ctx.gt
        if _Deferred.live() and \
                all(t is not None or g is None for t, g in zip(gt, (dW, dU, db))):
            for t, g in zip(gt, (dW, dU, db)):
                if g is not None:
                    t.add_(g.view(t.shape))
            _Deferred.note_stream()
            dW = dU = db = None
        return dx, dW, dU, db, None, None


def lstm(v, W, U, b, reverse=False, pre=None):
    return LSTMFn.apply(as_tensor(v).contiguous(), W, U, b, reverse, pre)


class GRUFn(torch.autograd.Function):
    @staticmethod
    def forward(ctx, x, W, U, b):
        f32c(x, 'gru.x'); f32c(W); f32c(U); f32c(b)
        B, T, In = x.shape
        ndir, H, G3 = U.shape
        assert G3 == 3 * H and W.shape == (ndir, In, G3) and b.shape == (ndir, G3)
        dev, M = x.device, B * T
        xproj = torch.empty((B, T, ndir * G3), dtype=torch.float32, device=dev)
        h = torch.empty((B, T, ndir * H), dtype=torch.float32, device=dev)
        gates = torch.empty((B, T, ndir * G3), dtype=torch.float32, device=dev)
        rh = torch.empty((B, T, ndir * H), dtype=torch.float32, device=dev)
        xp2 = xproj.view(M, ndir * G3)
        for d in range(ndir):
            gemm_raw(x, W[d], xp2[:, d * G3:], M, G3, In, ldc=ndir * G3, bias=b[d])
        ws = _workspace(_hip.lib().ptts_gru_fwd_workspace_bytes(B, T, H, ndir), dev)
        call('ptts_gru_fwd', ptr(xproj), ptr(U), ptr(h), ptr(gates), ptr(rh), ptr(ws), ws.numel(), B, T, H, ndir, stream(),
             tag=(B, T, H, ndir))
        ctx.save_for_backward(x, W, U, h, gates, rh)
        return h

    @staticmethod
    @torch.autograd.function.once_differentiable
    def backward(ctx, dh):
        x, W, U, h, gates, rh = ctx.saved_tensors
        B, T, In = x.shape
        ndir, H, G3 = U.shape
        dev, M = x.device, B * T
        dh = dh.contiguous()
        dgates = torch.empty_like(gates)
        ws = _workspace(_hip.lib().ptts_gru_bwd_workspace_bytes(B, T, H, ndir), dev)
        call('ptts_gru_bwd', ptr(dh), ptr(U), ptr(h), ptr(gates), ptr(dgates), ptr(ws), ws.numel(), B, T, H, ndir, stream(),
             tag=(B, T, H, ndir))
        dg2 = dgates.view(M, ndir * G3)
        dx = dW = dU = db = None
        if ctx.needs_input_grad[0]:
            dx = torch.empty_like(x)
            for d in range(ndir):
                gemm_raw(dg2[:, d * G3:], W[d], dx, M, In, G3, lda=ndir * G3, transB=1, ldb=G3, accumulate=int(d > 0))
        if ctx.needs_input_grad[1]:
            dW = torch.empty_like(W)
            for d in range(ndir):
                gemm_raw(x, dg2[:, d * G3:], dW[d], In, G3, M, transA=1, lda=In, rows_per_seg=M, ldb=ndir * G3)
        if ctx.needs_input_grad[3]:
            db = _colsum_f32(dg2).view(ndir, G3)
        if ctx.needs_input_grad[2]:
            hprev = _h_prev(h, ndir, H).view(M, ndir * H)
            rh2 = rh.view(M, ndir * H)
            dU = torch.empty_like(U)
            for d in range(ndir):
                gemm_raw(hprev[:, d * H:], dg2[:, d * G3:], dU[d][:, :2 * H], H, 2 * H, M, transA=1, lda=ndir * H,
                         rows_per_seg=M, ldb=ndir * G3, ldc=G3)
                gemm_raw(rh2[:, d * H:], dg2[:, d * G3 + 2 * H:], dU[d][:, 2 * H:], H, H, M, transA=1, lda=ndir * H,
                         rows_per_seg=M, ldb=ndir * G3, ldc=G3)
        return dx, dW, dU, db


def gru(v, W, U, b):
    return GRUFn.apply(as_tensor(v).contiguous(), W, U, b)


def gp_interpolate(real, fake, alpha_b, out=None):
    f32c(real, 'gp.real'); f32c(fake, 'gp.fake'); f32c(alpha_b, 'gp.alpha')
    assert real.shape == fake.shape and alpha_b.numel() == real.shape[0]
    if out is None:
        out = torch.empty_like(real)
    else:
        f32c(out, 'gp.out'); assert out.shape == real.shape
    B = real.shape[0]
    call('ptts_gp_interpolate', ptr(real), ptr(fake), ptr(alpha_b), ptr(out), B, real.numel() // B, stream())
    return out


class GradPenaltyFn(torch.autograd.Function):
    @staticmethod
    def forward(ctx, g):
        f32c(g, 'gp.g')
        B = g.shape[0]
        TD = g.numel() // B
        sq = torch.empty(B, dtype=torch.float32, device=g.device)
        pen = torch.empty(1, dtype=torch.float32, device=g.device)
        coef = torch.empty(B, dtype=torch.float32, device=g.device)
        call('ptts_gp_sqnorm', ptr(g), ptr(sq), B, TD, stream())
        call('ptts_gp_penalty', ptr(sq), ptr(pen), ptr(coef), B, stream())
        ctx.save_for_backward(g, coef)
        return pen.view(())

    @staticmethod
    @torch.autograd.function.once_differentiable
    def backward(ctx, up):
        g, coef = ctx.saved_tensors
        B = g.shape[0]
        dg = torch.empty_like(g)
        up = up.contiguous().view(1)
        call('ptts_gp_scale_rows', ptr(g), ptr(coef), ptr(up), ptr(dg), B, g.numel() // B, stream())
        return dg


def grad_penalty(g):
    return GradPenaltyFn.apply(g.contiguous())


class MeanScaledFn(torch.autograd.Function):
    @staticmethod
    def forward(ctx, v, sign):
        f32c(v, 'wasserstein.v')
        out = torch.empty(1, dtype=torch.float32, device=v.device)
        call('ptts_mean_scaled', ptr(v), v.numel(), float(sign), ptr(out), stream())
        ctx.sign, ctx.shape = float(sign), v.shape
        return out.view(())

    @staticmethod
    @torch.autograd.function.once_differentiable
    def backward(ctx, up):
        n = 1
        for s in ctx.shape:
            n *= s
        return (up * (ctx.sign / n)).expand(ctx.shape).contiguous(), None


class WassersteinPairFn(torch.autograd.Function):
    @staticmethod
    def forward(ctx, v, B):
        f32c(v, 'wasserstein.v')
        n = v.numel()
        h = n // v.shape[0] * B
        out = torch.empty(2, dtype=torch.float32, device=v.device)
        call('ptts_mean_scaled', ptr(v), h, -1.0, ptr(out), stream())
        call('ptts_mean_scaled', ptr(_ptr_off(v, h)), n - h, 1.0, ptr(_ptr_off(out, 1)), stream())
        ctx.cfg = (tuple(v.shape), B, h, n)
        return out[0], out[1]

    @staticmethod
    @torch.autograd.function.once_differentiable
    def backward(ctx, up_v, up_f):
        shape, B, h, n = ctx.cfg
        dv = torch.empty(shape, dtype=torch.float32, device=(up_v if up_v is not None else up_f).device)
        flat = dv.view(-1)
        if up_v is None: flat[:h].zero_()
        else: flat[:h].copy_((up_v * (-1.0 / h)).expand(h))
        if up_f is None: flat[h:].zero_()
        else: flat[h:].copy_((up_f * (1.0 / (n - h))).expand(n - h))
        return dv, None


def wasserstein_pair(v, B):
    return WassersteinPairFn.apply(v.contiguous(), int(B))


def wasserstein(v, sign):
    return MeanScaledFn.apply(v.contiguous(), sign)


class WLSEFn(torch.autograd.Function):
    @staticmethod
    def forward(ctx, yhat, y, w):
        f32c(yhat, 'wlse.yhat'); f32c(y, 'wlse.y'); f32c(w)
        assert yhat.shape == y.shape
        D = y.shape[-1]
        rows = y.numel() // D
        out = torch.empty(1, dtype=torch.float32, device=y.device)
        call('ptts_wlse_fwd', ptr(y), ptr(yhat), ptr(w), ptr(out), rows, D, stream())
        ctx.save_for_backward(yhat, y, w)
        return out.view(())

    @staticmethod
    @torch.autograd.function.once_differentiable
    def backward(ctx, up):
        yhat, y, w = ctx.saved_tensors
        D = y.shape[-1]
        rows = y.numel() // D
        d = torch.empty_like(yhat)
        up = up.contiguous().view(1)
        call('ptts_wlse_bwd', ptr(y), ptr(yhat), ptr(w), ptr(up), ptr(d), rows, D, stream())
        return d, None, None


def wlse(yhat, y, w=None):
    return WLSEFn.apply(yhat.contiguous(), y.contiguous(), w)


def weight_clip_(p, lo, hi):
    f32c(p, 'clip.p')
    call('ptts_weight_clip', ptr(p), p.numel(), float(lo), float(hi), stream())
    return p


def adam_keras_step_(p, g, m, v, step, lr, b1, b2, eps, gscale=1.0):
    for t in (p, g, m, v):
        f32c(t, 'adam')
    assert p.numel() == g.numel() == m.numel() == v.numel()
    assert step.is_cuda and step.dtype == torch.int32
    call('ptts_adam_keras_step', ptr(p), ptr(g), ptr(m), ptr(v), p.numel(), float(lr), float(b1), float(b2),
         float(eps), float(gscale), ptr(step), stream())
```

Measured before the change: 4.752 million.

## Fold small N/K remainder tiles into main dense and wgrad kernels

In the forward dense GEMM, when N exceeds a multiple of 256 by at most 16 columns, the last column block's spare waves compute the extra 16-column tile in-kernel. This replaces a separate fallback GEMM launch for the remainder. The wgrad kernel likewise handles a K remainder of at most 16 rows inside the last k-tile, instead of launching a mostly empty extra tile row, and the reduce kernel is extended to match. Waves with no output columns now skip the MFMA work and only help stage A. The cost is more LDS, more registers in the XT/XR variants, and a forced MT of 7 when 8 was chosen.

```diff
diff --git a/percivaltts_amd/csrc/dense.hip b/percivaltts_amd/csrc/dense.hip
--- a/percivaltts_amd/csrc/dense.hip
+++ b/percivaltts_amd/csrc/dense.hip
@@ -216,6 +216,9 @@
 #ifndef DNS_DEPTH
 #define DNS_DEPTH 2
 #endif
+#ifndef DNS_SKIP_DEAD
+#define DNS_SKIP_DEAD 1
+#endif
 struct DenseArgs {
     const float* A; const float* mask_src; const float* in_scale; const float* in_shift;
     const u16* planes; const float* bias; const float* out_mask; float* C;
@@ -229,7 +232,7 @@
     const float* om_scale; const float* om_shift;
 };
 
-template <int MODE, bool AFFINE, int MT, int NPL>
+template <int MODE, bool AFFINE, int MT, int NPL, bool XT = false>
 __global__ __launch_bounds__(THREADS) void dense_bf16x6_kernel(DenseArgs g) {
     if (gridDim.z > 1) {
         g.A += (long long)blockIdx.z * g.bsA;
@@ -248,6 +251,7 @@
     const int m0 = blockIdx.x * TBM, n0 = blockIdx.y * NBLK;
     const int KS = g.KS;
     const bool wave_live = n0 + 32 * wave < g.N;
+    const bool xt_wave = XT && blockIdx.y == gridDim.y - 1 && wave < MT;
 
     const int kq = tid & 7;
     const float* pa[NA]; const float* pm[NA]; bool oka[NA]; int dst[NA];
@@ -316,6 +320,11 @@
 #pragma unroll
             for (int p = 0; p < NPL; ++p) wf[j][p] = *reinterpret_cast<const bf16x8*>(wp[j] + p * ps + (size_t)s * 512);
     };
+    const u16* wpx = g.planes + (((size_t)((n0 >> 4) + (xt_wave ? NBLK / 16 : 0)) * KS) * 64 + lane) * 8;
+    auto load_wx = [&](int s, bf16x8 (&wf)[NPL]) {
+#pragma unroll
+        for (int p = 0; p < NPL; ++p) wf[p] = *reinterpret_cast<const bf16x8*>(wpx + p * ps + (size_t)s * 512);
+    };
 
     f32x4 acc[MT][2];
 #pragma unroll
@@ -335,9 +344,22 @@
         }
     };
 
+    f32x4 accx = {0.f, 0.f, 0.f, 0.f};
+    const int xoff = boff + (wave < MT ? wave : MT - 1) * 16 * BK;
+    auto read_x = [&](const u16* as, bf16x8 (&bf)[NPL]) {
+#pragma unroll
+        for (int p = 0; p < NPL; ++p) bf[p] = *reinterpret_cast<const bf16x8*>(as + p * PL + xoff);
+    };
+    auto mfma_x = [&](const bf16x8 (&wf)[NPL], const bf16x8 (&bf)[NPL]) {
+#define DNS_MM(PA, PW) accx = __builtin_amdgcn_mfma_f32_16x16x32_bf16(wf[PW < NPL ? PW : 0], bf[PA < NPL ? PA : 0], accx, 0, 0, 0);
+        DNS_PRODUCTS_NPL(NPL, DNS_MM);
+#undef DNS_MM
+    };
+
     constexpr int DEPTH = DNS_DEPTH;
     Stage sg[DEPTH];
     bf16x8 wc[2][NPL], wn[2][NPL];
+    bf16x8 wx[XT ? NPL : 1];
 #pragma unroll
     for (int j = 0; j < DEPTH; ++j) load_a(j, sg[j]);
     load_w(0, wc);
@@ -347,14 +369,25 @@
     auto step = [&](int s, int cut, Stage& nx) {
         const u16* as = As[s & 1];
         load_w(s + 1 < KS ? s + 1 : s, wn);
+        if constexpr (XT) load_wx(s, wx);
         mfma_rows(as, wc, 0, cut);
         commit(nx, As[(s + 1) & 1]);
         load_a(s + 1 + DEPTH, nx);
+        bf16x8 bx[XT ? NPL : 1];
+        if constexpr (XT) read_x(as, bx);
         mfma_rows(as, wc, cut, MT);
+        if constexpr (XT) {
+            if (xt_wave) mfma_x(wx, bx);
+        }
 #pragma unroll
         for (int j = 0; j < 2; ++j)
 #pragma unroll
             for (int p = 0; p < NPL; ++p) wc[j][p] = wn[j][p];
+        __syncthreads();
+    };
+    auto step_dead = [&](int s, Stage& nx) {
+        commit(nx, As[(s + 1) & 1]);
+        load_a(s + 1 + DEPTH, nx);
         __syncthreads();
     };
     auto run = [&](int cut) {
@@ -367,7 +400,45 @@
         for (int j = 0; j < DEPTH; ++j)
             if (s + j < KS) step(s + j, cut, sg[(j + 1) % DEPTH]);
     };
-    if (wave < 4) run(2); else run(MT - 2);
+    auto run_dead = [&]() {
+        int s = 0;
+        for (; s + DEPTH <= KS; s += DEPTH) {
+#pragma unroll
+            for (int j = 0; j < DEPTH; ++j) step_dead(s + j, sg[(j + 1) % DEPTH]);
+        }
+#pragma unroll
+        for (int j = 0; j < DEPTH; ++j)
+            if (s + j < KS) step_dead(s + j, sg[(j + 1) % DEPTH]);
+    };
+    if (DNS_SKIP_DEAD && !XT && !wave_live) run_dead();
+    else if (wave < 4) run(2); else run(MT - 2);
+    if constexpr (XT) {
+        const int m = m0 + 16 * wave + li, n = n0 + NBLK + 4 * lg;
+        if (xt_wave && m < g.M && n < g.N) {
+            const long long off = (long long)m * g.ldc + n;
+            int mr = m; while (g.res && mr >= g.res_rows) mr -= g.res_rows;
+            if (g.vec_out) {
+                f32x4 v = accx;
+                if (g.bias) v += *reinterpret_cast<const f32x4*>(g.bias + n);
+                if (g.out_mask) {
+                    const f32x4 mk = *reinterpret_cast<const f32x4*>(g.out_mask + off);
+#pragma unroll
+                    for (int e = 0; e < 4; ++e) v[e] = v[e] * (mk[e] > 0.f ? 1.f : g.out_alpha);
+                }
+                if (g.res) v += *reinterpret_cast<const f32x4*>(g.res + (long long)mr * g.ldr + n);
+                *reinterpret_cast<f32x4*>(g.C + off) = v;
+            } else {
+#pragma unroll
+                for (int e = 0; e < 4; ++e) {
+                    if (n + e >= g.N) continue;
+                    float v = accx[e] + (g.bias ? g.bias[n + e] : 0.f);
+                    if (g.out_mask) v *= g.out_mask[off + e] > 0.f ? 1.f : g.out_alpha;
+                    if (g.res) v += g.res[(long long)mr * g.ldr + n + e];
+                    g.C[off + e] = v;
+                }
+            }
+        }
+    }
     if (!wave_live) return;
     const bool interior = m0 + TBM <= g.M;
     if (!g.vec_out) {
@@ -467,6 +538,14 @@
     }
 }
 
+template <int MODE, bool AFFINE, int MT, int NPL>
+static void dense_launch_kernel(bool xt, dim3 grid, hipStream_t st, const DenseArgs& g) {
+    if constexpr (MT < 8) {
+        if (xt) { hipLaunchKernelGGL((dense_bf16x6_kernel<MODE, AFFINE, MT, NPL, true>), grid, dim3(THREADS), 0, st, g); return; }
+    }
+    hipLaunchKernelGGL((dense_bf16x6_kernel<MODE, AFFINE, MT, NPL>), grid, dim3(THREADS), 0, st, g);
+}
+
 static int pick_mt(int M, int col_blocks) {
     static int forced = -1;
     if (forced < 0) { const char* e = getenv("PTTS_DENSE_MT"); forced = e ? atoi(e) : 0; }
@@ -496,14 +575,21 @@
     long long lda, ldb;
     float alpha;
     int tiles_n, steps_total, split;
+    int tiles_k, part;
 };
 
 constexpr int WT = 128;
 constexpr int WROW = WT;
 constexpr int WPL = 32 * WROW;
 constexpr int WPART = WT * WT + WT;
-
-template <int MODE, bool AFFINE, int NPL>
+constexpr int WXR = 16;
+constexpr int WXPL = 32 * WXR + 4 * 64;
+constexpr int WPARTX = WXR * WT;
+__host__ __device__ inline bool wgrad_has_rem(int Kin) { return Kin > WT && Kin % WT >= 1 && Kin % WT <= WXR; }
+__host__ __device__ inline int wgrad_tiles_k(int Kin) { return wgrad_has_rem(Kin) ? Kin / WT : (Kin + WT - 1) / WT; }
+__host__ __device__ inline int wgrad_part(int Kin) { return WPART + (wgrad_has_rem(Kin) ? WPARTX : 0); }
+
+template <int MODE, bool AFFINE, int NPL, bool XR = false>
 __global__ __launch_bounds__(THREADS) void dense_wgrad_bf16x6_kernel(WgradArgs g) {
     constexpr bool MASK = MODE == PTTS_IN_MASKMUL;
     extern __shared__ __attribute__((aligned(16))) u16 lds_w[];
@@ -512,6 +598,7 @@
     const int li = lane & 15, lg = lane >> 4;
     const int tile = blockIdx.y, tk = tile / g.tiles_n, tn = tile - tk * g.tiles_n;
     const int k0 = tk * WT, n0 = tn * WT;
+    const bool xr_wg = XR && tk == g.tiles_k - 1;
     const int per = (g.steps_total + g.split - 1) / g.split;
     const int s_begin = blockIdx.x * per, s_end = min(g.steps_total, s_begin + per);
     const int nsteps = max(0, s_end - s_begin);
@@ -529,8 +616,24 @@
     }
     f32x4 sc = {1.f, 1.f, 1.f, 1.f}, sh = {0.f, 0.f, 0.f, 0.f};
     if (AFFINE && a_ok) { sc = *reinterpret_cast<const f32x4*>(g.in_scale + k0 + 4 * c4); sh = *reinterpret_cast<const f32x4*>(g.in_shift + k0 + 4 * c4); }
-    struct Stage { f32x4 va[2], vm[MASK ? 2 : 1], vd[2]; bool ok[2]; };
+    const bool xr_stage = xr_wg && wave < 2;
+    const int xrow = tid >> 2, xkq = g.tiles_k * WT + 4 * (tid & 3);
+    const bool x_ok = xr_stage && xkq < g.Kin;
+    const float* pax = g.A + (x_ok ? xkq : 0);
+    const float* pmx = MASK ? g.mask_src + (x_ok ? xkq : 0) : nullptr;
+    auto xrow_off = [](int row) { return row * WXR + 64 * (row >> 3); };
+    const int xdst = xrow_off(xrow & 31) + 4 * (tid & 3);
+    f32x4 scx = {1.f, 1.f, 1.f, 1.f}, shx = {0.f, 0.f, 0.f, 0.f};
+    if (AFFINE && x_ok) { scx = *reinterpret_cast<const f32x4*>(g.in_scale + xkq); shx = *reinterpret_cast<const f32x4*>(g.in_shift + xkq); }
+    struct Stage { f32x4 va[2], vm[MASK ? 2 : 1], vd[2]; bool ok[2]; f32x4 vx, vmx; bool okx; };
     auto load = [&](int s, Stage& sg) {
+        if (XR && xr_stage) {
+            const int m = (s_begin + s) * 32 + xrow;
+            sg.okx = s < nsteps && m < g.M && x_ok;
+            const long long r = sg.okx ? m : 0;
+            sg.vx = *reinterpret_cast<const f32x4*>(pax + r * g.lda);
+            if (MASK) sg.vmx = *reinterpret_cast<const f32x4*>(pmx + r * g.lda);
+        }
 #pragma unroll
         for (int j = 0; j < 2; ++j) {
             const int m = (s_begin + s) * 32 + ((tid + j * THREADS) >> 5);
@@ -542,8 +645,34 @@
         }
     };
     f32x4 bsum = {0.f, 0.f, 0.f, 0.f};
-    auto commit = [&](const Stage& sg, u16* ls) {
+    auto commit = [&](const Stage& sg, u16* ls, u16* lsx) {
         const f32x4 z4 = {0.f, 0.f, 0.f, 0.f};
+        if (XR && xr_stage) {
+            f32x4 a = sg.vx;
+            if (MODE == PTTS_IN_LRELU) {
+                if (AFFINE) a = a * scx + shx;
+                if (!sg.okx) a = z4;
+#pragma unroll
+                for (int e = 0; e < 4; ++e) a[e] = max_fast(a[e], g.alpha * a[e]);
+            } else if (MASK) {
+                if (!sg.okx) a = z4;
+#pragma unroll
+                for (int e = 0; e < 4; ++e) a[e] = a[e] * (sg.vmx[e] > 0.f ? 1.f : g.alpha);
+            } else {
+                if (!sg.okx) a = z4;
+            }
+            u16* q = lsx + xdst;
+            if (NPL == 3) {
+                unsigned a1, a2, a3, b1, b2, b3;
+                split3_pair(a[0], a[1], a1, a2, a3);
+                split3_pair(a[2], a[3], b1, b2, b3);
+                *reinterpret_cast<u32x2*>(q) = (u32x2){a1, b1};
+                *reinterpret_cast<u32x2*>(q + WXPL) = (u32x2){a2, b2};
+                *reinterpret_cast<u32x2*>(q + 2 * WXPL) = (u32x2){a3, b3};
+            } else {
+                *reinterpret_cast<u32x2*>(q) = (u32x2){pk_bf16(a[0], a[1]), pk_bf16(a[2], a[3])};
+            }
+        }
 #pragma unroll
         for (int j = 0; j < 2; ++j) {
             f32x4 a = sg.va[j], d = sg.vd[j];
@@ -599,6 +728,24 @@
     for (int i = 0; i < 2; ++i)
 #pragma unroll
         for (int j = 0; j < 4; ++j) acc[i][j] = f32x4{0.f, 0.f, 0.f, 0.f};
+    f32x4 accx = {0.f, 0.f, 0.f, 0.f};
+    int axo[2], bxo[2];
+#pragma unroll
+    for (int h = 0; h < 2; ++h) {
+        axo[h] = xrow_off(8 * lg + (li >> 2) + 4 * h) + (li & 3) * 4;
+        bxo[h] = 3 * WPL + tr_off(wave, h);
+    }
+    auto mfma_rem = [&](const u16* ls, const u16* lsx) {
+        bf16x8 af[NPL], bf[NPL];
+#pragma unroll
+        for (int p = 0; p < NPL; ++p) {
+            af[p] = cat8(tr_read(lsx + p * WXPL + axo[0]), tr_read(lsx + p * WXPL + axo[1]));
+            bf[p] = cat8(tr_read(ls + p * WPL + bxo[0]), tr_read(ls + p * WPL + bxo[1]));
+        }
+#define DNS_MM(PA, PW) accx = __builtin_amdgcn_mfma_f32_16x16x32_bf16(af[PA < NPL ? PA : 0], bf[PW < NPL ? PW : 0], accx, 0, 0, 0);
+        DNS_PRODUCTS_NPL(NPL, DNS_MM);
+#undef DNS_MM
+    };
     auto mfma_tile_row = [&](const u16* ls, int i, const bf16x8 (&bf)[4][NPL]) {
         bf16x8 af[NPL];
 #pragma unroll
@@ -616,33 +763,40 @@
             for (int p = 0; p < NPL; ++p) bf[j][p] = cat8(tr_read(ls + p * WPL + bo[j][0]), tr_read(ls + p * WPL + bo[j][1]));
     };
 
+    u16* const buf0 = lds_w;
+    u16* const buf1 = lds_w + 6 * WPL;
+    u16* const xbuf0 = lds_w + 12 * WPL;
+    u16* const xbuf1 = xbuf0 + 3 * WXPL;
     Stage sg;
     load(0, sg);
-    commit(sg, lds_w);
+    commit(sg, buf0, xbuf0);
     load(1, sg);
     __syncthreads();
-    u16* const buf0 = lds_w;
-    u16* const buf1 = lds_w + 6 * WPL;
-    auto step = [&](int s, const u16* cur, u16* nxt, bool stage_first) {
+    auto step = [&](int s, const u16* cur, u16* nxt, const u16* curx, u16* nxtx, bool stage_first) {
         bf16x8 bf[4][NPL];
-        if (stage_first) { commit(sg, nxt); load(s + 2, sg); }
+        if (stage_first) { commit(sg, nxt, nxtx); load(s + 2, sg); }
         read_bf(cur, bf);
         mfma_tile_row(cur, 0, bf);
-        if (!stage_first) { commit(sg, nxt); load(s + 2, sg); }
+        if (!stage_first) { commit(sg, nxt, nxtx); load(s + 2, sg); }
         mfma_tile_row(cur, 1, bf);
+        if (XR && xr_wg) mfma_rem(cur, curx);
         __syncthreads();
     };
     if (wave < 4) {
         int s = 0;
-        for (; s + 1 < nsteps; s += 2) { step(s, buf0, buf1, false); step(s + 1, buf1, buf0, false); }
-        if (s < nsteps) step(s, buf0, buf1, false);
+        for (; s + 1 < nsteps; s += 2) { step(s, buf0, buf1, xbuf0, xbuf1, false); step(s + 1, buf1, buf0, xbuf1, xbuf0, false); }
+        if (s < nsteps) step(s, buf0, buf1, xbuf0, xbuf1, false);
     } else {
         int s = 0;
-        for (; s + 1 < nsteps; s += 2) { step(s, buf0, buf1, true); step(s + 1, buf1, buf0, true); }
-        if (s < nsteps) step(s, buf0, buf1, true);
-    }
-
-    float* out = g.partials + ((size_t)tile * g.split + blockIdx.x) * WPART;
+        for (; s + 1 < nsteps; s += 2) { step(s, buf0, buf1, xbuf0, xbuf1, true); step(s + 1, buf1, buf0, xbuf1, xbuf0, true); }
+        if (s < nsteps) step(s, buf0, buf1, xbuf0, xbuf1, true);
+    }
+
+    float* out = g.partials + ((size_t)tile * g.split + blockIdx.x) * g.part;
+    if (XR && xr_wg) {
+#pragma unroll
+        for (int r = 0; r < 4; ++r) out[WPART + (4 * lg + r) * WT + 16 * wave + li] = accx[r];
+    }
 #pragma unroll
     for (int i = 0; i < 2; ++i)
 #pragma unroll
@@ -677,32 +831,38 @@
     int split[DR_MAX], tiles_n[DR_MAX], Kin[DR_MAX], N[DR_MAX];
     long long ldc[DR_MAX];
 };
-constexpr int DR_BPT = (WPART + 255) / 256;
+__host__ __device__ inline int dr_bpt(int Kin) { return (wgrad_part(Kin) + 255) / 256; }
 __global__ __launch_bounds__(256) void dense_wgrad_reduce_kernel(DwReduceArgs a) {
     int gi = 0;
     while ((int)blockIdx.x >= a.blk_begin[gi + 1]) ++gi;
     const int b = blockIdx.x - a.blk_begin[gi];
-    const int tile = b / DR_BPT, e = (b - tile * DR_BPT) * 256 + threadIdx.x;
-    if (e >= WPART) return;
+    const int PART = wgrad_part(a.Kin[gi]), BPT = dr_bpt(a.Kin[gi]);
+    const int tile = b / BPT, e = (b - tile * BPT) * 256 + threadIdx.x;
+    if (e >= PART) return;
+    const int tk = tile / a.tiles_n[gi], tn = tile - tk * a.tiles_n[gi];
+    const int tiles_k = wgrad_tiles_k(a.Kin[gi]);
+    if (e >= WPART && tk != tiles_k - 1) return;
     const int S = a.split[gi];
-    const float* p = a.partials[gi] + (size_t)tile * S * WPART + e;
+    const float* p = a.partials[gi] + (size_t)tile * S * PART + e;
     float v0 = 0.f, v1 = 0.f, v2 = 0.f, v3 = 0.f, v4 = 0.f, v5 = 0.f, v6 = 0.f, v7 = 0.f;
     int s = 0;
     for (; s + 8 <= S; s += 8) {
-        const float* q = p + (size_t)s * WPART;
-        const float t0 = q[0], t1 = q[(size_t)WPART], t2 = q[(size_t)2 * WPART], t3 = q[(size_t)3 * WPART];
-        const float t4 = q[(size_t)4 * WPART], t5 = q[(size_t)5 * WPART], t6 = q[(size_t)6 * WPART], t7 = q[(size_t)7 * WPART];
+        const float* q = p + (size_t)s * PART;
+        const float t0 = q[0], t1 = q[(size_t)PART], t2 = q[(size_t)2 * PART], t3 = q[(size_t)3 * PART];
+        const float t4 = q[(size_t)4 * PART], t5 = q[(size_t)5 * PART], t6 = q[(size_t)6 * PART], t7 = q[(size_t)7 * PART];
         v0 += t0; v1 += t1; v2 += t2; v3 += t3; v4 += t4; v5 += t5; v6 += t6; v7 += t7;
     }
-    for (; s < S; ++s) v0 += p[(size_t)s * WPART];
+    for (; s < S; ++s) v0 += p[(size_t)s * PART];
     const float v = ((v0 + v1) + (v2 + v3)) + ((v4 + v5) + (v6 + v7));
-    const int tk = tile / a.tiles_n[gi], tn = tile - tk * a.tiles_n[gi];
     if (e < WT * WT) {
         const int k = tk * WT + (e >> 7), n = tn * WT + (e & (WT - 1));
         if (k < a.Kin[gi] && n < a.N[gi]) atomicAdd(a.C[gi] + (long long)k * a.ldc[gi] + n, v);
-    } else if (tk == 0 && a.colsum[gi]) {
+    } else if (e < WPART) {
         const int n = tn * WT + (e - WT * WT);
-        if (n < a.N[gi]) atomicAdd(a.colsum[gi] + n, v);
+        if (tk == 0 && a.colsum[gi] && n < a.N[gi]) atomicAdd(a.colsum[gi] + n, v);
+    } else {
+        const int k = tiles_k * WT + ((e - WPART) >> 7), n = tn * WT + ((e - WPART) & (WT - 1));
+        if (k < a.Kin[gi] && n < a.N[gi]) atomicAdd(a.C[gi] + (long long)k * a.ldc[gi] + n, v);
     }
 }
 
@@ -791,21 +951,18 @@
             (long long)((N + NBLK - 1) / NBLK) <= 65535) ? 1 : 0;
 }
 
-extern "C" int ptts_dense_bf16x6_res(const float* A, const void* planes, const float* bias, float* C, int M, int N, int K,
-                                     long long lda, long long ldc, int in_mode, const float* in_scale, const float* in_shift,
-                                     const float* mask_src, float alpha, const float* res, int res_rows, long long ldr,
-                                     const float* out_mask, void* stream);
+static int dense_launch(const float* A, const void* planes, const float* bias, float* C, int M, int N, int K,
+                        long long lda, long long ldc, int in_mode, const float* in_scale, const float* in_shift,
+                        const float* mask_src, float alpha, const float* res, int res_rows, long long ldr,
+                        const float* out_mask, double* stats, int stats_capacity_rows, int* stats_rows_out, void* stream,
+                        bool extra_tile = false);
 extern "C" int ptts_dense_bf16x6(const float* A, const void* planes, const float* bias, float* C, int M, int N, int K,
                                  long long lda, long long ldc, int in_mode, const float* in_scale, const float* in_shift,
                                  const float* mask_src, float alpha, int accumulate, const float* out_mask, void* stream) {
-    return ptts_dense_bf16x6_res(A, planes, bias, C, M, N, K, lda, ldc, in_mode, in_scale, in_shift, mask_src, alpha,
-                                 accumulate ? C : nullptr, M, ldc, out_mask, stream);
-}
-
-static int dense_launch(const float* A, const void* planes, const float* bias, float* C, int M, int N, int K,
-                        long long lda, long long ldc, int in_mode, const float* in_scale, const float* in_shift,
-                        const float* mask_src, float alpha, const float* res, int res_rows, long long ldr,
-                        const float* out_mask, double* stats, int stats_capacity_rows, int* stats_rows_out, void* stream);
+    return dense_launch(A, planes, bias, C, M, N, K, lda, ldc, in_mode, in_scale, in_shift, mask_src, alpha,
+                        accumulate ? C : nullptr, M, ldc, out_mask, nullptr, 0, nullptr, stream, true);
+}
+
 static thread_local const float* g_om_scale = nullptr;
 static thread_local const float* g_om_shift = nullptr;
 
@@ -844,7 +1001,8 @@
 static int dense_launch(const float* A, const void* planes, const float* bias, float* C, int M, int N, int K,
                         long long lda, long long ldc, int in_mode, const float* in_scale, const float* in_shift,
                         const float* mask_src, float alpha, const float* res, int res_rows, long long ldr,
-                        const float* out_mask, double* stats, int stats_capacity_rows, int* stats_rows_out, void* stream) {
+                        const float* out_mask, double* stats, int stats_capacity_rows, int* stats_rows_out, void* stream,
+                        bool extra_tile) {
     const int accumulate = res != nullptr;
     PTTS_REQUIRE(!res || (res_rows > 0 && ldr >= N && M <= 8LL * res_rows), "dense_bf16x6: bad residual (rows %d, ldr %lld)", res_rows, ldr);
     PTTS_REQUIRE(A && planes && C, "dense_bf16x6: null matrix");
@@ -867,8 +1025,10 @@
     g.lda = lda; g.ldc = ldc; g.alpha = alpha; g.out_alpha = alpha; g.accumulate = accumulate; g.has_affine = in_scale != nullptr; g.vec_out = vec_out;
     g.res = res; g.res_rows = res ? res_rows : 1; g.ldr = ldr;
     g.bsA = g.bsP = g.bsC = 0;
-    const int cb = (N + NBLK - 1) / NBLK;
-    const int mt = pick_mt(M, cb);
+    const bool xt = extra_tile && !stats && !g_om_scale && N > NBLK && N % NBLK >= 1 && N % NBLK <= 16;
+    const int cb = xt ? N / NBLK : (N + NBLK - 1) / NBLK;
+    int mt = pick_mt(M, cb);
+    if (xt && mt == 8) mt = 7;
     const dim3 grid((unsigned)((M + 16 * mt - 1) / (16 * mt)), (unsigned)cb);
     g.stats = stats;
     g.om_scale = g_om_scale; g.om_shift = g_om_shift;
@@ -879,8 +1039,8 @@
     }
     hipStream_t st = (hipStream_t)stream;
     const bool one = ptts::bf16_products();
-#define DNS_L(MODE, AFF, MT) do { if (one) hipLaunchKernelGGL((dense_bf16x6_kernel<MODE, AFF, MT, 1>), grid, dim3(THREADS), 0, st, g); \
-                                  else hipLaunchKernelGGL((dense_bf16x6_kernel<MODE, AFF, MT, 3>), grid, dim3(THREADS), 0, st, g); } while (0)
+#define DNS_L(MODE, AFF, MT) do { if (one) dense_launch_kernel<MODE, AFF, MT, 1>(xt, grid, st, g); \
+                                  else dense_launch_kernel<MODE, AFF, MT, 3>(xt, grid, st, g); } while (0)
 #define DNS_M(MT)                                                                \
     do {                                                                         \
         if (in_mode == PTTS_IN_LRELU) { if (in_scale) DNS_L(PTTS_IN_LRELU, true, MT); else DNS_L(PTTS_IN_LRELU, false, MT); } \
@@ -967,12 +1127,12 @@
 
 extern "C" int ptts_dense_wgrad_bf16x6_supported(int Kin, int N, int M, long long lda, long long ldb) {
     return (Kin > 0 && N > 0 && M > 0 && Kin % 4 == 0 && N % 4 == 0 && lda % 4 == 0 && ldb % 4 == 0 &&
-            (long long)((Kin + WT - 1) / WT) * ((N + WT - 1) / WT) <= 65535) ? 1 : 0;
+            (long long)wgrad_tiles_k(Kin) * ((N + WT - 1) / WT) <= 65535) ? 1 : 0;
 }
 
 namespace {
 int wgrad_split(int Kin, int N, int M) {
-    const int tiles = ((Kin + WT - 1) / WT) * ((N + WT - 1) / WT), steps = (M + 31) / 32;
+    const int tiles = wgrad_tiles_k(Kin) * ((N + WT - 1) / WT), steps = (M + 31) / 32;
     int split = (256 + tiles - 1) / tiles;
     static int env_split = -1;
     if (env_split < 0) { const char* e = getenv("PTTS_DENSE_WGRAD_SPLIT"); env_split = e ? atoi(e) : 0; }
@@ -984,8 +1144,8 @@
 
 extern "C" size_t ptts_dense_wgrad_workspace_bytes(int Kin, int N, int M) {
     if (Kin <= 0 || N <= 0 || M <= 0) return 0;
-    const size_t tiles = (size_t)((Kin + WT - 1) / WT) * ((N + WT - 1) / WT);
-    return tiles * wgrad_split(Kin, N, M) * WPART * sizeof(float);
+    const size_t tiles = (size_t)wgrad_tiles_k(Kin) * ((N + WT - 1) / WT);
+    return tiles * wgrad_split(Kin, N, M) * wgrad_part(Kin) * sizeof(float);
 }
 
 extern "C" int ptts_dense_wgrad_bf16x6_partials(const float* A, const float* dY, const float* mask_src, const float* in_scale,
@@ -1007,7 +1167,9 @@
     WgradArgs g;
     g.A = A; g.dY = dY; g.mask_src = mask_src; g.in_scale = in_scale; g.in_shift = in_shift; g.partials = (float*)workspace;
     g.Kin = Kin; g.N = N; g.M = M; g.lda = lda; g.ldb = ldb; g.alpha = alpha;
-    const int tiles_k = (Kin + WT - 1) / WT;
+    const int tiles_k = wgrad_tiles_k(Kin);
+    const bool xr = wgrad_has_rem(Kin);
+    g.tiles_k = tiles_k; g.part = wgrad_part(Kin);
     g.tiles_n = (N + WT - 1) / WT;
     g.steps_total = (M + 31) / 32;
     const int tiles = tiles_k * g.tiles_n;
@@ -1016,13 +1178,19 @@
     const dim3 grid((unsigned)g.split, (unsigned)tiles);
     hipStream_t st = (hipStream_t)stream;
     constexpr size_t lds = (size_t)2 * 6 * WPL * sizeof(u16);
+    constexpr size_t ldsx = lds + (size_t)2 * 3 * WXPL * sizeof(u16);
     const bool one = ptts::bf16_products();
 #define DNS_W(MODE, AFF)                                                                                                  \
     do {                                                                                                                  \
         static bool attr = false;                                                                                         \
         if (!attr) { (void)hipFuncSetAttribute(reinterpret_cast<const void*>(&dense_wgrad_bf16x6_kernel<MODE, AFF, 3>), hipFuncAttributeMaxDynamicSharedMemorySize, (int)lds); \
-                     (void)hipFuncSetAttribute(reinterpret_cast<const void*>(&dense_wgrad_bf16x6_kernel<MODE, AFF, 1>), hipFuncAttributeMaxDynamicSharedMemorySize, (int)lds); attr = true; } \
-        if (one) hipLaunchKernelGGL((dense_wgrad_bf16x6_kernel<MODE, AFF, 1>), grid, dim3(THREADS), lds, st, g);          \
+                     (void)hipFuncSetAttribute(reinterpret_cast<const void*>(&dense_wgrad_bf16x6_kernel<MODE, AFF, 1>), hipFuncAttributeMaxDynamicSharedMemorySize, (int)lds); \
+                     (void)hipFuncSetAttribute(reinterpret_cast<const void*>(&dense_wgrad_bf16x6_kernel<MODE, AFF, 3, true>), hipFuncAttributeMaxDynamicSharedMemorySize, (int)ldsx); \
+                     (void)hipFuncSetAttribute(reinterpret_cast<const void*>(&dense_wgrad_bf16x6_kernel<MODE, AFF, 1, true>), hipFuncAttributeMaxDynamicSharedMemorySize, (int)ldsx); attr = true; } \
+        if (xr) {                                                                                                         \
+            if (one) hipLaunchKernelGGL((dense_wgrad_bf16x6_kernel<MODE, AFF, 1, true>), grid, dim3(THREADS), ldsx, st, g); \
+            else hipLaunchKernelGGL((dense_wgrad_bf16x6_kernel<MODE, AFF, 3, true>), grid, dim3(THREADS), ldsx, st, g);   \
+        } else if (one) hipLaunchKernelGGL((dense_wgrad_bf16x6_kernel<MODE, AFF, 1>), grid, dim3(THREADS), lds, st, g);   \
         else hipLaunchKernelGGL((dense_wgrad_bf16x6_kernel<MODE, AFF, 3>), grid, dim3(THREADS), lds, st, g);              \
     } while (0)
     if (in_mode == PTTS_IN_LRELU) { if (in_scale) DNS_W(PTTS_IN_LRELU, true); else DNS_W(PTTS_IN_LRELU, false); }
@@ -1043,7 +1211,7 @@
             PTTS_REQUIRE(d.partials && d.C && d.split > 0 && d.Kin > 0 && d.N > 0 && d.ldc >= d.N, "dense_wgrad_reduce_grouped: bad product %d", base + i);
             a.blk_begin[i] = blocks;
             a.tiles_n[i] = (d.N + WT - 1) / WT;
-            blocks += ((d.Kin + WT - 1) / WT) * a.tiles_n[i] * DR_BPT;
+            blocks += wgrad_tiles_k(d.Kin) * a.tiles_n[i] * dr_bpt(d.Kin);
             a.partials[i] = d.partials; a.C[i] = d.C; a.colsum[i] = d.colsum_b; a.split[i] = d.split; a.Kin[i] = d.Kin; a.N[i] = d.N; a.ldc[i] = d.ldc;
         }
         a.blk_begin[a.n] = blocks;
diff --git a/percivaltts_amd/ops.py b/percivaltts_amd/ops.py
--- a/percivaltts_amd/ops.py
+++ b/percivaltts_amd/ops.py
@@ -621,7 +621,7 @@
              ptr(ws), ws.numel(), M, N, K, lda, ldb, ldc, mode, alpha, stream(), tag=(M, N, K))
         return C
     if transA == 0 and seg_stride == 0 and rows_per_seg == M and colsum_b is None:
-        N1 = N if (N <= 256 or N % 256 == 0 or N % 256 > 32) else N - N % 256
+        N1 = N if (N <= 256 or N % 256 == 0 or N % 256 > 32 or N % 256 <= 16) else N - N % 256
         if _DenseSplit.eligible(A, C, M, N1, K, lda, ldc, (scale, shift, mask_src)):
             planes = _DenseSplit.get(Bm, K, N1, ldb, transB)
             if planes is not None and _BNStats.want and _BNStats.enabled and N1 == N and N % 4 == 0 and ldc % 4 == 0 and mask_src is None and \
```

New measurement: 4.801 million, median of 6. 1.01x the previous value.
